# dblanm/gnn-manip

Hardware: AMD Instinct MI355X
Metric: rollout steps/sec (N particles, 10 MP steps, hidden=128) (higher is better)
Workload: dtype f32; 1 GPU; north_star target: N=100k dense synthetic scene, conn_r=0.015, max_neighbours=20, hidden=128, 10 MP steps; n_particles=100000, hidden=128, edges_last_step=1966056, k_steps=6, candidates_per_gpu=1, parallelism=candidate-parallel x1

## Files before the change

gnn_manip_amd/_lib.py:

```python
import ctypes as C
import os

_HERE = os.path.dirname(os.path.abspath(__file__))
LIB_PATH = os.environ.get("GM_LIB_PATH") or os.path.join(_HERE, "libgnnmanip_hip.so")

GM_OK = 0


class GMError(RuntimeError):
    def __init__(self, code, msg):
        super().__init__(f"libgnnmanip_hip: {msg} (status {code})")
        self.code = code


class FeatureDesc(C.Structure):
    _fields_ = [("conn_r", C.c_double), ("k_steps", C.c_int32), ("data_dim", C.c_int32),
                ("cart_col", C.c_int32), ("material_col", C.c_int32), ("control_col", C.c_int32),
                ("nodes_per_graph", C.c_int32),
                ("vel_mean", C.c_float * 3), ("vel_std", C.c_float * 3),
                ("acc_mean", C.c_float * 3), ("acc_std", C.c_float * 3),
                ("lower_bounds", C.c_float * 3), ("upper_bounds", C.c_float * 3)]


class ModelDesc(C.Structure):
# ... 40 lines not shown
    "gm_state_post_backward": (_i32, [_vp, _i64, _FD, _vp, _i32, _vp, _vp, _vp, _vp]),
    "gm_rigid_transform": (_i32, [_vp, _i64, _vp, _i64, C.POINTER(_f32 * 3), _vp, _vp]),
    "gm_rigid_transform_backward": (_i32, [_vp, _i64, _vp, _i64, C.POINTER(_f32 * 3), _vp, _vp, _vp]),
    "gm_model_num_tensors": (_i32, [_MD]),
    "gm_model_create": (_i32, [_MD, C.POINTER(_vp), _i32, _i32, _vp, C.POINTER(_vp)]),
    "gm_model_update": (_i32, [_vp, C.POINTER(_vp), _i32, _i32, _vp]),
    "gm_model_destroy": (None, [_vp]),
    "gm_forward_workspace_bytes": (_sz, [_MD, _i64, _i64]),
    "gm_block_workspace_bytes": (_sz, [_MD, _i64, _i64]),
    "gm_epd_forward": (_i32, [_vp, _vp, _i64, _vp, _i32, _vp, _i64, _vp, _vp, _sz, _vp]),
    "gm_graph_independent_forward": (_i32, [_vp, _vp, _i64, _vp, _i64, _vp, _vp, _vp]),
    "gm_interaction_network_forward": (_i32, [_vp, _i32, _vp, _i64, _vp, _vp, _i64, _vp, _vp, _vp, _sz, _vp]),
    "gm_train_tape_bytes": (_sz, [_MD, _i64, _i64]),
    "gm_train_backward_workspace_bytes": (_sz, [_MD, _i64, _i64]),
    "gm_epd_forward_train": (_i32, [_vp, _vp, _i64, _vp, _vp, _i64, _vp, _vp, _sz, _vp]),
    "gm_epd_backward": (_i32, [_vp, _vp, _i32, _vp, _vp, _i64, _i64, _vp, _vp, _vp, _sz, _vp, _sz, _vp]),
    "gm_train_backward_inputs_workspace_bytes": (_sz, [_MD, _i64, _i64]),
    "gm_epd_backward_inputs": (_i32, [_vp, _vp, _i32, _vp, _vp, _i64, _i64, _vp, _vp, _vp, _vp, _vp, _sz, _vp, _sz, _vp]),
    "gm_epd_backward_inputs_only": (_i32, [_vp, _vp, _i32, _vp, _vp, _i64, _i64, _vp, _vp, _vp, _vp, _sz, _vp, _sz, _vp]),
    "gm_block_tape_bytes": (_sz, [_MD, _i32, _i64, _i64]),
    "gm_block_backward_workspace_bytes": (_sz, [_MD, _i64, _i64]),
    "gm_graph_independent_forward_train": (_i32, [_vp, _vp, _i64, _vp, _i64, _vp, _vp, _vp, _sz, _vp]),
    "gm_graph_independent_backward": (_i32, [_vp, _vp, _i32, _vp, _vp, _i64, _i64, _vp, _vp, _vp, _vp, _vp, _vp, _sz, _vp, _sz, _vp]),
    "gm_interaction_network_forward_train": (_i32, [_vp, _i32, _vp, _i64, _vp, _vp, _i64, _vp, _vp, _vp, _sz, _vp]),
    "gm_interaction_network_backward": (_i32, [_vp, _i32, _vp, _i32, _vp, _vp, _i64, _i64, _vp, _vp, _vp, _vp, _vp, _vp, _sz, _vp, _sz, _vp]),
    "gm_sinkhorn_workspace_bytes": (_sz, [_i64, _i64]),
    "gm_sinkhorn_divergence": (_i32, [_vp, _i64, _vp, _i64, _f32, _f32, _vp, _vp, _sz, _vp]),
    "gm_sinkhorn_batched_workspace_bytes": (_sz, [_i64, _i64, _i64]),
    "gm_sinkhorn_divergence_batched": (_i32, [_vp, _i64, _i64, _vp, _i64, _i32, _f32, _f32, _f32, _vp, _vp, _sz, _vp]),
    "gm_sinkhorn_batched_backward_workspace_bytes": (_sz, [_i64, _i64, _i64, _i32]),
    "gm_sinkhorn_divergence_batched_backward": (_i32, [_vp, _i64, _i64, _vp, _i64, _i32, _f32, _f32, _vp, _vp, _vp, _vp, _sz, _vp, _sz, _vp]),
    "gm_rollout_workspace_bytes": (_sz, [_MD, _i64, _i32]),
    "gm_rollout_step": (_i32, [_vp, _vp, _i64, _FD, _i32, _vp, _vp, _vp, _vp, _sz, _vp]),
    "gm_rollout_renumber_workspace_bytes": (_sz, [_FD, _i64]),
    "gm_rollout": (_i32, [_vp, _vp, _i64, _FD, _i32, _vp, _vp, _i64, _i64, _i64, _vp, _i64, _vp, _sz, _vp, _sz, _vp]),
    "gm_rollout_status": (_i32, [_vp, _MD, _i64, _i32, C.POINTER(_i64), _vp]),
    "gm_state_recorded": (_i32, [_vp, _i64, _FD, _vp, _vp, _vp, _i32, _vp]),
    "gm_rollout_recorded": (_i32, [_vp, _vp, _i64, _FD, _i32, _vp, _vp, _i64, _vp, _vp, _i64, _vp, _sz, _vp, _sz, _vp]),
    "gm_rollout_errors": (_i32, [_vp, _vp, _vp, _i64, _i64, _i64, _i64, _FD, _vp, _vp]),
    "gm_rollout_step_backward_workspace_bytes": (_sz, [_MD, _FD, _i64, _i32]),
    "gm_rollout_step_backward": (_i32, [_vp, _vp, _i32, _vp, _i64, _FD, _i32, _vp, _vp, _vp, _vp, _vp, C.POINTER(_i64), _vp, _sz, _vp]),
    "gm_rollout_backward_workspace_bytes": (_sz, [_MD, _FD, _i64, _i32]),
    "gm_rollout_backward": (_i32, [_vp, _vp, _i32, _vp, _i64, _FD, _i32, _vp, _vp, _i64, _i64, _i64, _vp, _vp, _vp, _vp, _sz, _vp]),
    "gm_rollout_step_backward_train": (_i32, [_vp, _vp, _i32, _vp, _i64, _FD, _i32, _vp, _vp, _vp, _vp, _vp, _vp, _vp, C.POINTER(_i64), _vp, _sz,
                                              _vp]),
    "gm_rollout_backward_train": (_i32, [_vp, _vp, _i32, _vp, _i64, _FD, _i32, _vp, _vp, _i64, _i64, _i64, _vp, _vp, _vp, _vp, _vp, _vp, _sz,
                                         _vp]),
    "gm_train_batch_workspace_bytes": (_sz, [_FD, _i64, _i64, _i32]),
    "gm_train_batch_build": (_i32, [_vp, _i64, _i64, _i32, _FD, _i32, _f64, _u64, _u64, _vp, _vp, _vp, _vp, _vp, _sz, _vp]),
    "gm_train_batch_edges": (_i32, [_vp, _i64, _i64, _FD, _i32, _i64, _vp, _vp, _vp]),
    "gm_train_batch_ragged_workspace_bytes": (_sz, [_FD, _i64, _i64, _i32]),
    "gm_train_batch_build_ragged": (_i32, [_vp, _vp, _i64, _i32, _FD, _i32, _f64, _u64, _u64, _vp, _vp, _vp, _vp, _vp, _sz, _vp]),
    "gm_train_batch_edges_ragged": (_i32, [_vp, _vp, _i64, _FD, _i32, _i64, _vp, _vp, _vp]),
    "gm_train_batch_num_edges": (_i32, [_vp, C.POINTER(_i64), _vp]),
    "gm_train_batch_status": (_i32, [_vp, C.POINTER(_i64)]),
    "gm_l1_loss_workspace_bytes": (_sz, [_i64, _i32]),
    "gm_l1_loss": (_i32, [_vp, _vp, _i64, _i32, _vp, _i32, _i32, _vp, _vp, _vp, _vp, _sz, _vp]),
    "gm_trainer_create": (_i32, [_vp, _f64, _f64, _f64, _vp, C.POINTER(_vp)]),
    "gm_trainer_destroy": (None, [_vp]),
    "gm_train_step_workspace_bytes": (_sz, [_MD, _i64, _i64]),
    "gm_train_step": (_i32, [_vp, _vp, _i64, _vp, _vp, _i64, _vp, _i32, _f64, _vp, _vp, _sz, _vp]),
    "gm_trainer_record": (_i32, [_vp, _vp, _vp]),
    "gm_trainer_export": (_i32, [_vp, _i32, C.POINTER(_vp), _i32, _vp]),
    "gm_trainer_import": (_i32, [_vp, _i32, C.POINTER(_vp), _i32, _i64, _vp]),
    "gm_rollout_l1_loss_workspace_bytes": (_sz, [_i64, _i64]),
    "gm_rollout_l1_loss": (_i32, [_vp, _vp, _vp, _i32, _i64, _i64, _FD, _vp, _i32, _vp, _vp, _vp, _vp, _vp, _vp, _sz, _vp]),
    "gm_train_rollout_step_workspace_bytes": (_sz, [_MD, _FD, _i64, _i64, _i32, _i64]),
    "gm_train_rollout_step": (_i32, [_vp, _vp, _i64, _FD, _i32, _vp, _i64, _vp, _i32, _i64, _i32, _vp, _f64, _i32, _vp, _vp,
                                     _sz, _vp]),
    "gm_trainer_begin": (_i32, [_vp, _vp]),
    "gm_train_step_accumulate": (_i32, [_vp, _vp, _i64, _vp, _vp, _i64, _vp, _i32, _vp, _vp, _sz, _vp]),
    "gm_train_rollout_accumulate": (_i32, [_vp, _vp, _i64, _FD, _i32, _vp, _i64, _vp, _i32, _i64, _i32, _vp, _vp, _vp, _sz, _vp]),
    "gm_trainer_apply": (_i32, [_vp, _f64, _f64, _vp, _vp, _vp]),
    "gm_trainer_accum_record": (_i32, [_vp, _vp, _vp]),
    "gm_grad_sumsq_workspace_bytes": (_sz, [_i64]),
    "gm_grad_sumsq": (_i32, [_vp, _i64, _vp, _vp, _sz, _vp]),
    "gm_rank_sum": (_i32, [_vp, _i64, _i32, _i64, _vp, _vp]),
    "gm_trainer_contribution_bytes": (_sz, [_vp]),
    "gm_trainer_contribution": (_i32, [_vp, _vp, _sz, _i32, _vp]),
    "gm_trainer_reduce": (_i32, [_vp, _vp, _i32, _sz, _i64, _vp]),
    "gm_model_profile": (_i32, [_vp, _i32]),
    "gm_model_set_edge_kernel": (_i32, [_vp, _i32]),
    "gm_model_set_node_fusion": (_i32, [_vp, _i32]),
    "gm_model_set_precision": (_i32, [_vp, _i32]),
    "gm_model_profile_query": (_i32, [_vp, _i32, C.POINTER(_i64), C.POINTER(_f64)]),
}

_lib = None


def lib():
    global _lib
    if _lib is None:
        if not os.path.exists(LIB_PATH):
            raise RuntimeError(
                f"{LIB_PATH} not found: the HIP extension has not been built "
                "(run `python -m gnn_manip_amd.build`). gnn_manip_amd has no CPU fallback.")
        handle = C.CDLL(LIB_PATH)
        for name, (res, args) in PROTOTYPES.items():
            fn = getattr(handle, name)
            fn.restype = res
            fn.argtypes = args
        _lib = handle
    return _lib


def check(status):
    if status != GM_OK:
        msg = lib().gm_last_error()
        raise GMError(status, msg.decode() if msg else "unknown error")


import threading

_tls = threading.local()


def ptr(t):
    if t is None:
        return None
    assert t.is_contiguous(), "libgnnmanip_hip needs contiguous tensors"
    if t.is_cuda:
        _tls.device = t.device
    return C.c_void_p(t.data_ptr())


def current_stream(device=None):
    import torch
    if device is not None and not isinstance(device, torch.device):
        device = device.device
    dev = device if device is not None else getattr(_tls, "device", None)
    return C.c_void_p(torch.cuda.current_stream(dev).cuda_stream)
```

gnn_manip_amd/csrc/blocks_dev.h:

```cpp
#pragma once
#include "common.h"
#include "hedge.h"

namespace gm {

constexpr int kBlockEdges = 32;
__host__ __device__ inline int edge_blocks_padded(int n_edges) { return ((n_edges + kBlockEdges - 1) / kBlockEdges + 3) & ~3; }

#if defined(__HIPCC__)
__device__ inline void edge_blocks_plan(const int* __restrict__ in_ptr, int n_nodes, const int* n_per_dev, int n_per_host,
                                        EdgeBlockHeader* tab, int* gblk, int max_graphs) {
    int n_per = n_per_dev ? *n_per_dev : n_per_host;
    if (n_per <= 0) n_per = n_nodes > 0 ? n_nodes : 1;
    int G = (n_nodes + n_per - 1) / n_per;
    if (G > max_graphs) G = max_graphs;
    int pb = 0;
    for (int g = 0; g < G; ++g) {
        const int lo = g * n_per, hi = min(n_nodes, (g + 1) * n_per);
        gblk[g] = pb;
        pb += edge_blocks_padded(in_ptr[hi] - in_ptr[lo]);
    }
    gblk[G] = pb;
    tab->n_blocks = pb;
    tab->n_groups = pb / 4;
    tab->n_graphs = G;
    tab->n_per_graph = n_per;
    tab->n_stitch = 0;
}

__device__ inline void edge_blocks_fill(const int* __restrict__ in_ptr, const int* __restrict__ dst, int n_nodes, EdgeBlockHeader* tab,
                                        const int* __restrict__ gblk, int2* blk, int2* seg, int* __restrict__ head, int* __restrict__ stitch,
                                        int* __restrict__ stitch_list, int t, int nt) {
    constexpr int BE = kBlockEdges;
    const int nblk = tab->n_blocks, G = tab->n_graphs, n_per = tab->n_per_graph;
    for (int b = t; b < nblk; b += nt) {
        int lo = 0, hi = G;
        while (hi - lo > 1) {
            const int mid = (lo + hi) >> 1;
            if (gblk[mid] <= b) lo = mid; else hi = mid;
        }
        const int g = lo, j = b - gblk[g];
        const int e0 = in_ptr[g * n_per], e1 = in_ptr[min(n_nodes, (g + 1) * n_per)];
        const int start = min(e0 + j * BE, e1);
        const int cnt = min(BE, e1 - start);
        const int fl = ((j & 3) == 0 ? 1 : 0) | ((j & 3) == 3 ? 2 : 0);
        blk[b] = make_int2(start, cnt | (fl << 8));
        {
            unsigned cont = 0, last = 0;
            int prev = (cnt > 0 && (j & 3) != 0 && start > e0) ? dst[start - 1] : -1;
            for (int n = 0; n < cnt; ++n) {
                const int d = dst[start + n];
                if (d == prev) cont |= 1u << n;
                prev = d;
                bool is_last;
                if (n + 1 < cnt) is_last = dst[start + n + 1] != d;
                else is_last = (j & 3) == 3 || cnt < BE || start + cnt >= e1 || dst[start + cnt] != d;
                if (is_last) last |= 1u << n;
            }
            seg[b] = make_int2((int)cont, (int)last);
        }
        if ((j & 3) == 0) {
            int h = -1;
            if (cnt > 0 && start > e0 && dst[start - 1] == dst[start]) h = dst[start];
            head[b >> 2] = h;
            if (h >= 0) {
                const int ps = start - 4 * BE;
                const bool prev_is_head = j >= 4 && dst[ps] == h && ps > e0 && dst[ps - 1] == h;
                if (!prev_is_head) {
                    stitch[h] = b >> 2;
                    stitch_list[atomicAdd(&tab->n_stitch, 1)] = h;
                }
            }
        }
    }
}
#endif

}
```

gnn_manip_amd/csrc/common.h:

```cpp
#pragma once
#include <hip/hip_runtime.h>
#include <stdint.h>
#include <stdio.h>
#include <string.h>
#include <mutex>
#include "../../include/gnn_manip_hip.h"

namespace gm {

void set_error(const char* fmt, ...);

#define GM_HIP_CHECK(expr)                                                                  \
    do {                                                                                    \
        hipError_t _e = (expr);                                                             \
        if (_e != hipSuccess) {                                                             \
            gm::set_error("%s failed: %s (%s:%d)", #expr, hipGetErrorString(_e), __FILE__,  \
                          __LINE__);                                                        \
            return GM_ERR_HIP;                                                              \
        }                                                                                   \
    } while (0)

#define GM_REQUIRE(cond, code, ...)          \
    do {                                     \
        if (!(cond)) {                       \
// ... 72 lines not shown
    int n_per_graph;
    int ncells_local;
    int ticket;
    int order_skip;
};

struct GraphWs {
    GraphHeader* hdr;
    int* cell_of;
    int* cell_start;
    int* cell_cursor;
    float4* sorted;
    int* cnt;
    int* out_ptr;
    int* nbr;
    int* scan_cells;
    int* scan_cnt;
    int max_cells;
    size_t bytes;
};
int max_cells_for(int64_t n);
GraphWs carve_graph(void* ws, int64_t n, int max_nb);

struct CsrHeader {
    int n_edges;
    int error_flags;
    int flow;
    int pad;
};
struct CsrWs {
    CsrHeader* hdr;
    int* in_ptr;
    int* cursor;
    int* dst;
    int* src;
    int* eid;
    int* scan_in;
    int* sort_tmp;
    int64_t cap;
    int* blocks;
    size_t bytes;
};
CsrWs carve_csr(void* ws, int64_t n, int64_t cap);

enum ProfKind : int { PROF_EDGE = 0, PROF_NODE = 1, PROF_GRAPH = 2, PROF_ENC = 3, PROF_REST = 4, PROF_KINDS = 5 };
constexpr int PROF_MAX = 4096;
struct ProfState {
    int mask = 0;
    int count[PROF_KINDS] = {};
    int dropped[PROF_KINDS] = {};
    hipEvent_t* start[PROF_KINDS] = {};
    hipEvent_t* stop[PROF_KINDS] = {};
    ~ProfState();
};
struct ProfScope {
    ProfState* p;
    int idx;
    int kind;
    hipStream_t s;
    ProfScope(ProfState* state, int kind, hipStream_t s);
    ~ProfScope();
};

struct StepClear;
struct RecordedDrive {
    const float* frame;
    const int* row_map;
    float* record;
    float* pred;
};
int rollout_pre_features(float* obs, int64_t n, const gm_feature_desc* d, const int* rank, const float* target, float* out,
                         hipStream_t s, const StepClear* clear,
                         const RecordedDrive* rec = nullptr);
int rollout_integrate_post(float* obs, int64_t n, const gm_feature_desc* d, const float* pred, const int* rank,
                           const float* target, float* pred_out, hipStream_t s, const RecordedDrive* rec = nullptr);
int renumber_gather(const float* in, float* out, int k, int64_t n, int D, const int* perm, const void* graph_ws, const int* total_in,
                    int* total_out, const int* rank_caller, int* rank_out, hipStream_t s);
int renumber_scatter(const float* in, float* out, int frames, int64_t n, int D, const int* total, hipStream_t s);
int csr_from_graph_with_features(const void* graph_ws, int64_t n, int K, void* csr_ws, size_t csr_ws_bytes, const float* pos,
                                 int64_t pos_stride, float conn_r, float* edge_attr, int flow, hipStream_t s);
int csr_from_edge_index(const int64_t* ei, int64_t n, int64_t e, int flow, void* csr_ws, size_t csr_ws_bytes, bool with_blocks, hipStream_t stream);

int cell_order(const float* pos, int64_t pos_stride, int64_t n, int64_t n_per, double conn_r, int K, void* graph_ws, size_t graph_ws_bytes,
               int* perm, hipStream_t s);

size_t scan_state_ints(int64_t n_max);
struct ScanJob {
    const int* in;
    int* out;
    long long n;
    int* total_out;
    int* state;
};
int scan_lookback(const ScanJob* jobs, int n_jobs, hipStream_t s);

struct ClearJob {
    int* p;
    long long n;
    int v;
};
constexpr int kClearJobsMax = 12;
struct GraphHeader;
struct StepClear {
    int n_jobs = 0;
    ClearJob job[kClearJobsMax] = {};
    GraphHeader* gh = nullptr;
    CsrHeader* ch = nullptr;
    int flow = 0;
    int add(int* p, long long n, int v) {
        if (!p || n <= 0) return GM_OK;
        GM_REQUIRE(n_jobs < kClearJobsMax, GM_ERR_INVALID_ARGUMENT, "StepClear: more than %d resets in one pass", kClearJobsMax);
        job[n_jobs++] = ClearJob{p, n, v};
        return GM_OK;
    }
};
int launch_step_clear(const StepClear& c, hipStream_t s);
#if defined(__HIPCC__)
__device__ inline void step_clear_run(const StepClear& c, long long t, long long nt) {
    for (int q = 0; q < c.n_jobs; ++q) {
        int* p = c.job[q].p;
        const long long n = c.job[q].n;
        const int v = c.job[q].v;
        if ((reinterpret_cast<uintptr_t>(p) & 15) == 0 && n >= 4) {
            const long long n4 = n >> 2;
            int4* p4 = reinterpret_cast<int4*>(p);
            for (long long i = t; i < n4; i += nt) p4[i] = make_int4(v, v, v, v);
            for (long long i = (n4 << 2) + t; i < n; i += nt) p[i] = v;
        } else {
            for (long long i = t; i < n; i += nt) p[i] = v;
        }
    }
    if (t == 0) {
        if (GraphHeader* hdr = c.gh) {
            hdr->n_edges = 0;
            hdr->error_flags = 0;
            hdr->ncells = 1;
            for (int a = 0; a < 3; ++a) {
                hdr->bbox_min[a] = 0xffffffffu;
                hdr->bbox_max[a] = 0u;
                hdr->dims[a] = 1;
                hdr->origin[a] = 0.0;
            }
            hdr->inv_h = 1.0;
            hdr->n_per_graph = 1;
            hdr->ncells_local = 1;
            hdr->ticket = 0;
            hdr->order_skip = 0;
        }
        if (CsrHeader* ch = c.ch) {
            ch->n_edges = 0;
            ch->error_flags = 0;
            ch->flow = c.flow;
            ch->pad = 0;
        }
    }
}
#endif
struct GraphWs;
struct CsrWs;
int graph_clear_jobs(StepClear& c, const GraphWs& g, int64_t n);
int csr_clear_jobs(StepClear& c, const CsrWs& w, int64_t n, int flow);

int radius_graph_build_fused(const float* pos, int64_t pos_stride, int64_t n, int64_t n_per, double conn_r, int K, void* graph_ws,
                             size_t graph_ws_bytes, void* csr_ws, size_t csr_ws_bytes, int flow, hipStream_t s);
int csr_from_graph_fused(const void* graph_ws, int64_t n, int K, void* csr_ws, size_t csr_ws_bytes, const float* pos, int64_t pos_stride,
                         float conn_r, float* edge_attr, int flow, hipStream_t s);

}
```

gnn_manip_amd/csrc/features.hip:

```cpp
#include "common.h"
#include "step_rows.h"

namespace gm {

int to_params(const gm_feature_desc* d, FeatParams* p, const char* who) {
    GM_REQUIRE(d != nullptr, GM_ERR_INVALID_ARGUMENT, "%s: null feature descriptor", who);
    GM_REQUIRE(d->k_steps >= 2 && d->k_steps <= 64, GM_ERR_INVALID_ARGUMENT, "%s: k_steps=%d out of range", who, d->k_steps);
    GM_REQUIRE(d->data_dim >= 4 && d->cart_col >= 0 && d->cart_col + 3 <= d->data_dim, GM_ERR_INVALID_ARGUMENT,
               "%s: bad cartesian columns", who);
    GM_REQUIRE(d->material_col >= 0 && d->material_col < d->data_dim, GM_ERR_INVALID_ARGUMENT, "%s: bad material column", who);
    GM_REQUIRE(d->control_col < 0 || d->control_col + 3 <= d->data_dim, GM_ERR_INVALID_ARGUMENT, "%s: bad control columns", who);
    GM_REQUIRE(d->conn_r > 0.0, GM_ERR_INVALID_ARGUMENT, "%s: conn_r must be > 0", who);
    p->k = d->k_steps; p->D = d->data_dim; p->cart = d->cart_col; p->mat = d->material_col; p->ctrl = d->control_col;
    p->r = (float)d->conn_r;
    for (int a = 0; a < 3; ++a) {
        p->vm[a] = d->vel_mean[a]; p->vs[a] = d->vel_std[a];
        p->am[a] = d->acc_mean[a]; p->as[a] = d->acc_std[a];
        p->lo[a] = d->lower_bounds[a]; p->hi[a] = d->upper_bounds[a];
    }
    return GM_OK;
}

template <class Kernel, class... Args>
static int launch_rows(Kernel kernel, int64_t rows, hipStream_t s, Args... args) {
// ... 171 lines not shown
#pragma unroll
        for (int x = 0; x < 3; ++x) {
            const double d = (double)a[x] - (double)b[x];
            e += d * d;
        }
        s_all += e;
        if (gf[r * P.D + P.mat] != 0.0f) continue;
        s_cof += e;
        cnt += 1.0;
        if (!pred) continue;
        double ea = 0.0;
#pragma unroll
        for (int x = 0; x < 3; ++x) {
            const double acc = ((double)b[fs + x] - 2.0 * (double)b[x]) + (double)b[x - fs];
            const double d = (double)pred[(step * n + r) * 3 + x] - (acc - (double)P.am[x]) / (double)P.as[x];
            ea += d * d;
        }
        s_acc += ea;
    }
    red[0][tid] = s_all; red[1][tid] = s_cof; red[2][tid] = s_acc; red[3][tid] = cnt;
    __syncthreads();
    for (int w = 128; w >= 1; w >>= 1) {
        if (tid < w) {
#pragma unroll
            for (int q = 0; q < 4; ++q) red[q][tid] += red[q][tid + w];
        }
        __syncthreads();
    }
    if (tid < 4) sums[(int64_t)blockIdx.x * 4 + tid] = red[tid][0];
}

__global__ void __launch_bounds__(256) rigid_transform_kernel(const float* __restrict__ init, int64_t nr,
                                                               const float* __restrict__ cst, int64_t steps, float tx,
                                                               float ty, float tz, float* __restrict__ out) {
    const int64_t id = (int64_t)blockIdx.x * blockDim.x + threadIdx.x;
    if (id >= nr * steps) return;
    const int64_t t = id / nr, i = id - t * nr;
    const float c = cst[t * 3], s = cst[t * 3 + 1], typ = cst[t * 3 + 2];
    const float i0 = __fsub_rn(tx, init[i * 3 + 0]);
    const float i1 = __fsub_rn(ty, init[i * 3 + 2]);
    const float i2 = __fsub_rn(tz, init[i * 3 + 1]);
    const float p0 = __fadd_rn(i0, tx);
    const float p1 = __fadd_rn(__fmaf_rn(-s, i2, __fmul_rn(c, i1)), typ);
    const float p2 = __fadd_rn(__fmaf_rn(c, i2, __fmul_rn(s, i1)), tz);
    out[id * 3 + 0] = p0;
    out[id * 3 + 2] = p1;
    out[id * 3 + 1] = p2;
}

__global__ void __launch_bounds__(256) rigid_transform_bwd_kernel(const float* __restrict__ init, int64_t nr, float ty, float tz,
                                                                   const float* __restrict__ g, float* __restrict__ d_cst) {
    __shared__ double red[3][256];
    const int tid = threadIdx.x;
    const int64_t t = blockIdx.x;
    const float* gt = g + t * nr * 3;
    double dc = 0.0, ds = 0.0, dt = 0.0;
    for (int64_t i = tid; i < nr; i += 256) {
        const double i1 = (double)ty - (double)init[i * 3 + 2];
        const double i2 = (double)tz - (double)init[i * 3 + 1];
        const double g1 = gt[i * 3 + 1], g2 = gt[i * 3 + 2];
        dc += g2 * i1 + g1 * i2;
        ds += g1 * i1 - g2 * i2;
        dt += g2;
    }
    red[0][tid] = dc; red[1][tid] = ds; red[2][tid] = dt;
    __syncthreads();
    for (int w = 128; w >= 1; w >>= 1) {
        if (tid < w) {
#pragma unroll
            for (int a = 0; a < 3; ++a) red[a][tid] += red[a][tid + w];
        }
        __syncthreads();
    }
    if (tid < 3) d_cst[t * 3 + tid] = (float)red[tid][0];
}

__global__ void __launch_bounds__(256) renumber_gather_kernel(const float* __restrict__ in, float* __restrict__ out, int k, int64_t n, int D,
                                                               const int* __restrict__ perm, const GraphHeader* __restrict__ ghdr,
                                                               const int* __restrict__ total_in, int* __restrict__ total_out,
                                                               const int* __restrict__ rank_caller, int* __restrict__ rank_out) {
    const int64_t id = (int64_t)blockIdx.x * blockDim.x + threadIdx.x;
    if (id >= (int64_t)k * n) return;
    const int64_t t = id / n, j = id - t * n;
    const int64_t src = ghdr->order_skip ? j : (int64_t)perm[j];
    const float* a = in + (t * n + src) * D;
    float* b = out + (t * n + j) * D;
    for (int d = 0; d < D; ++d) b[d] = a[d];
    if (t == 0) {
        const int tot = total_in ? total_in[src] : (int)src;
        total_out[j] = tot;
        if (rank_out) rank_out[j] = rank_caller[tot];
    }
}
__global__ void __launch_bounds__(256) renumber_scatter_kernel(const float* __restrict__ in, float* __restrict__ out, int frames, int64_t n, int D,
                                                                const int* __restrict__ total) {
    const int64_t id = (int64_t)blockIdx.x * blockDim.x + threadIdx.x;
    if (id >= (int64_t)frames * n) return;
    const int64_t t = id / n, j = id - t * n;
    const float* a = in + (t * n + j) * D;
    float* b = out + (t * n + (int64_t)total[j]) * D;
    for (int d = 0; d < D; ++d) b[d] = a[d];
}
int renumber_gather(const float* in, float* out, int k, int64_t n, int D, const int* perm, const void* graph_ws, const int* total_in,
                    int* total_out, const int* rank_caller, int* rank_out, hipStream_t s) {
    if (n <= 0 || k <= 0) return GM_OK;
    return launch_rows(renumber_gather_kernel, (int64_t)k * n, s, in, out, k, n, D, perm, static_cast<const GraphHeader*>(graph_ws), total_in,
                       total_out, rank_caller, rank_out);
}
int renumber_scatter(const float* in, float* out, int frames, int64_t n, int D, const int* total, hipStream_t s) {
    if (n <= 0 || frames <= 0) return GM_OK;
    return launch_rows(renumber_scatter_kernel, (int64_t)frames * n, s, in, out, frames, n, D, total);
}

int rollout_pre_features(float* obs, int64_t n, const gm_feature_desc* d, const int* rank, const float* target, float* out,
                         hipStream_t s, const StepClear* clear, const RecordedDrive* rec) {
    FeatParams P;
    int rc = to_params(d, &P, "gm_rollout_step");
    if (rc != GM_OK) return rc;
    const StepClear clr = clear ? *clear : StepClear{};
    if (rec) return launch_rows(pre_features_kernel<RecordedDrive>, n, s, obs, n, P, rank, target, out, clr, *rec);
    return launch_rows(pre_features_kernel<>, n, s, obs, n, P, rank, target, out, clr);
}

int rollout_integrate_post(float* obs, int64_t n, const gm_feature_desc* d, const float* pred, const int* rank,
                           const float* target, float* pred_out, hipStream_t s, const RecordedDrive* rec) {
    FeatParams P;
    int rc = to_params(d, &P, "gm_rollout_step");
    if (rc != GM_OK) return rc;
    if (rec) return launch_rows(integrate_post_kernel<RecordedDrive>, n, s, obs, n, P, pred, rank, target, pred_out, *rec);
    return launch_rows(integrate_post_kernel<>, n, s, obs, n, P, pred, rank, target, pred_out);
}



__device__ __forceinline__ void zero_window_row(float* __restrict__ row, int64_t fs, const FeatParams& P) {
    for (int t = 0; t < P.k; ++t)
        for (int d = 0; d < P.D; ++d) row[t * fs + d] = 0.f;
}

__global__ void __launch_bounds__(256) node_features_bwd_kernel(const float* __restrict__ obs, int64_t n, FeatParams P,
                                                                 const float* __restrict__ g, float* __restrict__ d_obs) {
    const int64_t i = (int64_t)blockIdx.x * blockDim.x + threadIdx.x;
    if (i >= n) return;
    const float* gi = g + i * node_feature_dim(P.k, P.ctrl);
    const int64_t fs = n * P.D;
    float* row = d_obs + i * P.D;
    zero_window_row(row, fs, P);
    for (int t = 0; t < P.k; ++t) {
#pragma unroll
        for (int a = 0; a < 3; ++a) {
            float v = 0.f;
            if (t >= 1) v = __fdiv_rn(gi[(t - 1) * 3 + a], P.vs[a]);
            if (t + 1 < P.k) v = __fsub_rn(v, __fdiv_rn(gi[t * 3 + a], P.vs[a]));
            row[t * fs + P.cart + a] = v;
        }
    }
    const float* b = gi + 3 * (P.k - 1);
    const float* last_in = obs + (int64_t)(P.k - 1) * fs + i * P.D;
    float* last = row + (int64_t)(P.k - 1) * fs;
#pragma unroll
    for (int a = 0; a < 3; ++a) {
        float l, u;
        boundary_terms(last_in[P.cart + a], P, a, l, u);
        float v = last[P.cart + a];
        if (in_unit(l)) v = __fadd_rn(v, __fdiv_rn(b[a], P.r));
        if (in_unit(u)) v = __fsub_rn(v, __fdiv_rn(b[3 + a], P.r));
        last[P.cart + a] = v;
// ... 414 lines not shown
```

gnn_manip_amd/csrc/graph.hip:

```cpp
#include <stdarg.h>
#include "common.h"
#include "hedge.h"
#include "blocks_dev.h"
#include "step_rows.h"

namespace gm {

static thread_local char g_err[512] = "";
void set_error(const char* fmt, ...) {
    va_list ap;
    va_start(ap, fmt);
    vsnprintf(g_err, sizeof(g_err), fmt, ap);
    va_end(ap);
}
const char* last_error() { return g_err; }

ProfState::~ProfState() {
    for (int k = 0; k < PROF_KINDS; ++k) {
        if (!start[k]) continue;
        for (int i = 0; i < PROF_MAX; ++i) { (void)hipEventDestroy(start[k][i]); (void)hipEventDestroy(stop[k][i]); }
        delete[] start[k];
        delete[] stop[k];
    }
}
// ... 299 lines not shown
            d[a] = (int)c;
            prod *= c;
        }
        if (prod <= (double)max_cells) break;
        h *= 1.2599210498948732;
    }
    for (int a = 0; a < 3; ++a) {
        hdr->dims[a] = d[a];
        hdr->origin[a] = lo[a];
    }
    hdr->inv_h = 1.0 / h;
    hdr->ncells_local = d[0] * d[1] * d[2];
    hdr->ncells = hdr->ncells_local * (int)n_graphs;
    hdr->n_per_graph = RAGGED ? (int)n : (int)(n_per > 0 ? n_per : (n > 0 ? n : 1));
}

__device__ __forceinline__ int cell_coord(float v, double origin, double inv_h, int dim) {
    double c = floor(((double)v - origin) * inv_h);
    int ci = (c > 0.0) ? (c < (double)(dim - 1) ? (int)c : dim - 1) : 0;
    return ci;
}

__device__ __forceinline__ int ragged_graph_of_row(const RaggedOffsets& R, int64_t i) {
    __shared__ int s_off[GM_RAGGED_MAX_GRAPHS + 1];
    for (int t = threadIdx.x; t <= R.n_graphs; t += blockDim.x) s_off[t] = R.off[t];
    __syncthreads();
    int lo = 0, hi = R.n_graphs;
    while (hi - lo > 1) {
        const int mid = (lo + hi) >> 1;
        if ((int64_t)s_off[mid] <= i) lo = mid; else hi = mid;
    }
    return lo;
}

template <typename... Ragged>
__global__ void __launch_bounds__(256) cell_assign_kernel(const float* __restrict__ pos, int64_t stride, int64_t n,
                                                           const GraphHeader* __restrict__ hdr,
                                                           int* __restrict__ cell_of, int* __restrict__ cell_count, Ragged... ragged) {
    int64_t i = (int64_t)blockIdx.x * blockDim.x + threadIdx.x;
    int graph = 0;
    if constexpr (sizeof...(Ragged) != 0) graph = ragged_graph_of_row(ragged..., i < n ? i : n - 1);
    if (i >= n) return;
    const int dx = hdr->dims[0], dy = hdr->dims[1], dz = hdr->dims[2];
    float x = pos[i * stride], y = pos[i * stride + 1], z = pos[i * stride + 2];
    if (!isfinite(x)) x = 0.f;
    if (!isfinite(y)) y = 0.f;
    if (!isfinite(z)) z = 0.f;
    int cx = cell_coord(x, hdr->origin[0], hdr->inv_h, dx);
    int cy = cell_coord(y, hdr->origin[1], hdr->inv_h, dy);
    int cz = cell_coord(z, hdr->origin[2], hdr->inv_h, dz);
    if constexpr (sizeof...(Ragged) == 0) graph = (int)(i / hdr->n_per_graph);
    int c = graph * hdr->ncells_local + (cz * dy + cy) * dx + cx;
    cell_of[i] = c;
    atomicAdd(&cell_count[c], 1);
}

__global__ void __launch_bounds__(256) cell_fill_kernel(const float* __restrict__ pos, int64_t stride, int64_t n,
                                                         const int* __restrict__ cell_of,
                                                         const int* __restrict__ cell_start,
                                                         int* __restrict__ cell_cursor, float4* __restrict__ sorted) {
    int64_t i = (int64_t)blockIdx.x * blockDim.x + threadIdx.x;
    if (i >= n) return;
    int c = cell_of[i];
    int p = cell_start[c] + atomicAdd(&cell_cursor[c], 1);
    sorted[p] = make_float4(pos[i * stride], pos[i * stride + 1], pos[i * stride + 2], __int_as_float((int)i));
}

constexpr int kCellOrderCap = 1024;
__global__ void __launch_bounds__(256) cell_order_kernel(const float4* __restrict__ sorted, const int* __restrict__ cell_of,
                                                          const int* __restrict__ cell_start, GraphHeader* hdr, int64_t n,
                                                          int* __restrict__ perm) {
    const int64_t p = (int64_t)blockIdx.x * blockDim.x + threadIdx.x;
    if (p >= n) return;
    const int i = __float_as_int(sorted[p].w);
    const int c = cell_of[i];
    const int lo = cell_start[c], hi = cell_start[c + 1];
    if (hi - lo > kCellOrderCap) {
        if (p == lo) atomicOr(&hdr->order_skip, 1);
        return;
    }
    int before = 0;
    for (int q = lo; q < hi; ++q) before += __float_as_int(sorted[q].w) < i ? 1 : 0;
    perm[lo + before] = i;
}

constexpr int NB_LPQ = 16;
constexpr int NB_CAP = 96;
constexpr int NB_STRIDE = NB_CAP + 1;
constexpr int NB_QPB = 256 / NB_LPQ;

struct Query {
    int qi;
    double x, y, z;
    int cbase, dx, dy, x0, x1, y0, y1, z0, z1;
    __device__ __forceinline__ void row_range(const int* __restrict__ cell_start, int zc, int yc, int& b, int& e) const {
        const int row = cbase + (zc * dy + yc) * dx;
        b = cell_start[row + x0];
        e = cell_start[row + x1 + 1];
    }
};
template <typename... CellOf>
__device__ __forceinline__ Query decode_query(const float4 q, const GraphHeader* __restrict__ hdr, CellOf... cell_of) {
    Query Q;
    Q.qi = __float_as_int(q.w);
    Q.dx = hdr->dims[0];
    Q.dy = hdr->dims[1];
    const int dz = hdr->dims[2];
    const double inv_h = hdr->inv_h;
    const int cx = cell_coord(q.x, hdr->origin[0], inv_h, Q.dx);
    const int cy = cell_coord(q.y, hdr->origin[1], inv_h, Q.dy);
    const int cz = cell_coord(q.z, hdr->origin[2], inv_h, dz);
    Q.x = (double)q.x; Q.y = (double)q.y; Q.z = (double)q.z;
    if constexpr (sizeof...(CellOf) == 0) {
        Q.cbase = (Q.qi / hdr->n_per_graph) * hdr->ncells_local;
    } else {
        const int own = (cell_of[Q.qi], ...);
        Q.cbase = own - own % hdr->ncells_local;
    }
    Q.x0 = max(cx - 1, 0); Q.x1 = min(cx + 1, Q.dx - 1);
    Q.y0 = max(cy - 1, 0); Q.y1 = min(cy + 1, Q.dy - 1);
    Q.z0 = max(cz - 1, 0); Q.z1 = min(cz + 1, dz - 1);
    return Q;
}
__device__ __forceinline__ double query_dist2(const Query& Q, const float4 p) {
    double d = Q.x - (double)p.x;
    double d2 = __dmul_rn(d, d);
    d = Q.y - (double)p.y;
    d2 = __dadd_rn(d2, __dmul_rn(d, d));
    d = Q.z - (double)p.z;
    return __dadd_rn(d2, __dmul_rn(d, d));
}

template <typename... CellOf>
__global__ void __launch_bounds__(256) neighbor_fast_kernel(const float4* __restrict__ sorted,
                                                             const int* __restrict__ cell_start,
                                                             const GraphHeader* __restrict__ hdr, int64_t n, double r2,
                                                             int K, int* __restrict__ cnt, int* __restrict__ nbr,
                                                             int* __restrict__ indeg, int* __restrict__ arrival, int flow,
                                                             CellOf... cell_of) {
    __shared__ double sd2[NB_QPB * NB_STRIDE];
    __shared__ int sj[NB_QPB * NB_STRIDE];
    const int tid = threadIdx.x, sub = tid & (NB_LPQ - 1), ql = tid / NB_LPQ, lane = tid & 63;
    const int grp_shift = (lane / NB_LPQ) * NB_LPQ;
    const int64_t slot = (int64_t)blockIdx.x * NB_QPB + ql;
    const bool active = slot < n;
    const Query Q = decode_query(sorted[active ? slot : 0], hdr, cell_of...);
    const int qi = Q.qi;
    double* ld = sd2 + ql * NB_STRIDE;
    int* lj = sj + ql * NB_STRIDE;
    int count = 0;
    if (active) {
        for (int z = Q.z0; z <= Q.z1; ++z) {
            for (int y = Q.y0; y <= Q.y1; ++y) {
                int b, e;
                Q.row_range(cell_start, z, y, b, e);
                for (int c0 = b; c0 < e; c0 += NB_LPQ) {
                    const int c = c0 + sub;
                    bool in = false;
                    double d2 = 0.0;
                    int j = 0;
                    if (c < e) {
                        const float4 p = sorted[c];
                        d2 = query_dist2(Q, p);
                        in = d2 <= r2;
                        j = __float_as_int(p.w);
                    }
// ... 50 lines not shown
    extern __shared__ __attribute__((aligned(16))) char smem[];
    double* kd = reinterpret_cast<double*>(smem);
    int* ki = reinterpret_cast<int*>(smem + (size_t)K * BS * 8);
    const int t = threadIdx.x;
    const int64_t slot = (int64_t)blockIdx.x * BS + t;
    if (slot >= n) return;
    const float4 q = sorted[slot];
    if (cnt[__float_as_int(q.w)] != -1) return;
    const Query Q = decode_query(q, hdr, cell_of...);
    const int qi = Q.qi;
    int kept = 0;
    for (int z = Q.z0; z <= Q.z1; ++z) {
        for (int y = Q.y0; y <= Q.y1; ++y) {
            int b, e;
            Q.row_range(cell_start, z, y, b, e);
            for (int c = b; c < e; ++c) {
                const float4 p = sorted[c];
                const double d2 = query_dist2(Q, p);
                if (!(d2 <= r2)) continue;
                const int j = __float_as_int(p.w);
                int pos;
                if (kept < K) {
                    pos = kept++;
                } else {
                    const double ld = kd[(K - 1) * BS + t];
                    const int lj = ki[(K - 1) * BS + t];
                    if (!(d2 < ld || (d2 == ld && j < lj))) continue;
                    pos = K - 1;
                }
                while (pos > 0) {
                    const double pd = kd[(pos - 1) * BS + t];
                    const int pj = ki[(pos - 1) * BS + t];
                    if (!(d2 < pd || (d2 == pd && j < pj))) break;
                    kd[pos * BS + t] = pd;
                    ki[pos * BS + t] = pj;
                    --pos;
                }
                kd[pos * BS + t] = d2;
                ki[pos * BS + t] = j;
            }
        }
    }
    cnt[qi] = kept;
    for (int s = 0; s < kept; ++s) {
        const int j = ki[s * BS + t];
        nbr[(int64_t)qi * K + s] = j;
        if (indeg) arrival[(int64_t)qi * K + s] = atomicAdd(&indeg[flow ? qi : j], 1);
    }
}

__device__ __forceinline__ bool decode_slot(int64_t id, int64_t n, int K, const int* __restrict__ cnt, int64_t& i, int& s) {
    if (id >= n * K) return false;
    i = id / K;
    s = (int)(id - i * K);
    return s < cnt[i];
}

__global__ void __launch_bounds__(256) emit_edges_kernel(const int* __restrict__ cnt, const int* __restrict__ out_ptr,
                                                          const int* __restrict__ nbr, int64_t n, int K,
                                                          int64_t capacity, int64_t* __restrict__ senders,
                                                          int64_t* __restrict__ receivers) {
    int64_t id = (int64_t)blockIdx.x * blockDim.x + threadIdx.x, i;
    int s;
    if (!decode_slot(id, n, K, cnt, i, s)) return;
    int64_t e = (int64_t)out_ptr[i] + s;
    if (e >= capacity) return;
    senders[e] = i;
    receivers[e] = nbr[id];
}

__global__ void __launch_bounds__(256) indeg_graph_kernel(const int* __restrict__ cnt, const int* __restrict__ nbr,
                                                           int64_t n, int K, int flow, int* __restrict__ indeg, int* __restrict__ slot) {
    int64_t id = (int64_t)blockIdx.x * blockDim.x + threadIdx.x, i;
    int s;
    if (!decode_slot(id, n, K, cnt, i, s)) return;
    slot[id] = atomicAdd(&indeg[flow ? (int)i : nbr[id]], 1);
}

__global__ void __launch_bounds__(256) fill_graph_kernel(const int* __restrict__ cnt, const int* __restrict__ out_ptr,
                                                          const int* __restrict__ nbr, int64_t n, int K,
                                                          const int* __restrict__ in_ptr, const int* __restrict__ slot,
                                                          int64_t cap, int flow, int* __restrict__ dst, int* __restrict__ src,
                                                          int* __restrict__ eid, CsrHeader* hdr, const int* n_per_dev,
                                                          EdgeBlockHeader* tab, int* gblk) {
    int64_t id = (int64_t)blockIdx.x * blockDim.x + threadIdx.x, i;
    int s;
    if (id == 0 && tab) edge_blocks_plan(in_ptr, (int)n, n_per_dev, 0, tab, gblk, (int)n + 1);
    if (!decode_slot(id, n, K, cnt, i, s)) return;
    const int d = flow ? (int)i : nbr[id];
    int p = in_ptr[d] + slot[id];
    if (p >= cap) { atomicOr(&hdr->error_flags, ERRF_CAPACITY); return; }
    dst[p] = d;
    src[p] = flow ? nbr[id] : (int)i;
    eid[p] = out_ptr[i] + s;
}

__device__ __forceinline__ bool decode_endpoints(const int64_t* __restrict__ ei, int64_t n, int64_t e, int64_t id, int flow, int64_t& s,
                                                 int64_t& d) {
    s = ei[flow ? e + id : id];
    d = ei[flow ? id : e + id];
    return s >= 0 && s < n && d >= 0 && d < n;
}

__global__ void __launch_bounds__(256) indeg_ei_kernel(const int64_t* __restrict__ ei, int64_t n, int64_t e, int flow,
                                                        int* __restrict__ indeg, CsrHeader* hdr) {
    int64_t id = (int64_t)blockIdx.x * blockDim.x + threadIdx.x, s, d;
    if (id >= e) return;
    if (!decode_endpoints(ei, n, e, id, flow, s, d)) { atomicOr(&hdr->error_flags, ERRF_BAD_EDGE_INDEX); return; }
    atomicAdd(&indeg[d], 1);
}

__global__ void __launch_bounds__(256) fill_ei_kernel(const int64_t* __restrict__ ei, int64_t n, int64_t e, int flow,
                                                       const int* __restrict__ in_ptr, int* __restrict__ cursor,
                                                       int* __restrict__ dst, int* __restrict__ src,
                                                       int* __restrict__ eid, CsrHeader* hdr) {
    int64_t id = (int64_t)blockIdx.x * blockDim.x + threadIdx.x, s, d;
    if (id >= e) return;
    if (!decode_endpoints(ei, n, e, id, flow, s, d)) {
        const int p = (int)e - 1 - atomicAdd(&hdr->pad, 1);
        dst[p] = 0;
        src[p] = 0;
        eid[p] = (int)id;
        return;
    }
    int p = in_ptr[d] + atomicAdd(&cursor[d], 1);
    dst[p] = (int)d;
    src[p] = (int)s;
    eid[p] = (int)id;
}

constexpr int SEG_LPS = 8;
constexpr int SEG_PER_WG = 256 / SEG_LPS;
constexpr int SEG_CAP = 96;
constexpr int SEG_STRIDE = SEG_CAP + 1;
struct BlockTabArgs {
    const int* dst;
    EdgeBlockHeader* hdr;
    const int* gblk;
    int2* blk;
    int2* seg;
    int* head;
    int* stitch;
    int* stitch_list;
    int n_tab;
};
__global__ void __launch_bounds__(256) segment_sort_kernel(const int* __restrict__ in_ptr, int64_t n,
                                                            int* __restrict__ src, int* __restrict__ eid,
                                                            CsrHeader* hdr, const float* __restrict__ pos,
                                                            int64_t pos_stride, float conn_r, float* __restrict__ edge_attr, int flow,
                                                            int* __restrict__ tmp_eid, int* __restrict__ tmp_src, BlockTabArgs bt) {
    __shared__ int se[SEG_PER_WG * SEG_STRIDE];
    __shared__ int ss[SEG_PER_WG * SEG_STRIDE];
    __shared__ int s_long[SEG_PER_WG];
    if ((int)blockIdx.x < bt.n_tab) {
        edge_blocks_fill(in_ptr, bt.dst, (int)n, bt.hdr, bt.gblk, bt.blk, bt.seg, bt.head, bt.stitch, bt.stitch_list,
                         (int)blockIdx.x * 256 + (int)threadIdx.x, bt.n_tab * 256);
        return;
    }
    const int wg = (int)blockIdx.x - bt.n_tab;
    const int tid = threadIdx.x, sub = tid & (SEG_LPS - 1), sl = tid / SEG_LPS;
    const int64_t i = (int64_t)wg * SEG_PER_WG + sl;
    if (i == 0 && sub == 0) hdr->n_edges = in_ptr[n];
    const bool active = i < n;
    const int b = active ? in_ptr[i] : 0, e = active ? in_ptr[i + 1] : 0;
    const int len = e - b;
    int* le = se + sl * SEG_STRIDE;
    int* ls = ss + sl * SEG_STRIDE;
    const bool small = len <= SEG_CAP;
    if (small)
        for (int a = sub; a < len; a += SEG_LPS) {
            le[a] = eid[b + a];
            ls[a] = src[b + a];
        }
    if (sub == 0) s_long[sl] = (active && !small) ? 1 : 0;
    __syncthreads();
    auto write_attr = [&](int64_t node, int srcv, int64_t at) {
        const int64_t s = flow ? node : (int64_t)srcv, r = flow ? (int64_t)srcv : node;
        *reinterpret_cast<float4*>(edge_attr + at * 4) = edge_feature(pos + s * pos_stride, pos + r * pos_stride, conn_r);
    };
    if (active && small) {
        for (int a = sub; a < len; a += SEG_LPS) {
            const int ka = le[a];
            int rank = 0;
            for (int f = 0; f < len; ++f) rank += le[f] < ka ? 1 : 0;
            eid[b + rank] = ka;
            src[b + rank] = ls[a];
            if (edge_attr) write_attr(i, ls[a], (int64_t)b + rank);
        }
    }
    for (int q = 0; q < SEG_PER_WG; ++q) {
        if (!s_long[q]) continue;
        const int64_t node = (int64_t)wg * SEG_PER_WG + q;
        const int lb = in_ptr[node], ll = in_ptr[node + 1] - lb;
        for (int a = tid; a < ll; a += 256) { tmp_eid[lb + a] = eid[lb + a]; tmp_src[lb + a] = src[lb + a]; }
        __syncthreads();
        for (int a = tid; a < ll; a += 256) {
            const int ka = tmp_eid[lb + a];
            int rank = 0;
            for (int f = 0; f < ll; ++f) rank += tmp_eid[lb + f] < ka ? 1 : 0;
            eid[lb + rank] = ka;
            src[lb + rank] = tmp_src[lb + a];
            if (edge_attr) write_attr(node, tmp_src[lb + a], (int64_t)lb + rank);
        }
        __syncthreads();
    }
}

static int grid_phase(const float* pos, int64_t pos_stride, int64_t n, int64_t n_per, double conn_r, const GraphWs& g, hipStream_t s,
                      const RaggedOffsets* ragged = nullptr) {
    const int nb = (int)cdiv(n, 256);
    if (ragged) {
        hipLaunchKernelGGL(bbox_kernel<true>, dim3(nb < 64 ? nb : 64), dim3(256), 0, s, pos, pos_stride, n, g.hdr, conn_r, g.max_cells,
                           (int64_t)ragged->n_graphs);
        hipLaunchKernelGGL(cell_assign_kernel<RaggedOffsets>, dim3(nb), dim3(256), 0, s, pos, pos_stride, n, g.hdr, g.cell_of, g.cell_start,
                           *ragged);
    } else {
        hipLaunchKernelGGL(bbox_kernel<false>, dim3(nb < 64 ? nb : 64), dim3(256), 0, s, pos, pos_stride, n, g.hdr, conn_r, g.max_cells, n_per);
        hipLaunchKernelGGL(cell_assign_kernel<>, dim3(nb), dim3(256), 0, s, pos, pos_stride, n, g.hdr, g.cell_of, g.cell_start);
    }
    const ScanJob sj{g.cell_start, g.cell_start, (long long)g.max_cells + 1, nullptr, g.scan_cells};
    const int rc = scan_lookback(&sj, 1, s);
    if (rc != GM_OK) return rc;
    hipLaunchKernelGGL(cell_fill_kernel, dim3(nb), dim3(256), 0, s, pos, pos_stride, n, g.cell_of, g.cell_start, g.cell_cursor, g.sorted);
    GM_LAUNCH_CHECK();
    return GM_OK;
}

int cell_order(const float* pos, int64_t pos_stride, int64_t n, int64_t n_per, double conn_r, int K, void* graph_ws, size_t graph_ws_bytes,
               int* perm, hipStream_t s) {
    GM_REQUIRE(pos && graph_ws && perm && n > 0 && pos_stride >= 3 && conn_r > 0.0, GM_ERR_INVALID_ARGUMENT, "cell_order: bad argument");
    GraphWs g = carve_graph(graph_ws, n, K);
    GM_REQUIRE(graph_ws_bytes >= g.bytes, GM_ERR_WORKSPACE, "cell_order: workspace %zu < %zu", graph_ws_bytes, g.bytes);
    StepClear clr;
    int rc = graph_clear_jobs(clr, g, n);
    if (rc == GM_OK) rc = launch_step_clear(clr, s);
    if (rc == GM_OK) rc = grid_phase(pos, pos_stride, n, n_per, conn_r, g, s);
    if (rc != GM_OK) return rc;
    hipLaunchKernelGGL(cell_order_kernel, dim3((unsigned)cdiv(n, 256)), dim3(256), 0, s, g.sorted, g.cell_of, g.cell_start, g.hdr, n, perm);
    GM_LAUNCH_CHECK();
    return GM_OK;
}

}

using namespace gm;

extern "C" {

const char* gm_last_error(void) { return gm::last_error(); }

int gm_abi_version(void) { return 7; }

size_t gm_graph_workspace_bytes(int64_t n_nodes, int max_neighbours) {
    if (n_nodes < 0 || max_neighbours < 1) return 0;
    return carve_graph(nullptr, n_nodes, max_neighbours).bytes;
}

int gm_radius_graph_build(const float* pos, int64_t pos_stride, int64_t n, double conn_r, int K, void* ws,
                          size_t ws_bytes, void* stream) {
    return gm_radius_graph_build_batched(pos, pos_stride, n, n, conn_r, K, ws, ws_bytes, stream);
}

}

namespace {
int check_build_args(const float* pos, int64_t pos_stride, int64_t n, int64_t n_per, double conn_r, int K, const void* ws) {
    GM_REQUIRE(n_per >= 0 && (n_per == 0 || n % n_per == 0 || n_per >= n), GM_ERR_INVALID_ARGUMENT,
               "gm_radius_graph_build_batched: n_nodes=%lld is not a multiple of nodes_per_graph=%lld", (long long)n, (long long)n_per);
    GM_REQUIRE(n >= 0 && n < (int64_t)1 << 30, GM_ERR_INVALID_ARGUMENT, "gm_radius_graph_build: n_nodes=%lld out of range", (long long)n);
    GM_REQUIRE(K >= 1 && K <= 160, GM_ERR_UNSUPPORTED, "gm_radius_graph_build: max_neighbours=%d unsupported (1..160)", K);
    GM_REQUIRE(n * (int64_t)K < (int64_t)1 << 31, GM_ERR_UNSUPPORTED, "gm_radius_graph_build: n*max_neighbours overflows int32");
    GM_REQUIRE(conn_r > 0.0 && conn_r == conn_r, GM_ERR_INVALID_ARGUMENT, "gm_radius_graph_build: conn_r must be > 0");
    GM_REQUIRE(pos_stride >= 3, GM_ERR_INVALID_ARGUMENT, "gm_radius_graph_build: pos_stride < 3");
    GM_REQUIRE(ws != nullptr && (pos != nullptr || n == 0), GM_ERR_INVALID_ARGUMENT, "gm_radius_graph_build: null pointer");
    return GM_OK;
}

template <int BS, typename... CellOf>
int launch_neighbor(const GraphWs& g, int64_t n, double r2, int K, int* indeg, int* slot, int flow, hipStream_t s, CellOf... cell_of) {
    const auto kernel = neighbor_kernel<BS, CellOf...>;
    const size_t lds = (size_t)K * BS * 12;
    GM_REQUIRE(lds <= 160 * 1024, GM_ERR_UNSUPPORTED, "gm_radius_graph_build: max_neighbours=%d needs %zu bytes of LDS", K, lds);
    if (lds > 64 * 1024) {
        static PerDeviceOnce big_lds;
        const int rc_attr = big_lds.run([kernel]() -> int {
            GM_HIP_CHECK(hipFuncSetAttribute(reinterpret_cast<const void*>(kernel), hipFuncAttributeMaxDynamicSharedMemorySize, 160 * 1024));
            return GM_OK;
        });
        if (rc_attr != GM_OK) return rc_attr;
    }
    hipLaunchKernelGGL(kernel, dim3((int)cdiv(n, BS)), dim3(BS), lds, s, g.sorted, g.cell_start, g.hdr, n, r2, K, g.cnt, g.nbr,
                       indeg, slot, flow, cell_of...);
    GM_LAUNCH_CHECK();
    return GM_OK;
}

}
namespace gm {
int radius_graph_check_args(const float* pos, int64_t pos_stride, int64_t n, int64_t n_per, double conn_r, int K, const void* ws) {
    return check_build_args(pos, pos_stride, n, n_per, conn_r, K, ws);
}
int radius_graph_build_core(const float* pos, int64_t pos_stride, int64_t n, int64_t n_per, double conn_r, int K, const GraphWs& g,
                            int* indeg, int* slot, int flow, hipStream_t s) {
    if (n <= 0) return GM_OK;
    const int rc = grid_phase(pos, pos_stride, n, n_per, conn_r, g, s);
    if (rc != GM_OK) return rc;
    const double r2 = conn_r * conn_r;
    hipLaunchKernelGGL(neighbor_fast_kernel<>, dim3((unsigned)cdiv(n, NB_QPB)), dim3(256), 0, s, g.sorted, g.cell_start,
                       g.hdr, n, r2, K, g.cnt, g.nbr, indeg, slot, flow);
    return K <= 64 ? launch_neighbor<128>(g, n, r2, K, indeg, slot, flow, s) : launch_neighbor<64>(g, n, r2, K, indeg, slot, flow, s);
}
int radius_graph_build_ragged_core(const float* pos, int64_t pos_stride, const RaggedOffsets& R, double conn_r, int K, const GraphWs& g,
                                   hipStream_t s) {
    const int64_t n = R.off[R.n_graphs];
    const int rc = grid_phase(pos, pos_stride, n, 0, conn_r, g, s, &R);
    if (rc != GM_OK) return rc;
    const double r2 = conn_r * conn_r;
    const int* cell_of = g.cell_of;
    hipLaunchKernelGGL(neighbor_fast_kernel<const int*>, dim3((unsigned)cdiv(n, NB_QPB)), dim3(256), 0, s, g.sorted, g.cell_start,
                       g.hdr, n, r2, K, g.cnt, g.nbr, (int*)nullptr, (int*)nullptr, 0, cell_of);
    return K <= 64 ? launch_neighbor<128>(g, n, r2, K, nullptr, nullptr, 0, s, cell_of) : launch_neighbor<64>(g, n, r2, K, nullptr, nullptr, 0, s, cell_of);
// ... 29 lines not shown
    if (rc != GM_OK) return rc;
    GraphWs g = carve_graph(ws, n, K);
    GM_REQUIRE(ws_bytes >= g.bytes, GM_ERR_WORKSPACE, "gm_radius_graph_build: workspace %zu < %zu", ws_bytes, g.bytes);
    hipStream_t s = (hipStream_t)stream;
    StepClear clr;
    rc = graph_clear_jobs(clr, g, n);
    if (rc == GM_OK) rc = launch_step_clear(clr, s);
    if (rc == GM_OK) rc = radius_graph_build_core(pos, pos_stride, n, n_per, conn_r, K, g, nullptr, nullptr, 0, s);
    if (rc != GM_OK) return rc;
    const ScanJob sj{g.cnt, g.out_ptr, (long long)n + 1, &g.hdr->n_edges, g.scan_cnt};
    return scan_lookback(&sj, 1, s);
}

size_t gm_graph_ragged_workspace_bytes(int64_t n_nodes, int64_t n_graphs, int max_neighbours) {
    if (n_graphs < 1 || n_graphs > GM_RAGGED_MAX_GRAPHS || n_nodes < n_graphs || n_nodes >= (int64_t)1 << 30) return 0;
    if (max_neighbours < 1 || max_neighbours > 160 || n_nodes * max_neighbours >= (int64_t)1 << 31) return 0;
    return carve_graph(nullptr, n_nodes, max_neighbours).bytes;
}

int gm_radius_graph_build_ragged(const float* pos, int64_t pos_stride, const int64_t* graph_offsets_host, int64_t n_graphs, double conn_r,
                                 int K, void* ws, size_t ws_bytes, void* stream) {
    const char* who = "gm_radius_graph_build_ragged";
    RaggedOffsets R;
    int rc = ragged_offsets(graph_offsets_host, n_graphs, conn_r, K, ws, who, &R);
    if (rc != GM_OK) return rc;
    GM_REQUIRE(pos, GM_ERR_INVALID_ARGUMENT, "%s: null pointer", who);
    GM_REQUIRE(pos_stride >= 3, GM_ERR_INVALID_ARGUMENT, "%s: pos_stride < 3", who);
    const int64_t n = R.off[R.n_graphs];
    GraphWs g = carve_graph(ws, n, K);
    GM_REQUIRE(ws_bytes >= g.bytes, GM_ERR_INVALID_ARGUMENT, "%s: workspace %zu < %zu", who, ws_bytes, g.bytes);
    gm::DevGuard dev_guard(pos);
    hipStream_t s = (hipStream_t)stream;
    StepClear clr;
    rc = graph_clear_jobs(clr, g, n);
    if (rc == GM_OK) rc = launch_step_clear(clr, s);
    if (rc == GM_OK) rc = radius_graph_build_ragged_core(pos, pos_stride, R, conn_r, K, g, s);
    if (rc != GM_OK) return rc;
    const ScanJob sj{g.cnt, g.out_ptr, (long long)n + 1, &g.hdr->n_edges, g.scan_cnt};
    return scan_lookback(&sj, 1, s);
}

int gm_radius_graph_num_edges(const void* ws, int64_t* n_edges_host, void* stream) {
    gm::DevGuard dev_guard(ws);
    GM_REQUIRE(ws && n_edges_host, GM_ERR_INVALID_ARGUMENT, "gm_radius_graph_num_edges: null pointer");
    GraphHeader h;
    GM_HIP_CHECK(hipMemcpyAsync(&h, ws, sizeof(h), hipMemcpyDeviceToHost, (hipStream_t)stream));
    GM_HIP_CHECK(hipStreamSynchronize((hipStream_t)stream));
    *n_edges_host = h.n_edges;
    GM_REQUIRE(!(h.error_flags & ERRF_NONFINITE_POS), GM_ERR_DATA, "radius graph: non-finite position in input");
    return GM_OK;
}

int gm_radius_graph_edges(const void* ws, int64_t n, int K, int64_t* senders, int64_t* receivers, int64_t capacity,
                          void* stream) {
    gm::DevGuard dev_guard(ws);
    GM_REQUIRE(ws && (capacity == 0 || (senders && receivers)), GM_ERR_INVALID_ARGUMENT, "gm_radius_graph_edges: null pointer");
    if (n == 0 || capacity == 0) return GM_OK;
    GraphWs g = carve_graph(const_cast<void*>(ws), n, K);
    hipLaunchKernelGGL(emit_edges_kernel, dim3((unsigned)cdiv(n * K, 256)), dim3(256), 0, (hipStream_t)stream, g.cnt,
                       g.out_ptr, g.nbr, n, K, capacity, senders, receivers);
    GM_LAUNCH_CHECK();
    return GM_OK;
}

size_t gm_csr_workspace_bytes(int64_t n_nodes, int64_t edge_capacity) {
    if (n_nodes < 0 || edge_capacity < 0) return 0;
    return carve_csr(nullptr, n_nodes, edge_capacity).bytes;
}

int gm_csr_from_graph(const void* graph_ws, int64_t n, int K, void* csr_ws, size_t csr_ws_bytes, void* stream) {
    return gm_csr_from_graph_flow(graph_ws, n, K, 0, csr_ws, csr_ws_bytes, stream);
}

int gm_csr_from_graph_flow(const void* graph_ws, int64_t n, int K, int flow, void* csr_ws, size_t csr_ws_bytes, void* stream) {
    gm::DevGuard dev_guard(graph_ws);
    return gm::csr_from_graph_with_features(graph_ws, n, K, csr_ws, csr_ws_bytes, nullptr, 3, 1.f, nullptr, flow, (hipStream_t)stream);
}

}

namespace gm {
namespace {
int csr_tail(const GraphWs& g, int64_t n, int K, const CsrWs& c, const float* pos, int64_t pos_stride, float conn_r, float* edge_attr,
             int flow, bool with_cnt_scan, hipStream_t s) {
    const int64_t cap = n * K;
    const unsigned nb = (unsigned)cdiv(cap, 256);
    int* slot = c.sort_tmp;
    ScanJob sj[2] = {{c.in_ptr, c.in_ptr, (long long)n + 1, nullptr, c.scan_in},
                     {g.cnt, g.out_ptr, (long long)n + 1, &g.hdr->n_edges, g.scan_cnt}};
    int rc = scan_lookback(sj, with_cnt_scan ? 2 : 1, s);
    if (rc != GM_OK) return rc;
    const EdgeBlocks t = carve_edge_blocks(c.blocks, n, cap);
    hipLaunchKernelGGL(fill_graph_kernel, dim3(nb), dim3(256), 0, s, g.cnt, g.out_ptr, g.nbr, n, K, c.in_ptr,
                       slot, cap, flow, c.dst, c.src, c.eid, c.hdr, &g.hdr->n_per_graph, t.hdr, t.gblk);
    int gb = (int)cdiv(cdiv(cap, kBlockEdges) + 8, 256);
    gb = gb < 1 ? 1 : (gb > 512 ? 512 : gb);
    const BlockTabArgs bt{c.dst, t.hdr, t.gblk, t.blk, t.seg, t.head, t.stitch, t.stitch_list, gb};
    hipLaunchKernelGGL(segment_sort_kernel, dim3((unsigned)cdiv(n, SEG_PER_WG) + (unsigned)gb), dim3(256), 0, s, c.in_ptr, n, c.src, c.eid, c.hdr,
                       pos, pos_stride, conn_r, edge_attr, flow, c.sort_tmp, c.sort_tmp + c.cap, bt);
    GM_LAUNCH_CHECK();
    return GM_OK;
}
}

int csr_from_graph_with_features(const void* graph_ws, int64_t n, int K, void* csr_ws, size_t csr_ws_bytes, const float* pos,
                                 int64_t pos_stride, float conn_r, float* edge_attr, int flow, hipStream_t stream) {
    GM_REQUIRE(graph_ws && csr_ws, GM_ERR_INVALID_ARGUMENT, "gm_csr_from_graph: null pointer");
    GM_REQUIRE(flow == 0 || flow == 1, GM_ERR_INVALID_ARGUMENT, "gm_csr_from_graph: flow must be 0 or 1");
    const int64_t cap = n * K;
    GraphWs g = carve_graph(const_cast<void*>(graph_ws), n, K);
    CsrWs c = carve_csr(csr_ws, n, cap);
    GM_REQUIRE(csr_ws_bytes >= c.bytes, GM_ERR_WORKSPACE, "gm_csr_from_graph: workspace %zu < %zu", csr_ws_bytes, c.bytes);
    hipStream_t s = (hipStream_t)stream;
    StepClear clr;
    int rc = csr_clear_jobs(clr, c, n, flow);
    if (rc == GM_OK) rc = launch_step_clear(clr, s);
    if (rc != GM_OK || n <= 0) return rc;
    hipLaunchKernelGGL(indeg_graph_kernel, dim3((unsigned)cdiv(cap, 256)), dim3(256), 0, s, g.cnt, g.nbr, n, K, flow, c.in_ptr, c.sort_tmp);
    return csr_tail(g, n, K, c, pos, pos_stride, conn_r, edge_attr, flow, false, s);
}

int radius_graph_build_fused(const float* pos, int64_t pos_stride, int64_t n, int64_t n_per, double conn_r, int K, void* graph_ws,
                             size_t graph_ws_bytes, void* csr_ws, size_t csr_ws_bytes, int flow, hipStream_t s) {
    int rc = check_build_args(pos, pos_stride, n, n_per, conn_r, K, graph_ws);
    if (rc != GM_OK) return rc;
    GM_REQUIRE(csr_ws && (flow == 0 || flow == 1), GM_ERR_INVALID_ARGUMENT, "radius_graph_build_fused: bad csr workspace / flow");
    GraphWs g = carve_graph(graph_ws, n, K);
    CsrWs c = carve_csr(csr_ws, n, n * K);
    GM_REQUIRE(graph_ws_bytes >= g.bytes && csr_ws_bytes >= c.bytes, GM_ERR_WORKSPACE, "radius_graph_build_fused: workspace too small");
    return radius_graph_build_core(pos, pos_stride, n, n_per, conn_r, K, g, c.in_ptr, c.sort_tmp, flow, s);
}
int csr_from_graph_fused(const void* graph_ws, int64_t n, int K, void* csr_ws, size_t csr_ws_bytes, const float* pos, int64_t pos_stride,
                         float conn_r, float* edge_attr, int flow, hipStream_t s) {
    if (n <= 0) return GM_OK;
    GraphWs g = carve_graph(const_cast<void*>(graph_ws), n, K);
    CsrWs c = carve_csr(csr_ws, n, n * K);
    GM_REQUIRE(csr_ws_bytes >= c.bytes, GM_ERR_WORKSPACE, "csr_from_graph_fused: workspace %zu < %zu", csr_ws_bytes, c.bytes);
    return csr_tail(g, n, K, c, pos, pos_stride, conn_r, edge_attr, flow, true, s);
}
}

extern "C" {

int gm_csr_from_edge_index(const int64_t* ei, int64_t n, int64_t e, void* csr_ws, size_t csr_ws_bytes, void* stream) {
    return gm_csr_from_edge_index_flow(ei, n, e, 0, csr_ws, csr_ws_bytes, stream);
}

int gm_csr_from_edge_index_flow(const int64_t* ei, int64_t n, int64_t e, int flow, void* csr_ws, size_t csr_ws_bytes, void* stream) {
    return gm::csr_from_edge_index(ei, n, e, flow, csr_ws, csr_ws_bytes, true, (hipStream_t)stream);
}

}

namespace gm {
int csr_from_edge_index(const int64_t* ei, int64_t n, int64_t e, int flow, void* csr_ws, size_t csr_ws_bytes, bool with_blocks, hipStream_t stream) {
    gm::DevGuard dev_guard(csr_ws);
    GM_REQUIRE(flow == 0 || flow == 1, GM_ERR_INVALID_ARGUMENT, "gm_csr_from_edge_index: flow must be 0 or 1");
    GM_REQUIRE(csr_ws && (ei || e == 0), GM_ERR_INVALID_ARGUMENT, "gm_csr_from_edge_index: null pointer");
    GM_REQUIRE(n >= 0 && e >= 0 && e < ((int64_t)1 << 31) && n < ((int64_t)1 << 31), GM_ERR_INVALID_ARGUMENT,
               "gm_csr_from_edge_index: sizes out of range");
    CsrWs c = carve_csr(csr_ws, n, e);
    GM_REQUIRE(csr_ws_bytes >= c.bytes, GM_ERR_WORKSPACE, "gm_csr_from_edge_index: workspace %zu < %zu", csr_ws_bytes, c.bytes);
    hipStream_t s = (hipStream_t)stream;
    {
        StepClear clr;
        int rc = csr_clear_jobs(clr, c, n, flow);
        if (rc == GM_OK) rc = clr.add(c.cursor, n + 1, 0);
        if (rc == GM_OK) rc = launch_step_clear(clr, s);
        if (rc != GM_OK) return rc;
    }
    if (e > 0) {
        unsigned nb = (unsigned)cdiv(e, 256);
        hipLaunchKernelGGL(indeg_ei_kernel, dim3(nb), dim3(256), 0, s, ei, n, e, flow, c.in_ptr, c.hdr);
        const ScanJob sj{c.in_ptr, c.in_ptr, (long long)n + 1, nullptr, c.scan_in};
        int rc = scan_lookback(&sj, 1, s);
        if (rc != GM_OK) return rc;
        hipLaunchKernelGGL(fill_ei_kernel, dim3(nb), dim3(256), 0, s, ei, n, e, flow, c.in_ptr, c.cursor, c.dst, c.src, c.eid, c.hdr);
    }
    if (n > 0)
        hipLaunchKernelGGL(segment_sort_kernel, dim3((unsigned)cdiv(n, SEG_PER_WG)), dim3(256), 0, s, c.in_ptr, n, c.src, c.eid, c.hdr, nullptr, 3, 1.f, nullptr, 0, c.sort_tmp, c.sort_tmp + c.cap, BlockTabArgs{});
    GM_LAUNCH_CHECK();
    if (!with_blocks) return GM_OK;
    return build_edge_blocks(c.in_ptr, c.dst, n, nullptr, (int)n, carve_edge_blocks(c.blocks, n, e), s);
}
}

extern "C" {

int gm_csr_header_status(const int32_t* header_host, int64_t* n_edges_host) {
    GM_REQUIRE(header_host, GM_ERR_INVALID_ARGUMENT, "gm_csr_header_status: null pointer");
    CsrHeader h;
    memcpy(&h, header_host, sizeof(h));
    if (n_edges_host) *n_edges_host = h.n_edges;
    GM_REQUIRE(!(h.error_flags & ERRF_BAD_EDGE_INDEX), GM_ERR_DATA, "edge_index entry out of range [0, n_nodes)");
    GM_REQUIRE(!(h.error_flags & ERRF_CAPACITY), GM_ERR_DATA, "edge capacity exceeded");
    GM_REQUIRE(!(h.error_flags & ERRF_SPLIT_RANGE), GM_ERR_DATA,
               "fp16 split range exceeded: a feature, latent or hidden activation of the last forward over this edge structure reached "
               "|x| >= 65504 in a matrix-pipe operand image (include/gnn_manip_hip.h, numeric domain); its results are not valid");
    return GM_OK;
}

int gm_csr_num_edges(const void* csr_ws, int64_t* n_edges_host, void* stream) {
    gm::DevGuard dev_guard(csr_ws);
    GM_REQUIRE(csr_ws && n_edges_host, GM_ERR_INVALID_ARGUMENT, "gm_csr_num_edges: null pointer");
    CsrHeader h;
    GM_HIP_CHECK(hipMemcpyAsync(&h, csr_ws, sizeof(h), hipMemcpyDeviceToHost, (hipStream_t)stream));
    GM_HIP_CHECK(hipStreamSynchronize((hipStream_t)stream));
    return gm_csr_header_status(reinterpret_cast<const int32_t*>(&h), n_edges_host);
}

}
```

gnn_manip_amd/csrc/hedge.h:

```cpp
#pragma once
#include "common.h"
#include "mlp.h"

namespace gm {

struct EdgeBlockHeader {
    int n_blocks;
    int n_groups;
    int n_graphs;
    int n_per_graph;
    int n_stitch;
    int pad[3];
};
struct EdgeBlocks {
    EdgeBlockHeader* hdr;
    int* gblk;
    int2* blk;
    int2* seg;
    int* head;
    int* stitch;
    int* stitch_list;
    int64_t max_blocks;
};
size_t edge_blocks_ints(int64_t n_nodes, int64_t edge_capacity);
constexpr int kSinkRows = 1024;
size_t edge_groups_max(int64_t n_nodes, int64_t edge_capacity);
EdgeBlocks carve_edge_blocks(int* base, int64_t n_nodes, int64_t edge_capacity);
int build_edge_blocks(const int* in_ptr, const int* dst, int64_t n_nodes, const int* n_per_graph_dev, int n_per_graph_host, const EdgeBlocks& t, hipStream_t s);

constexpr int kPackH3Max = 16;
struct PackH3Job {
    const float* W1;
    int W1_col0;
    int W1_ld;
    const float* W2;
    const float* W3;
    const float* b1;
    const float* b2;
    const float* b3;
    const float* gamma;
    const float* beta;
    float* dst;
    int enc_k1;
};
size_t h3_image_floats();
int pack_h3(const PackH3Job* jobs, int n, hipStream_t s);

int launch_edge_sys(const EdgeArgs& a, const EdgeBlocks& t, int64_t edge_capacity, hipStream_t s);
inline const float* edge_sys_p_scale(const float* h3_image) { return h3_image; }

struct NodeSysArgs {
    const float* h;
    const float* agg;
    const float* Q;
    float* h_out;
    const float* image;
    int n;
    int* flags;
    float eps;
    ProfState* prof;
    int precision;
};
int launch_node_sys(const NodeSysArgs& a, hipStream_t s);
struct ProjSysArgs {
    const float* h;
    float* P;
    float* Q;
    const float* img_p;
    const float* img_q;
    const float* scale_p;
    const float* scale_q;
    int n;
    int* flags;
    ProfState* prof;
    int precision;
};
int launch_proj_sys(const ProjSysArgs& a, hipStream_t s);
int launch_node_proj_sys(const NodeSysArgs& a, const ProjSysArgs& p, hipStream_t s);
int launch_agg_stitch(float* agg, const float* side, const EdgeBlocks& t, int64_t n, ProfState* prof, hipStream_t s);
constexpr int64_t kSysNodeMinNodes = 32 * 256 * 6;
int launch_edge_sys_enc(const EdgeArgs& a, hipStream_t s);
bool edge_sys_fits(int64_t n_nodes, int64_t edge_capacity);
constexpr int kEdgePadRows = 32;
int zero_edge_pad_rows(const CsrHeader* hdr, float* e, int row_floats, hipStream_t s);

}
```

gnn_manip_amd/csrc/hedge.hip:

```cpp
#include <type_traits>
#include "common.h"
#include "mlp.h"
#include "hedge.h"
#include "hmlp.h"
#include "hmma_dev.h"
#include "blocks_dev.h"

namespace gm {

namespace {

constexpr int H = 128;
constexpr int BE = 32;
constexpr int SYS_THREADS = 768;
static_assert(BE == kBlockEdges, "block tables and the systolic kernels agree on the block size");
#ifdef HEDGE_STAMPS
__device__ unsigned long long g_sys_stamps[3 * 32 * 8 + 32];
#define SYS_STAMP(tick, slot)                                                                                         \
    do {                                                                                                              \
        if (blockIdx.x == 0 && jb == 0 && lane0 == 0 && (tick) >= 16 && (tick) < 48) {                                \
            g_sys_stamps[(role * 32 + (tick) - 16) * 8 + (slot)] = __builtin_readcyclecounter();                     \
            if (role == 0 && (slot) == 0) g_sys_stamps[3 * 32 * 8 + (tick) - 16] = __builtin_amdgcn_s_memrealtime(); \
        }                                                                                                             \
    } while (0)
// ... 187 lines not shown
}

__device__ __forceinline__ void set_role_prio(int role) {
    if (role == 2) __builtin_amdgcn_s_setprio(3);
    else __builtin_amdgcn_s_setprio(1);
}

__device__ __forceinline__ floatx16 vec_to_acc(char* smem, int vec_b, int f, int jb, int hi) {
    floatx16 a;
#pragma unroll
    for (int g = 0; g < 4; ++g) {
        const floatx4 v = LDS(floatx4, vec_b + (f + 32 * jb + 4 * hi + 8 * g) * 4);
#pragma unroll
        for (int tt = 0; tt < 4; ++tt) a[4 * g + tt] = v[tt];
    }
    return a;
}

__device__ __forceinline__ void publish_ln_stats(const floatx16& acc, unsigned st_w, unsigned z_w) {
    float q = 0.f;
#pragma unroll
    for (int r = 0; r < 16; ++r) q = fmaf(acc[r], acc[r], q);
    LDS(float, st_w) = sum_of_halves(q);
#pragma unroll
    for (int g = 0; g < 4; ++g) {
        floatx4 z;
#pragma unroll
        for (int tt = 0; tt < 4; ++tt) z[tt] = acc[4 * g + tt];
        LDS(floatx4, z_w + 32 * g) = z;
    }
}

struct LnGroup {
    float k;
    floatx4 z;
    __device__ __forceinline__ void load(unsigned km, unsigned zt) {
        k = LDS(float, km);
        z = LDS(floatx4, zt);
    }
    template <int AUX>
    __device__ __forceinline__ void store(float* out, unsigned r0, int j, int cnt, unsigned v_off, const floatx4& gm, const floatx4& bt, floatx4& e,
                                          float res_w, srd_t srd_e, unsigned res_row) const {
        floatx4 o;
#pragma unroll
        for (int tt = 0; tt < 4; ++tt) o[tt] = fmaf(e[tt], res_w, fmaf(z[tt] * k, gm[tt], bt[tt]));
        bst4s<AUX>(make_srd(out + (size_t)(r0 + 8 * j) * H, (unsigned)s_clamp0(cnt - 8 * j, 8) * 512u), v_off, 0, o);
        e = bld4(srd_e, v_off, res_row * 512 + j * 4096);
    }
};

#define RUN_TICKS(FIRST, last, tick)                                                   \
    _Pragma("unroll 1") for (int t_ = (FIRST); t_ <= (last); t_ += 2) {                \
        tick(std::integral_constant<int, (FIRST) & 1>{}, t_);                          \
        tick(std::integral_constant<int, 1 - ((FIRST) & 1)>{}, t_ + 1);                \
    }

constexpr int TICK_FULL = 0, TICK_FILL = 1, TICK_DRAIN = 2;
constexpr int TICK_IDLE = 3, TICK_LAST = 4;
template <int V>
using int_c = std::integral_constant<int, V>;

#define NODE_TICKS(tick_as)                                                                          \
    {                                                                                                \
        auto tick = [&](auto par_c, int t) { tick_as(par_c, int_c<TICK_FULL>{}, t); };               \
        tick_as(int_c<1>{}, int_c<TICK_FILL>{}, -1);                                                 \
        RUN_TICKS(0, nb, tick);                                                                      \
        if (nb & 1) {                                                                                \
            tick(int_c<0>{}, nb + 1);                                                                \
            tick_as(int_c<1>{}, int_c<TICK_DRAIN>{}, nb + 2);                                        \
        } else {                                                                                     \
            tick_as(int_c<0>{}, int_c<TICK_DRAIN>{}, nb + 2);                                        \
        }                                                                                            \
    }

template <bool MAY_BE_NULL = true>
__device__ __forceinline__ void report_split_range(int rng, int lane0, int* flags) {
    if (rng && lane0 == 0 && (!MAY_BE_NULL || flags)) atomicOr(flags, ERRF_SPLIT_RANGE);
}

template <bool WRITE_E, bool STREAM, int NP>
__global__ void __launch_bounds__(SYS_THREADS, 1) sys_edge_kernel(const CsrHeader* a_hdr, const int* __restrict__ a_dst, const int* __restrict__ a_src, const float* __restrict__ a_P,
                                                                       const float* a_e_in, float* a_e_out, float* __restrict__ a_agg, const float* __restrict__ a_hw,
                                                                       const int2* __restrict__ a_blk, const int2* __restrict__ a_seg, const int* __restrict__ a_head,
                                                                       const EdgeBlockHeader* __restrict__ a_tab, unsigned a_side_off, unsigned a_agg_bytes, unsigned a_P_bytes,
                                                                       int* a_flags, float a_eps, int a_residual) {
    const int tid = threadIdx.x, lane0 = tid & 63;
    const int wave = __builtin_amdgcn_readfirstlane(tid >> 6);
#ifdef HEDGE_FORCE_ROLE
    const int role = HEDGE_FORCE_ROLE, jb = wave & 3;
#else
    const int role = wave >> 2, jb = wave & 3;
#endif
    const int E = a_hdr->n_edges;
    const int2 cr = wg_range(a_tab->n_groups, true);
    if (cr.y <= cr.x) return;
    const int b0 = 4 * cr.x, b1 = 4 * cr.y;
    const int nb = b1 - b0;
    if (nb <= 0) return;
    const float inv_T = a_hw[1];
    half8 wh[8], wl[8];
    sys_prologue<NP>(wh, wl, reinterpret_cast<const half8*>(a_hw + HW_HEADER_FLOATS + HW_VEC_FLOATS), role * 4 + jb, false, L_ZERO_END, L_VEC,
                      a_hw + HW_HEADER_FLOATS, 4 * H);
    auto ok = [&](int x) { return x >= b0 && x < b1; };
    auto clampb = [&](int x) { return x < b0 ? b0 : (x < b1 ? x : b1 - 1); };
    const int e0 = a_blk[b0].x;
    const srd_t srd_ein = make_srd(a_e_in + (size_t)e0 * H, 0xffffffffu);
    const int n = lane0 & 31, hi = lane0 >> 5, rr = lane0 >> 3, cq = lane0 & 7;
    const unsigned v_eoff = opaque(rr * 512 + jb * 128 + cq * 16);
    set_role_prio(role);
    if (role == 0) {
        const srd_t srd_P = make_srd(a_P, a_P_bytes);
        const unsigned idx_bytes = (unsigned)s_clamp0(E - e0, 1 << 28) * 4u;
        const srd_t srd_dst = make_srd(a_dst + e0, idx_bytes), srd_src = make_srd(a_src + e0, idx_bytes);
        const unsigned v_poff = opaque(jb * 128 + cq * 16), v_ioff = opaque(rr * 16);
        const unsigned ps_w = opaque(L_PS + jb * TILE_B + 4 * rr * TILE_ROW_B + cq * 16);
        const unsigned ps_r = opaque(L_PS + jb * TILE_B + n * TILE_ROW_B + hi * 16);
        const int kg = cq & 1, ksb = cq >> 2, half = (cq >> 1) & 1;
        const unsigned e_w = opaque(L_E + ((2 * jb + ksb) * 2 * 64 + ((rr ^ (2 * (ksb + 2 * kg))) + 32 * kg)) * 16 + half * 8);
        const unsigned e_r0 = opaque(L_E + eslot(n, hi, 0) * 16), e_r1 = opaque(L_E + eslot(n, hi, 1) * 16);
        const unsigned x1_w = opaque(L_X1 + 4 * jb * 1024 + lane0 * 16);
        floatx4 pi[4], pj[4];
#pragma unroll
        for (int j = 0; j < 4; ++j) { pi[j] = floatx4{0.f, 0.f, 0.f, 0.f}; pj[j] = pi[j]; }
        int rng = 0;
        floatx4 eq[4];
#pragma unroll
        for (int j = 0; j < 4; ++j) eq[j] = bld4(srd_ein, v_eoff, j * 4096);
        floatx16 acc, c0v;
#pragma unroll
        for (int r = 0; r < 16; ++r) { c0v[r] = 0.f; acc[r] = 0.f; }
        intx4 di = bldi4(srd_dst, v_ioff, 0), si = bldi4(srd_src, v_ioff, 0);
        int2 be = a_blk[clampb(b0 + 1)];
        auto tick_as = [&](auto par_c, auto kind_c, int t) __attribute__((always_inline)) {
            constexpr int PAR = decltype(par_c)::value;
            constexpr int KIND = decltype(kind_c)::value;
            if constexpr (KIND == TICK_IDLE) {
                lds_barrier();
                return;
            }
            if constexpr (KIND == TICK_LAST) {
                auto nothing = [](int) {};
                mlp_layer<NP>(acc, c0v, wh, wl, smem, e_r0 + PAR * IMG_B, e_r1 + PAR * IMG_B, nothing);
                rng |= __any(row_bad<NP>(acc[0])) ? 1 : 0;
                GM_SB;
                acc_to_image<NP>(acc, smem, x1_w + PAR * IMG_B);
                lds_barrier();
                return;
            }
            const int x = b0 + t;
            SYS_STAMP(t, 0);
            auto prepare = [&]() {
#pragma unroll
                for (int j = 0; j < 4; ++j) LDS(floatx4, ps_w + j * TILE_ROW_B) = pi[j] + pj[j];
#pragma unroll
                for (int g = 0; g < 4; ++g) {
                    const floatx4 v = LDS(floatx4, ps_r + 32 * g);
#pragma unroll
                    for (int tt = 0; tt < 4; ++tt) c0v[4 * g + tt] = v[tt];
                }
            };
            SYS_STAMP(t, 1);
            if (jb == 0 && cq == 0) LDS(intx4, v_ioff + (L_DR + ((x + 1) & (DR_SLOTS - 1)) * (BE * 4))) = di;
            const unsigned rel = (unsigned)(be.x - e0);
            auto p_loads = [&](int j) {
                pi[j] = bld4(srd_P, (unsigned)(di[j] << 10) + v_poff, 0);
                pj[j] = bld4(srd_P, (unsigned)(si[j] << 10) + v_poff + H * 4, 0);
            };
            auto idx_loads = [&]() {
                di = bldi4(srd_dst, v_ioff + rel * 4, 0);
                si = bldi4(srd_src, v_ioff + rel * 4, 0);
            };
#pragma unroll
            for (int j = 0; j < 4; ++j) p_loads(j);
            SYS_STAMP(t, 7);
            idx_loads();
            const int2 be_next = a_blk[clampb(x + 3)];
            auto side = [&](int slot) {
// ... 785 lines not shown
        for (int i = tid; i < H * cols; i += H3_PACK_THREADS) {
            const int col = i % cols;
            float v = Wl[l][(size_t)(i / cols) * ld[l] + (l == 0 ? 0 : c0[l]) + col];
            if (l == 2) v = (float)((double)v - (double)coarse[col]) - cmean[col];
            ss = fmaf(v, v, ss);
            if (l != 0 || enc || (col >= c0[0] && col < c0[0] + H)) wm = fmaxf(wm, fabsf(v));
        }
        red[tid] = ss;
        __syncthreads();
        for (int s = H3_PACK_THREADS / 2; s > 0; s >>= 1) {
            if (tid < s) red[tid] += red[tid + s];
            __syncthreads();
        }
        const float ss_all = red[0];
        __syncthreads();
        red[tid] = wm;
        __syncthreads();
        for (int s = H3_PACK_THREADS / 2; s > 0; s >>= 1) {
            if (tid < s) red[tid] = fmaxf(red[tid], red[tid + s]);
            __syncthreads();
        }
        if (tid == 0) {
            const float wmax = red[0];
            float bs = 0.f, bmax = 0.f;
            for (int o = 0; o < H; ++o) {
                const float bv = l == 2 ? (float)((double)bl[l][o] - (double)coarse[H]) - cmean[H] : bl[l][o];
                bs = fmaf(bv, bv, bs);
                bmax = fmaxf(bmax, fabsf(bv));
            }
            const float g2 = ss_all / (float)H * 0.5f;
            float m = sqrtf(fmaf(enc ? 0.f : 0.5f, bs / (float)H, g2 * m_est * m_est));
            if (!(m > 1.0e-30f) || !(m < 1.0e30f)) m = 1.f;
            auto pow2 = [](float want, bool nearest) {
                if (!(want > 0.f) || !(want < 3.0e38f)) return 1.f;
                int ex;
                const float f = frexpf(want, &ex);
                int sh = (nearest && f >= 0.70710678f) ? ex : ex - 1;
                sh = sh < -100 ? -100 : (sh > 100 ? 100 : sh);
                return ldexpf(1.f, sh);
            };
            float t = pow2(kHmTargetRms / m, true) / U_prev;
            if (wmax > 0.f && wmax < 3.0e38f) {
                if (wmax * t > 8192.0f) t = pow2(8192.0f / wmax, false);
                if (wmax * t < 0.0625f) t = 2.f * pow2(0.0625f / wmax, false);
            }
            tsc[l] = t;
            tsc[3] = m;
            if (enc && bmax > 0.f) capv = fminf(capv, pow2(4096.0f / (U_prev * t * bmax), false));
        }
        __syncthreads();
        m_est = tsc[3];
        U_prev *= tsc[l];
        __syncthreads();
    }
    const float T1 = tsc[0], T2 = T1 * tsc[1], T3 = T2 * tsc[2];
    float* dst = J.dst[job];
    if (tid == 0) { dst[0] = T1; dst[1] = 1.0f / T3; dst[2] = capv; dst[3] = 0.f; }
    float* vec = dst + HW_HEADER_FLOATS;
    for (int i = tid; i < H; i += H3_PACK_THREADS) {
        vec[4 * H + i] = J.b1[job][i] * T1;
        vec[i] = J.b2[job][i] * T2;
        vec[H + i] = ((float)((double)J.b3[job][i] - (double)coarse[H]) - cmean[H]) * T3;
        vec[2 * H + i] = J.gamma[job][i];
        vec[3 * H + i] = J.beta[job][i];
    }
    _Float16* img = reinterpret_cast<_Float16*>(dst + HW_HEADER_FLOATS + HW_VEC_FLOATS);
    for (int idx = tid; idx < 3 * 4 * 8 * 64 * 8; idx += H3_PACK_THREADS) {
        const int j = idx & 7, lane = (idx >> 3) & 63, ks = (idx >> 9) & 7, w = (idx >> 12) & 3, l = idx >> 14;
        const int i = lane & 31, kg = lane >> 5;
        const int kcol = 16 * ks + 8 * (j >> 2) + 4 * kg + (j & 3);
        const bool pad = l == 0 && enc && kcol >= k1;
        const float wv = pad ? 0.f : Wl[l][(size_t)(32 * w + i) * ld[l] + c0[l] + kcol];
        const float v = (l == 2 ? (float)((double)wv - (double)coarse[kcol]) - cmean[kcol] : wv) * tsc[l];
        const _Float16 h = (_Float16)v;
        const _Float16 lo = (_Float16)(v - (float)h);
        const size_t base = ((((size_t)(l * 4 + w) * 8 + ks) * 2) * 64 + lane) * 8 + j;
        img[base] = h;
        img[base + 64 * 8] = lo;
    }
}

__global__ void __launch_bounds__(256) edge_blocks_plan_kernel(const int* __restrict__ in_ptr, int n_nodes, const int* n_per_dev, int n_per_host,
                                                               EdgeBlockHeader* tab, int* gblk, int max_graphs) {
    if (threadIdx.x == 0) edge_blocks_plan(in_ptr, n_nodes, n_per_dev, n_per_host, tab, gblk, max_graphs);
}

__global__ void __launch_bounds__(256) edge_blocks_fill_kernel(const int* __restrict__ in_ptr, const int* __restrict__ dst, int n_nodes,
                                                               EdgeBlockHeader* tab, const int* __restrict__ gblk, int2* blk, int2* seg,
                                                               int* __restrict__ head, int* __restrict__ stitch, int* __restrict__ stitch_list) {
    edge_blocks_fill(in_ptr, dst, n_nodes, tab, gblk, blk, seg, head, stitch, stitch_list, blockIdx.x * blockDim.x + threadIdx.x,
                     gridDim.x * blockDim.x);
}

}

size_t h3_image_floats() { return (size_t)HW_HEADER_FLOATS + HW_VEC_FLOATS + (size_t)HW_IMAGE_HALF8 * 4; }

int pack_h3(const PackH3Job* jobs, int n, hipStream_t s) {
    for (int off = 0; off < n; off += kPackH3Max) {
        PackH3Jobs J{};
        J.n = n - off < kPackH3Max ? n - off : kPackH3Max;
        for (int i = 0; i < J.n; ++i) {
            const PackH3Job& j = jobs[off + i];
            J.W1[i] = j.W1; J.c1[i] = j.W1_col0; J.W2[i] = j.W2; J.W3[i] = j.W3; J.b1[i] = j.b1; J.b2[i] = j.b2; J.b3[i] = j.b3; J.gamma[i] = j.gamma; J.beta[i] = j.beta;
            J.dst[i] = j.dst;
            J.enc_k1[i] = j.enc_k1;
            J.ld1[i] = j.W1_ld;
        }
        hipLaunchKernelGGL(pack_h3_kernel, dim3(J.n), dim3(H3_PACK_THREADS), 0, s, J);
        GM_LAUNCH_CHECK();
    }
    return GM_OK;
}

static size_t max_blocks_of(int64_t n_nodes, int64_t edge_capacity) {
    return (size_t)cdiv(edge_capacity, BE) + 4 * (size_t)n_nodes + 4;
}
size_t edge_groups_max(int64_t n_nodes, int64_t edge_capacity) { return max_blocks_of(n_nodes, edge_capacity) / 4 + 1 + kSinkRows; }

size_t edge_blocks_ints(int64_t n_nodes, int64_t edge_capacity) {
    const size_t nblk = max_blocks_of(n_nodes, edge_capacity);
    return 8 + ((size_t)n_nodes + 2) + 1 + 4 * nblk + (nblk / 4 + 2) + 2 * (size_t)n_nodes;
}

EdgeBlocks carve_edge_blocks(int* base, int64_t n_nodes, int64_t edge_capacity) {
    EdgeBlocks t;
    const size_t nblk = max_blocks_of(n_nodes, edge_capacity);
    t.hdr = reinterpret_cast<EdgeBlockHeader*>(base);
    t.gblk = base + 8;
    int* p = t.gblk + n_nodes + 2;
    p += (reinterpret_cast<uintptr_t>(p) & 4) ? 1 : 0;
    t.blk = reinterpret_cast<int2*>(p);
    t.seg = reinterpret_cast<int2*>(p + 2 * nblk);
    t.head = p + 4 * nblk;
    t.stitch = t.head + nblk / 4 + 2;
    t.stitch_list = t.stitch + n_nodes;
    t.max_blocks = (int64_t)nblk;
    return t;
}

int build_edge_blocks(const int* in_ptr, const int* dst, int64_t n_nodes, const int* n_per_graph_dev, int n_per_graph_host, const EdgeBlocks& t, hipStream_t s) {
    hipLaunchKernelGGL(edge_blocks_plan_kernel, dim3(1), dim3(64), 0, s, in_ptr, (int)n_nodes, n_per_graph_dev, n_per_graph_host,
                       t.hdr, t.gblk, (int)n_nodes + 1);
    int gb = (int)cdiv(t.max_blocks, 256);
    gb = gb < 1 ? 1 : (gb > 1024 ? 1024 : gb);
    hipLaunchKernelGGL(edge_blocks_fill_kernel, dim3(gb), dim3(256), 0, s, in_ptr, dst, (int)n_nodes, t.hdr, t.gblk, t.blk, t.seg, t.head, t.stitch,
                       t.stitch_list);
    GM_LAUNCH_CHECK();
    return GM_OK;
}

bool edge_sys_fits(int64_t n_nodes, int64_t edge_capacity) {
    const uint64_t agg_rows = (uint64_t)n_nodes + edge_groups_max(n_nodes, edge_capacity);
    return (uint64_t)n_nodes * 2 * H * 4 < (1ull << 32) && agg_rows * H * 4 < (1ull << 32);
}

constexpr uint64_t kStreamStoreBytes = 128ull << 20;

template <auto KERNEL, class... Args>
static int launch_sys(size_t lds, ProfState* prof_state, int kind, hipStream_t s, Args... args) {
    static PerDeviceOnce attr_done;
    const int rc_attr = attr_done.run([lds]() -> int {
        GM_HIP_CHECK(hipFuncSetAttribute(reinterpret_cast<const void*>(KERNEL), hipFuncAttributeMaxDynamicSharedMemorySize, (int)lds));
        return GM_OK;
    });
    if (rc_attr != GM_OK) return rc_attr;
    {
        ProfScope prof(prof_state, kind, s);
        hipLaunchKernelGGL(KERNEL, dim3(device_cus()), dim3(SYS_THREADS), lds, s, args...);
    }
    GM_LAUNCH_CHECK();
    return GM_OK;
}
template <auto KERNEL>
using kernel_c = std::integral_constant<decltype(KERNEL), KERNEL>;
int launch_edge_sys(const EdgeArgs& a, const EdgeBlocks& t, int64_t edge_capacity, hipStream_t s) {
    GM_REQUIRE(a.hdr && a.wstream_h3 && a.agg && a.side && !a.eid && !a.eid_out, GM_ERR_INVALID_ARGUMENT, "launch_edge_sys: unsupported argument combination");
    GM_REQUIRE(a.P_prescaled, GM_ERR_INVALID_ARGUMENT, "launch_edge_sys: P must carry the weight scale of this step (HmNodeArgs::p_scale = edge_sys_p_scale(image))");
    const uint64_t agg_bytes = ((uint64_t)(a.side - a.agg) + (uint64_t)(t.max_blocks / 4 + 1) * H) * 4;
    GM_REQUIRE(a.side >= a.agg && agg_bytes < (1ull << 32) && (uint64_t)a.n_nodes_tab * 2 * H * 4 < (1ull << 32), GM_ERR_INVALID_ARGUMENT,
               "launch_edge_sys: P and agg + side buffer must each stay below 4 GiB (edge_sys_fits)");
    const bool stream = (uint64_t)edge_capacity * H * 4 > kStreamStoreBytes;
    auto go = [&](auto kern) {
        return launch_sys<decltype(kern)::value>(SYS_LDS_BYTES, a.prof, PROF_EDGE, s, a.hdr, a.dst, a.src, a.P, a.e_in, a.e_out, a.agg, a.wstream_h3,
                                                 t.blk, t.seg, t.head, t.hdr, (unsigned)(a.side - a.agg), (unsigned)agg_bytes,
                                                 (unsigned)((uint64_t)a.n_nodes_tab * 2 * H * 4), const_cast<int*>(&a.hdr->error_flags), a.eps, a.residual);
    };
    auto pick = [&](auto np_c) {
        constexpr int NP = decltype(np_c)::value;
        if (a.discard_e_out) return stream ? go(kernel_c<sys_edge_kernel<false, true, NP>>{}) : go(kernel_c<sys_edge_kernel<false, false, NP>>{});
        return stream ? go(kernel_c<sys_edge_kernel<true, true, NP>>{}) : go(kernel_c<sys_edge_kernel<true, false, NP>>{});
    };
    return a.precision == kPrecisionF16 ? pick(int_c<NP_F16>{}) : pick(int_c<NP_F32>{});
}

int launch_edge_sys_enc(const EdgeArgs& a, hipStream_t s) {
    GM_REQUIRE(a.hdr && a.wstream_h3 && a.e_in && a.e_out && !a.eid && !a.eid_out && a.k1 == 4, GM_ERR_INVALID_ARGUMENT,
               "launch_edge_sys_enc: unsupported argument combination");
    auto go = [&](auto kern) {
        return launch_sys<decltype(kern)::value>(ENC_LDS_BYTES, a.prof, PROF_ENC, s, a.hdr, a.e_in, a.e_out, a.wstream_h3, const_cast<int*>(&a.hdr->error_flags),
                                                 a.eps, a.zero_pad_rows ? 1 : 0);
    };
    return a.precision == kPrecisionF16 ? go(kernel_c<sys_enc_kernel<NP_F16>>{}) : go(kernel_c<sys_enc_kernel<NP_F32>>{});
}

int launch_node_sys(const NodeSysArgs& a, hipStream_t s) {
    GM_REQUIRE(a.h && a.agg && a.Q && a.h_out && a.image && a.n > 0, GM_ERR_INVALID_ARGUMENT, "launch_node_sys: bad argument");
    auto go = [&](auto kern) {
        return launch_sys<decltype(kern)::value>(NODE_LDS_BYTES, a.prof, PROF_NODE, s, a.h, a.agg, a.Q, a.h_out, a.image, a.n, a.flags, a.eps);
    };
    return a.precision == kPrecisionF16 ? go(kernel_c<sys_node_kernel<NP_F16>>{}) : go(kernel_c<sys_node_kernel<NP_F32>>{});
}

int launch_proj_sys(const ProjSysArgs& a, hipStream_t s) {
    GM_REQUIRE(a.h && a.P && a.Q && a.img_p && a.img_q && a.n > 0, GM_ERR_INVALID_ARGUMENT, "launch_proj_sys: bad argument");
    auto go = [&](auto kern) {
        return launch_sys<decltype(kern)::value>(PROJ_LDS_BYTES, a.prof, PROF_NODE, s, a.h, a.P, a.Q, a.img_p, a.img_q, a.scale_p, a.scale_q, a.n, a.flags);
    };
    return a.precision == kPrecisionF16 ? go(kernel_c<sys_proj_kernel<NP_F16>>{}) : go(kernel_c<sys_proj_kernel<NP_F32>>{});
}

int launch_node_proj_sys(const NodeSysArgs& a, const ProjSysArgs& p, hipStream_t s) {
    GM_REQUIRE(a.h && a.agg && a.Q && a.h_out && a.image && a.n > 0, GM_ERR_INVALID_ARGUMENT, "launch_node_proj_sys: bad argument");
    GM_REQUIRE(p.P && p.img_p && p.img_q, GM_ERR_INVALID_ARGUMENT, "launch_node_proj_sys: bad argument");
    GM_REQUIRE(p.h == a.h_out && p.Q == a.Q && p.n == a.n && p.flags == a.flags, GM_ERR_INVALID_ARGUMENT,
               "launch_node_proj_sys: the projection must read the node MLP's h_out and write its Q, over the same rows");
    GM_REQUIRE(p.precision == a.precision, GM_ERR_INVALID_ARGUMENT, "launch_node_proj_sys: the two halves disagree on the precision");
    auto go = [&](auto kern) {
        return launch_sys<decltype(kern)::value>(NODE_PROJ_LDS_BYTES, a.prof, PROF_NODE, s, a.h, a.h_out, a.agg, p.Q, a.image, p.P, p.img_p, p.img_q,
                                                 p.scale_p, p.scale_q, a.n, a.flags, a.eps);
    };
    return a.precision == kPrecisionF16 ? go(kernel_c<sys_node_proj_kernel<NP_F16>>{}) : go(kernel_c<sys_node_proj_kernel<NP_F32>>{});
}

int launch_agg_stitch(float* agg, const float* side, const EdgeBlocks& t, int64_t n, ProfState* prof_state, hipStream_t s) {
    if (n <= 0) return GM_OK;
    {
        ProfScope prof(prof_state, PROF_NODE, s);
        int64_t gb = cdiv(n * 8, 256 * 4);
        gb = gb < 1 ? 1 : (gb > 2048 ? 2048 : gb);
        hipLaunchKernelGGL(agg_stitch_kernel, dim3((unsigned)gb), dim3(256), 0, s, agg, side, t.stitch, t.stitch_list, t.head, t.hdr, (int)n);
    }
    GM_LAUNCH_CHECK();
    return GM_OK;
}

__global__ void __launch_bounds__(256) edge_pad_rows_kernel(const CsrHeader* hdr, float* e, int row_floats) {
    const size_t base = (size_t)hdr->n_edges * row_floats;
    for (int i = blockIdx.x * blockDim.x + threadIdx.x; i < kEdgePadRows * row_floats; i += gridDim.x * blockDim.x) e[base + i] = 0.f;
}
int zero_edge_pad_rows(const CsrHeader* hdr, float* e, int row_floats, hipStream_t s) {
    hipLaunchKernelGGL(edge_pad_rows_kernel, dim3(4), dim3(256), 0, s, hdr, e, row_floats);
    GM_LAUNCH_CHECK();
    return GM_OK;
}

#ifdef HEDGE_STAMPS
extern "C" int gm_debug_sys_stamps(unsigned long long* out) {
    return hipMemcpyFromSymbol(out, HIP_SYMBOL(g_sys_stamps), sizeof(unsigned long long) * (3 * 32 * 8 + 32)) == hipSuccess ? 0 : -1;
}
#endif

}
```

gnn_manip_amd/csrc/mlp.h:

```cpp
#pragma once
#include "common.h"

namespace gm {

constexpr int kPrecisionF32 = 0;
constexpr int kPrecisionF16 = 1;

struct EdgeArgs {
    const CsrHeader* hdr;
    int n_edges_host;
    const int* dst;
    const int* src;
    const int* eid;
    const int* eid_out;
    const float* P;
    const float* e_in;
    float* e_out;
    float* agg;
    float* side;
    const float* wstream_h3;
    const float* wstream_hm;
    const int* edge_blocks;
    int64_t n_nodes_tab;
    ProfState* prof;
    const float* ln_g;
    const float* ln_b;
    float eps;
    int residual;
    int discard_e_out;
    int P_prescaled;
    int k1;
    int h_valid;
    int zero_pad_rows;
    int precision;
};

#ifdef __HIPCC__
__device__ __forceinline__ float coarse_mean(double mean, float spread) {
    if (!(spread > 0.f)) return (float)mean;
    if (!(spread < 1.0e30f)) return 0.f;
    int ex;
    (void)frexpf(spread, &ex);
    const double g = ldexp(1.0, ex + 1);
    return (float)(rint(mean / g) * g);
}
__device__ __forceinline__ float coarse_mean_of(const float* p, size_t stride, int n) {
    if (n <= 0) return 0.f;
    double a = 0.0;
    for (int r = 0; r < n; ++r) a += (double)p[(size_t)r * stride];
    a /= (double)n;
    float s = 0.f;
    for (int r = 0; r < n; ++r) s = fmaxf(s, fabsf((float)((double)p[(size_t)r * stride] - a)));
    return coarse_mean(a, s);
}
#endif

struct VecJob {
    const float* src;
    size_t dst_off;
    int count;
    int zero_to;
    int center;
};
constexpr int kVecJobsMax = 96;
struct VecJobs {
    int n;
    VecJob job[kVecJobsMax];
};
int launch_vec_batch(const VecJobs& jobs, float* base, hipStream_t s);
int launch_edge(int H, int NL, bool enc, bool sys, const EdgeArgs& a, int64_t edge_capacity, hipStream_t s);

}
```

gnn_manip_amd/csrc/model.h:

```cpp
#pragma once
#include <mutex>
#include <vector>
#include "common.h"
#include "hmlp.h"
#include "mlp.h"
#include "step_rows.h"
#include "train.h"

namespace gm {
enum EdgeKernel : int {
    EK_AUTO = 0,
    EK_SYS = 5,
    EK_HM = 6,
    EK_SYS_ALL = 7,
};

struct MlpSpec { int base, end, in, out; bool normed; };
struct TStream { size_t off = 0; int stages = 0, stages_tail = 0; };
std::vector<MlpSpec> model_mlps(const gm_model_desc& d);

static inline int check_model_for_scene(const gm_model_desc& d, const gm_feature_desc* fd, const char* who) {
    const int F = node_feature_dim(fd);
    GM_REQUIRE(d.node_dim == F, GM_ERR_INVALID_ARGUMENT, "%s: model node_dim=%d but features give %d", who, d.node_dim, F);
    GM_REQUIRE(d.edge_dim == 4 && d.out_dim == 3, GM_ERR_INVALID_ARGUMENT, "%s: needs edge_dim=4, out_dim=3 (3-D scene)", who);
    return GM_OK;
}
}

struct gm_model {
    gm_model_desc d;
    int H, NL, M;
    int Hp = 0;
    int ci = 0, cj = 1, ce = 2;
    int ch = 0, ca = 1;
    std::vector<gm::MlpSpec> mlp;
    const gm::MlpSpec& edge_mlp(int k) const { return mlp[2 + 2 * k]; }
    const gm::MlpSpec& node_mlp(int k) const { return mlp[3 + 2 * k]; }
    float* raw = nullptr;
    std::vector<gm::VecJob> raw_jobs;
    float* vec = nullptr;
    std::vector<gm::VecJob> vec_jobs;
    size_t v_enc_edge, v_enc_node, v_dec;
    std::vector<size_t> v_edge, v_node;
    float* packed_t3 = nullptr;
    std::vector<gm::PackTJob> t_jobs;
    gm::TStream t_enc_edge, t_enc_node, t_dec;
    std::vector<gm::TStream> t_edge, t_node, t_proj;
    float* packed_hm = nullptr;
    std::vector<gm::PackHmJob> hm_jobs;
    gm::PackHmJob* hm_jobs_dev = nullptr;
    float* hm_stats = nullptr;
    size_t hm_enc_edge = 0, hm_enc_node = 0, hm_enc_node_tail = 0;
    std::vector<size_t> hm_edge, hm_node, hm_node_tail, hm_node_q;
    float* packed_h3 = nullptr;
    std::vector<gm::PackH3Job> h3_jobs;
    size_t h3_enc = 0;
    std::vector<size_t> h3_edge, h3_node;
    bool infer_stale = true;
    std::mutex lazy_mu;
    gm::ProfState* prof = nullptr;
    int edge_kernel = gm::EK_AUTO;
    bool node_fusion = true;
    int precision = gm::kPrecisionF32;
    hipEvent_t ready = nullptr;
    hipStream_t ready_stream = nullptr;
};
int ensure_inference_images(const gm_model* m, hipStream_t s);
int weights_ready_on(const gm_model* m, hipStream_t s);
int weights_changed_in_place(gm_model* m, hipStream_t s);
```

gnn_manip_amd/csrc/model.hip:

```cpp
#include <algorithm>
#include <vector>
#include "common.h"
#include "mlp.h"
#include "model.h"
#include "train.h"
#include "hedge.h"
#include "hmlp.h"

using namespace gm;

std::vector<MlpSpec> gm::model_mlps(const gm_model_desc& d) {
    const int H = d.hidden_size, NL = d.num_layers;
    std::vector<MlpSpec> mlp;
    auto add = [&](int in, int out, bool normed) {
        const int base = mlp.empty() ? 0 : mlp.back().end;
        mlp.push_back({base, base + 2 * (NL + 1) + (normed ? 2 : 0), in, out, normed});
    };
    add(d.edge_dim, H, true);
    add(d.node_dim, H, true);
    for (int k = 0; k < d.m_steps; ++k) {
        add(3 * H, H, true);
        add(2 * H, H, true);
    }
    add(H, d.out_dim, false);
// ... 369 lines not shown
    r.sys_enc = sys && attr_sorted && m->d.edge_dim == 4;
    r.sys_edge = sys && cap > 0 && edge_sys_fits(n, cap);
    r.sys_node = r.sys_edge && (m->edge_kernel == EK_SYS_ALL || (n_per_graph > 0 ? n_per_graph : n) >= kSysNodeMinNodes);
    return r;
}

template <class A>
void set_ln(const gm_model* m, A& a, size_t voff) {
    const float* v = m->vec + voff;
    a.ln_g = v + (size_t)(m->NL + 1) * m->Hp; a.ln_b = v + (size_t)(m->NL + 2) * m->Hp; a.eps = m->d.ln_eps;
}

EdgeArgs enc_edge_args(const gm_model* m, const float* edge_attr, const int* eid, const CsrHeader* hdr, int e_host, float* e_out) {
    EdgeArgs a{};
    a.hdr = hdr; a.n_edges_host = e_host; a.eid = eid;
    a.e_in = edge_attr; a.e_out = e_out; a.k1 = m->d.edge_dim;
    a.wstream_hm = m->packed_hm + m->hm_enc_edge;
    a.wstream_h3 = m->packed_h3 ? m->packed_h3 + m->h3_enc : nullptr;
    a.prof = m->prof;
    a.precision = m->precision;
    set_ln(m, a, m->v_enc_edge);
    a.h_valid = m->H;
    return a;
}
EdgeArgs proc_edge_args(const gm_model* m, int k, const CsrWs& c, int64_t n, const int* eid, const float* P, const float* e_in,
                        float* e_out, float* agg, float* side, int residual) {
    EdgeArgs a{};
    a.hdr = c.hdr; a.dst = c.dst; a.src = c.src; a.eid = eid; a.eid_out = eid;
    a.P = P; a.e_in = e_in; a.e_out = e_out; a.agg = agg; a.side = side; a.residual = residual;
    a.wstream_hm = m->packed_hm + m->hm_edge[k];
    a.wstream_h3 = m->packed_h3 ? m->packed_h3 + m->h3_edge[k] : nullptr;
    a.edge_blocks = c.blocks;
    a.n_nodes_tab = n;
    a.prof = m->prof;
    a.precision = m->precision;
    set_ln(m, a, m->v_edge[k]);
    a.h_valid = m->H;
    return a;
}

HmNodeArgs node_args(const gm_model* m, int64_t n, const float* x_in, int* flags) {
    HmNodeArgs a{};
    a.n_nodes = (int)n; a.x_in = x_in; a.nl = m->NL; a.h_valid = m->H; a.flags = flags; a.prof = m->prof;
    a.precision = m->precision;
    return a;
}
HmNodeArgs enc_node_args(const gm_model* m, int64_t n, const float* x, float* h_out, int* flags) {
    HmNodeArgs a = node_args(m, n, x, flags);
    a.k1 = m->d.node_dim; a.h_out = h_out;
    a.w = m->packed_hm + m->hm_enc_node;
    set_ln(m, a, m->v_enc_node);
    return a;
}
HmNodeArgs proc_node_args(const gm_model* m, int k, const CsrWs& c, int64_t n, int64_t cap, const float* h, const float* agg,
                          const float* side, float* h_out, int residual) {
    HmNodeArgs a = node_args(m, n, h, &c.hdr->error_flags);
    a.agg = agg; a.h_out = h_out; a.residual = residual;
    a.w = m->packed_hm + m->hm_node[k];
    set_ln(m, a, m->v_node[k]);
    const EdgeBlocks t = carve_edge_blocks(c.blocks, n, cap);
    a.stitch = t.stitch; a.head = t.head; a.side = side; a.tab = t.hdr;
    return a;
}
void set_tail(const gm_model* m, HmNodeArgs& a, int next, float* P, float* out, bool p_scaled) {
    a.w_tail = m->packed_hm + (next == 0 ? m->hm_enc_node_tail : m->hm_node_tail[next - 1]);
    if (next < m->M) {
        a.tail = 1;
        a.P_out = P;
        a.p_scale = p_scaled ? edge_sys_p_scale(m->packed_h3 + m->h3_edge[next]) : nullptr;
    } else {
        a.tail = 2;
        a.dec_out = out;
        a.out_dim = m->d.out_dim;
    }
}
HmNodeArgs tail_args(const gm_model* m, int next, int64_t n, const float* h, float* P, float* out, int* flags) {
    HmNodeArgs a = node_args(m, n, h, flags);
    set_tail(m, a, next, P, out, false);
    return a;
}

int epd_forward_impl(const gm_model* m, const float* nodes, int64_t n, const float* edge_attr, int attr_is_csr_order,
                     const void* csr_ws, int64_t cap, float* out, void* fwd_ws, size_t fwd_ws_bytes, void* stream, bool agg_cleared,
                     int64_t n_per_graph) {
    gm::DevGuard dev_guard(out);
    GM_REQUIRE(m && csr_ws && fwd_ws, GM_ERR_INVALID_ARGUMENT, "gm_epd_forward: null pointer");
    GM_REQUIRE(n >= 0 && cap >= 0 && n < ((int64_t)1 << 31) && cap < ((int64_t)1 << 31), GM_ERR_INVALID_ARGUMENT, "gm_epd_forward: sizes out of range");
    if (n == 0) return GM_OK;
    GM_REQUIRE(nodes && out && (edge_attr || cap == 0), GM_ERR_INVALID_ARGUMENT, "gm_epd_forward: null tensor");
    const int H = m->Hp, NL = m->NL, M = m->M;
    FwdWs f = carve_fwd(fwd_ws, H, n, cap, cap);
    GM_REQUIRE(fwd_ws_bytes >= f.bytes, GM_ERR_WORKSPACE, "gm_epd_forward: workspace %zu < %zu", fwd_ws_bytes, f.bytes);
    CsrWs c = carve_csr(const_cast<void*>(csr_ws), n, cap);
    int* flags = &c.hdr->error_flags;
    hipStream_t s = (hipStream_t)stream;
    int rc = ensure_inference_images(m, s);
    if (rc != GM_OK) return rc;
    const Route route = route_forward(m, Entry::Fused, n, n_per_graph, cap, attr_is_csr_order != 0);
    {
        EdgeArgs ee = enc_edge_args(m, edge_attr, attr_is_csr_order ? nullptr : c.eid, c.hdr, 0, f.e);
        ee.zero_pad_rows = 1;
        rc = launch_edge(H, NL, true, route.sys_enc, ee, cap, s);
    }
    if (rc != GM_OK) return rc;
    if (cap > 0 && !route.sys_enc) {
        ProfScope prof(m->prof, PROF_REST, s);
        rc = zero_edge_pad_rows(c.hdr, f.e, H, s);
        if (rc != GM_OK) return rc;
    }
    auto proj_args = [&](int k) {
        ProjSysArgs pa{};
        pa.h = f.h; pa.P = f.P; pa.Q = f.Q; pa.n = (int)n; pa.flags = flags; pa.prof = m->prof;
        pa.precision = m->precision;
        pa.img_p = m->packed_hm + (k == 0 ? m->hm_enc_node_tail : m->hm_node_tail[k - 1]);
        pa.img_q = m->packed_hm + m->hm_node_q[k];
        pa.scale_p = edge_sys_p_scale(m->packed_h3 + m->h3_edge[k]);
        pa.scale_q = edge_sys_p_scale(m->packed_h3 + m->h3_node[k]);
        return pa;
    };
    {
        HmNodeArgs na = enc_node_args(m, n, nodes, f.h, flags);
        if (!route.sys_node) set_tail(m, na, 0, f.P, out, route.sys_edge);
        rc = launch_node_hm(H, 0, na, s);
    }
    if (rc == GM_OK && route.sys_node) rc = launch_proj_sys(proj_args(0), s);
    if (rc != GM_OK) return rc;
    if (!agg_cleared) {
        ProfScope prof(m->prof, PROF_REST, s);
        GM_HIP_CHECK(hipMemsetAsync(f.agg, 0, (size_t)n * H * sizeof(float), s));
    }
    for (int k = 0; k < M; ++k) {
        EdgeArgs ea = proc_edge_args(m, k, c, n, nullptr, f.P, f.e, f.e, f.agg, f.side, 1);
        ea.discard_e_out = k + 1 == M;
        ea.P_prescaled = route.sys_edge;
        rc = launch_edge(H, NL, false, route.sys_edge, ea, cap, s);
        if (rc != GM_OK) return rc;
        if (route.sys_node) {
            rc = launch_agg_stitch(f.agg, f.side, carve_edge_blocks(c.blocks, n, cap), n, m->prof, s);
            NodeSysArgs ns{};
            ns.h = f.h; ns.agg = f.agg; ns.Q = f.Q; ns.h_out = f.h; ns.image = m->packed_h3 + m->h3_node[k];
            ns.n = (int)n; ns.flags = flags; ns.eps = m->d.ln_eps; ns.prof = m->prof;
            ns.precision = m->precision;
            const bool fused = k + 1 < M && m->node_fusion;
            if (rc == GM_OK) rc = fused ? launch_node_proj_sys(ns, proj_args(k + 1), s) : launch_node_sys(ns, s);
            if (rc == GM_OK && k + 1 < M && !fused) rc = launch_proj_sys(proj_args(k + 1), s);
            if (rc == GM_OK && k + 1 == M) rc = launch_node_hm(H, 2, tail_args(m, M, n, f.h, f.P, out, flags), s);
        } else {
            HmNodeArgs a = proc_node_args(m, k, c, n, cap, f.h, f.agg, f.side, f.h, 1);
            set_tail(m, a, k + 1, f.P, out, route.sys_edge);
            rc = launch_node_hm(H, 1, a, s);
        }
        if (rc != GM_OK) return rc;
    }
    return GM_OK;
}
}

extern "C" {

int gm_epd_forward(const gm_model* m, const float* nodes, int64_t n, const float* edge_attr, int attr_is_csr_order,
                   const void* csr_ws, int64_t cap, float* out, void* fwd_ws, size_t fwd_ws_bytes, void* stream) {
    return epd_forward_impl(m, nodes, n, edge_attr, attr_is_csr_order, csr_ws, cap, out, fwd_ws, fwd_ws_bytes, stream, false, n);
}

int gm_graph_independent_forward(const gm_model* m, const float* x, int64_t n, const float* edge_attr, int64_t e,
                                 float* h_out, float* e_out, void* stream) {
    gm::DevGuard dev_guard(x ? (const void*)x : (const void*)edge_attr);
    GM_REQUIRE(m, GM_ERR_INVALID_ARGUMENT, "gm_graph_independent_forward: null model");
    GM_REQUIRE(n >= 0 && e >= 0 && n < ((int64_t)1 << 31) && e < ((int64_t)1 << 31), GM_ERR_INVALID_ARGUMENT, "sizes out of range");
    GM_REQUIRE((n == 0 || (x && h_out)) && (e == 0 || (edge_attr && e_out)), GM_ERR_INVALID_ARGUMENT, "gm_graph_independent_forward: null tensor");
    hipStream_t s = (hipStream_t)stream;
    int rc = ensure_inference_images(m, s);
    if (rc != GM_OK) return rc;
    const Route route = route_forward(m, Entry::Independent, n, n, e, true);
    rc = launch_edge(m->Hp, m->NL, true, route.sys_enc, enc_edge_args(m, edge_attr, nullptr, nullptr, (int)e, e_out), e, s);
    if (rc != GM_OK || n == 0) return rc;
    return launch_node_hm(m->Hp, 0, enc_node_args(m, n, x, h_out, nullptr), s);
}

int gm_interaction_network_forward(const gm_model* m, int k, const float* h, int64_t n, const float* e,
                                   const void* csr_ws, int64_t cap, float* h_out, float* e_out, void* fwd_ws,
                                   size_t fwd_ws_bytes, void* stream) {
    gm::DevGuard dev_guard(h);
    GM_REQUIRE(m && csr_ws && fwd_ws, GM_ERR_INVALID_ARGUMENT, "gm_interaction_network_forward: null pointer");
    GM_REQUIRE(k >= 0 && k < m->M, GM_ERR_INVALID_ARGUMENT, "gm_interaction_network_forward: block %d out of range", k);
    GM_REQUIRE(n >= 0 && cap >= 0 && n < ((int64_t)1 << 31) && cap < ((int64_t)1 << 31), GM_ERR_INVALID_ARGUMENT, "sizes out of range");
    if (n == 0) return GM_OK;
    GM_REQUIRE(h && h_out && (cap == 0 || (e && e_out)), GM_ERR_INVALID_ARGUMENT, "gm_interaction_network_forward: null tensor");
    const int H = m->Hp, NL = m->NL;
    FwdWs f = carve_fwd(fwd_ws, H, n, 0, cap);
    GM_REQUIRE(fwd_ws_bytes >= f.bytes, GM_ERR_WORKSPACE, "gm_interaction_network_forward: workspace %zu < %zu", fwd_ws_bytes, f.bytes);
    CsrWs c = carve_csr(const_cast<void*>(csr_ws), n, cap);
    hipStream_t s = (hipStream_t)stream;
    int rc = ensure_inference_images(m, s);
    if (rc != GM_OK) return rc;
    const Route route = route_forward(m, Entry::Block, n, n, cap, false);
    rc = launch_node_hm(H, 2, tail_args(m, k, n, h, f.P, nullptr, &c.hdr->error_flags), s);
    if (rc != GM_OK) return rc;
    GM_HIP_CHECK(hipMemsetAsync(f.agg, 0, (size_t)n * H * sizeof(float), s));
    rc = launch_edge(H, NL, false, route.sys_edge, proc_edge_args(m, k, c, n, c.eid, f.P, e, e_out, f.agg, f.side, 0), cap, s);
    if (rc != GM_OK) return rc;
    return launch_node_hm(H, 1, proc_node_args(m, k, c, n, cap, h, f.agg, f.side, h_out, 0), s);
}

}

namespace {
struct RolloutWs {
    void *graph, *csr, *fwd;
    float *x, *edge_attr, *pred;
    size_t graph_bytes, csr_bytes, fwd_bytes, bytes;
};
RolloutWs carve_rollout(void* ws, const gm_model_desc* d, int64_t n, int K) {
    RolloutWs r;
    const int64_t cap = n * K;
    r.graph_bytes = gm_graph_workspace_bytes(n, K);
    r.csr_bytes = gm_csr_workspace_bytes(n, cap);
    r.fwd_bytes = gm_forward_workspace_bytes(d, n, cap);
    Carver c(ws);
    r.graph = c.take<char>(r.graph_bytes);
    r.csr = c.take<char>(r.csr_bytes);
    r.fwd = c.take<char>(r.fwd_bytes);
    r.x = c.take<float>((size_t)n * 32);
    r.edge_attr = c.take<float>((size_t)cap * 4);
    r.pred = c.take<float>((size_t)n * 4);
    r.bytes = c.used();
    return r;
}
struct RenumberWs {
    float* state[2];
    int* total[2];
    int *perm, *rank;
    size_t bytes;
};
RenumberWs carve_renumber(void* ws, const gm_feature_desc* fd, int64_t n) {
    RenumberWs w;
    Carver c(ws);
    const size_t st = (size_t)fd->k_steps * n * fd->data_dim;
    w.state[0] = c.take<float>(st);
    w.state[1] = c.take<float>(st);
    w.total[0] = c.take<int>(n);
    w.total[1] = c.take<int>(n);
    w.perm = c.take<int>(n);
    w.rank = c.take<int>(n);
    w.bytes = c.used();
    return w;
}
}

extern "C" {

int gm_model_set_edge_kernel(gm_model* m, int choice) {
    GM_REQUIRE(m, GM_ERR_INVALID_ARGUMENT, "gm_model_set_edge_kernel: null model");
    GM_REQUIRE(choice >= EK_AUTO && choice <= EK_SYS_ALL, GM_ERR_INVALID_ARGUMENT, "gm_model_set_edge_kernel: choice %d out of range", choice);
    GM_REQUIRE(choice == EK_AUTO || choice >= EK_SYS, GM_ERR_UNSUPPORTED,
               "gm_model_set_edge_kernel: choices 1..4 (the round-1 fp32 / bf16 x 6 kernels) were removed from the library (round 5)");
    GM_REQUIRE((choice != EK_SYS && choice != EK_SYS_ALL) || m->packed_h3, GM_ERR_UNSUPPORTED, "gm_model_set_edge_kernel: the systolic kernel is for hidden_size 128, num_layers 2");
    m->edge_kernel = choice;
    return GM_OK;
}

int gm_model_set_node_fusion(gm_model* m, int on) {
    GM_REQUIRE(m, GM_ERR_INVALID_ARGUMENT, "gm_model_set_node_fusion: null model");
    m->node_fusion = on != 0;
    return GM_OK;
}

int gm_model_set_precision(gm_model* m, int precision) {
    GM_REQUIRE(m, GM_ERR_INVALID_ARGUMENT, "gm_model_set_precision: null model");
    GM_REQUIRE(precision == GM_PRECISION_F32 || precision == GM_PRECISION_F16, GM_ERR_INVALID_ARGUMENT,
               "gm_model_set_precision: precision %d (GM_PRECISION_F32 = 0, GM_PRECISION_F16 = 1)", precision);
    m->precision = precision;
    return GM_OK;
}

int gm_model_profile(gm_model* m, int kind_mask) {
    GM_REQUIRE(m, GM_ERR_INVALID_ARGUMENT, "gm_model_profile: null model");
    if (!m->prof) {
        if (!kind_mask) return GM_OK;
        m->prof = new ProfState();
    }
    for (int k = 0; k < PROF_KINDS; ++k)
        if (((kind_mask & ~m->prof->mask) >> k) & 1) m->prof->count[k] = m->prof->dropped[k] = 0;
    m->prof->mask = kind_mask;
    return GM_OK;
}

int gm_model_profile_query(const gm_model* m, int kind, int64_t* launches, double* total_ms) {
    GM_REQUIRE(m && kind >= 0 && kind < PROF_KINDS && launches && total_ms, GM_ERR_INVALID_ARGUMENT, "gm_model_profile_query: bad argument");
    *launches = 0;
    *total_ms = 0.0;
    const ProfState* p = m->prof;
    if (!p) return GM_OK;
    *launches = p->dropped[kind] ? -(int64_t)(p->count[kind] + p->dropped[kind]) : p->count[kind];
    for (int i = 0; i < p->count[kind]; ++i) {
        GM_HIP_CHECK(hipEventSynchronize(p->stop[kind][i]));
        float ms = 0.f;
        GM_HIP_CHECK(hipEventElapsedTime(&ms, p->start[kind][i], p->stop[kind][i]));
        *total_ms += ms;
    }
    return GM_OK;
}

size_t gm_rollout_workspace_bytes(const gm_model_desc* desc, int64_t n, int K) {
    if (!desc || n < 0 || K < 1) return 0;
    return carve_rollout(nullptr, desc, n, K).bytes;
}

}

namespace {
int rollout_step_impl(const gm_model* m, float* obs, int64_t n, const gm_feature_desc* fd, int K, const int32_t* rigid_rank,
                      const float* rigid_target, float* pred_acc_out, const gm::RecordedDrive* rec, void* ws, size_t ws_bytes,
                      void* stream) {
    gm::DevGuard dev_guard(obs);
    GM_REQUIRE(m && obs && fd && ws, GM_ERR_INVALID_ARGUMENT, "gm_rollout_step: null pointer");
    int rc = gm::check_model_for_scene(m->d, fd, "gm_rollout_step");
    if (rc != GM_OK) return rc;
    GM_REQUIRE(n < ((int64_t)1 << 31) / (K > 0 ? K : 1), GM_ERR_UNSUPPORTED, "gm_rollout_step: n*max_neighbours overflows int32");
    RolloutWs r = carve_rollout(ws, &m->d, n, K);
    GM_REQUIRE(ws_bytes >= r.bytes, GM_ERR_WORKSPACE, "gm_rollout_step: workspace %zu < %zu", ws_bytes, r.bytes);
    if (n == 0) return GM_OK;
    const int64_t cap = n * K;
    hipStream_t hs = (hipStream_t)stream;
    {
        StepClear clr;
        rc = graph_clear_jobs(clr, carve_graph(r.graph, n, K), n);
        if (rc == GM_OK) rc = csr_clear_jobs(clr, carve_csr(r.csr, n, cap), n, m->d.flow);
        FwdWs f = carve_fwd(r.fwd, m->Hp, n, cap, cap);
        if (rc == GM_OK) rc = clr.add(reinterpret_cast<int*>(f.agg), (long long)n * m->Hp, 0);
        if (rc != GM_OK) return rc;
        ProfScope prof(m->prof, PROF_REST, hs);
        rc = gm::rollout_pre_features(obs, n, fd, rigid_rank, rigid_target, r.x, hs, &clr, rec);
    }
    if (rc != GM_OK) return rc;
    const float* last_pos = obs + (size_t)(fd->k_steps - 1) * n * fd->data_dim + fd->cart_col;
    {
        ProfScope prof(m->prof, PROF_GRAPH, hs);
        rc = gm::radius_graph_build_fused(last_pos, fd->data_dim, n, gm::graph_nodes(fd, n), fd->conn_r, K,
                                          r.graph, r.graph_bytes, r.csr, r.csr_bytes, m->d.flow, hs);
    }
    if (rc != GM_OK) return rc;
    {
        ProfScope prof(m->prof, PROF_REST, hs);
        rc = gm::csr_from_graph_fused(r.graph, n, K, r.csr, r.csr_bytes, last_pos, fd->data_dim, (float)fd->conn_r, r.edge_attr,
                                      m->d.flow, hs);
    }
    if (rc != GM_OK) return rc;
    rc = epd_forward_impl(m, r.x, n, r.edge_attr, 1, r.csr, cap, r.pred, r.fwd, r.fwd_bytes, stream, true, gm::graph_nodes(fd, n));
    if (rc != GM_OK) return rc;
    ProfScope prof(m->prof, PROF_REST, hs);
    return gm::rollout_integrate_post(obs, n, fd, r.pred, rigid_rank, rigid_target, pred_acc_out, hs, rec);
}
}

extern "C" {

int gm_rollout_step(const gm_model* m, float* obs, int64_t n, const gm_feature_desc* fd, int K, const int32_t* rigid_rank,
                    const float* rigid_target, float* pred_acc_out, void* ws, size_t ws_bytes, void* stream) {
    return rollout_step_impl(m, obs, n, fd, K, rigid_rank, rigid_target, pred_acc_out, nullptr, ws, ws_bytes, stream);
}

size_t gm_rollout_renumber_workspace_bytes(const gm_feature_desc* fd, int64_t n) {
    if (!fd || n < 0 || fd->k_steps < 1 || fd->data_dim < 1) return 0;
    return carve_renumber(nullptr, fd, n).bytes;
}

}

namespace {
struct RolloutDrive {
    const float* targets = nullptr;
    int64_t n_targets = 0, n_rigid = 0;
    const float* frames = nullptr;
    float* record_pred = nullptr;
};
int rollout_loop(const char* who, const gm_model* m, float* obs, int64_t n, const gm_feature_desc* fd, int K, const int32_t* rigid_rank,
                 const RolloutDrive& drive, int64_t steps, float* record_last, int64_t renumber_every, void* renumber_ws,
                 size_t renumber_ws_bytes, void* ws, size_t ws_bytes, void* stream) {
    hipStream_t hs = (hipStream_t)stream;
    const float* rigid_targets = drive.targets;
    const int64_t n_targets = drive.n_targets, n_rigid = drive.n_rigid;
    const size_t frame = (size_t)n * fd->data_dim;
    const bool renum = renumber_every > 0 && n > 0 && steps > 0;
    RenumberWs rw{};
    RolloutWs r{};
    if (renum) {
        GM_REQUIRE(renumber_ws, GM_ERR_INVALID_ARGUMENT, "%s: renumber_every > 0 needs renumber_ws (gm_rollout_renumber_workspace_bytes)", who);
        rw = carve_renumber(renumber_ws, fd, n);
        GM_REQUIRE(renumber_ws_bytes >= rw.bytes, GM_ERR_WORKSPACE, "%s: renumber workspace %zu < %zu", who, renumber_ws_bytes, rw.bytes);
        GM_REQUIRE(n < ((int64_t)1 << 31) / (K > 0 ? K : 1), GM_ERR_UNSUPPORTED, "%s: n*max_neighbours overflows int32", who);
        r = carve_rollout(ws, &m->d, n, K);
        GM_REQUIRE(ws_bytes >= r.bytes, GM_ERR_WORKSPACE, "%s: workspace %zu < %zu", who, ws_bytes, r.bytes);
    }
    float* state = obs;
    const int* rank = rigid_rank;
    const int* total = nullptr;
    int flip = 0;
    for (int64_t i = 0; i < steps; ++i) {
        if (renum && i % renumber_every == 0) {
            const float* last_pos = state + (size_t)(fd->k_steps - 1) * frame + fd->cart_col;
            int rc = gm::cell_order(last_pos, fd->data_dim, n, gm::graph_nodes(fd, n), fd->conn_r, K, r.graph,
                                    r.graph_bytes, rw.perm, hs);
            if (rc != GM_OK) return rc;
            rc = gm::renumber_gather(state, rw.state[flip], fd->k_steps, n, fd->data_dim, rw.perm, r.graph, total, rw.total[flip],
                                     rigid_rank, rigid_rank ? rw.rank : nullptr, hs);
            if (rc != GM_OK) return rc;
            state = rw.state[flip];
            total = rw.total[flip];
            rank = rigid_rank ? rw.rank : nullptr;
            flip ^= 1;
        }
        if (drive.frames) {
            const gm::RecordedDrive rec{drive.frames + (size_t)i * frame, total, record_last ? record_last + (size_t)i * frame : nullptr,
                                        drive.record_pred ? drive.record_pred + (size_t)i * n * 3 : nullptr};
            int rc = rollout_step_impl(m, state, n, fd, K, rank, nullptr, nullptr, &rec, ws, ws_bytes, stream);
            if (rc != GM_OK) return rc;
            continue;
        }
        float* last = state + (size_t)(fd->k_steps - 1) * frame;
        const float* target = i < n_targets ? rigid_targets + (size_t)i * n_rigid * 3 : nullptr;
        if (record_last) {
            int rc = fd->control_col >= 0 ? gm_state_pre(state, n, fd, rank, target, stream) : GM_OK;
            if (rc != GM_OK) return rc;
            if (total) rc = gm::renumber_scatter(last, record_last + (size_t)i * frame, 1, n, fd->data_dim, total, hs);
            else GM_HIP_CHECK(hipMemcpyAsync(record_last + (size_t)i * frame, last, frame * sizeof(float), hipMemcpyDeviceToDevice, hs));
            if (rc != GM_OK) return rc;
        }
        int rc = gm_rollout_step(m, state, n, fd, K, rank, target, nullptr, ws, ws_bytes, stream);
        if (rc != GM_OK) return rc;
    }
    if (total) return gm::renumber_scatter(state, obs, fd->k_steps, n, fd->data_dim, total, hs);
    return GM_OK;
}
}

extern "C" {

int gm_rollout(const gm_model* m, float* obs, int64_t n, const gm_feature_desc* fd, int K, const int32_t* rigid_rank,
               const float* rigid_targets, int64_t n_targets, int64_t n_rigid, int64_t steps, float* record_last,
               int64_t renumber_every, void* renumber_ws, size_t renumber_ws_bytes, void* ws, size_t ws_bytes, void* stream) {
    gm::DevGuard dev_guard(obs);
    GM_REQUIRE(m && obs && fd && ws, GM_ERR_INVALID_ARGUMENT, "gm_rollout: null pointer");
    GM_REQUIRE(steps >= 0 && n_targets >= 0 && n_rigid >= 0 && renumber_every >= 0, GM_ERR_INVALID_ARGUMENT, "gm_rollout: negative count");
    GM_REQUIRE(rigid_targets || n_targets == 0 || n_rigid == 0, GM_ERR_INVALID_ARGUMENT, "gm_rollout: n_targets > 0 without rigid_targets");
    GM_REQUIRE(!rigid_targets || rigid_rank, GM_ERR_INVALID_ARGUMENT, "gm_rollout: rigid_targets need rigid_rank");
    RolloutDrive drive;
    drive.targets = rigid_targets; drive.n_targets = n_targets; drive.n_rigid = n_rigid;
    return rollout_loop("gm_rollout", m, obs, n, fd, K, rigid_rank, drive, steps, record_last, renumber_every, renumber_ws, renumber_ws_bytes,
                        ws, ws_bytes, stream);
}

int gm_rollout_recorded(const gm_model* m, float* obs, int64_t n, const gm_feature_desc* fd, int K, const int32_t* rigid_rank,
                        const float* frames, int64_t steps, float* record_last, float* record_pred, int64_t renumber_every,
                        void* renumber_ws, size_t renumber_ws_bytes, void* ws, size_t ws_bytes, void* stream) {
    gm::DevGuard dev_guard(obs);
    GM_REQUIRE(m && obs && fd && ws, GM_ERR_INVALID_ARGUMENT, "gm_rollout_recorded: null pointer");
    GM_REQUIRE(steps >= 0 && renumber_every >= 0, GM_ERR_INVALID_ARGUMENT, "gm_rollout_recorded: negative count");
    GM_REQUIRE(frames || steps == 0 || n == 0, GM_ERR_INVALID_ARGUMENT, "gm_rollout_recorded: steps > 0 without frames");
    if (steps == 0 || n <= 0) return GM_OK;
    RolloutDrive drive;
    drive.frames = frames; drive.record_pred = record_pred;
    return rollout_loop("gm_rollout_recorded", m, obs, n, fd, K, rigid_rank, drive, steps, record_last, renumber_every, renumber_ws,
                        renumber_ws_bytes, ws, ws_bytes, stream);
}

int gm_rollout_status(const void* ws, const gm_model_desc* desc, int64_t n, int K, int64_t* n_edges_host, void* stream) {
    gm::DevGuard dev_guard(ws);
    GM_REQUIRE(ws && desc && n_edges_host, GM_ERR_INVALID_ARGUMENT, "gm_rollout_status: null pointer");
    RolloutWs r = carve_rollout(const_cast<void*>(ws), desc, n, K);
    int rc = gm_radius_graph_num_edges(r.graph, n_edges_host, stream);
    if (rc != GM_OK) return rc;
    int64_t e2 = 0;
    return gm_csr_num_edges(r.csr, &e2, stream);
}

}
```

gnn_manip_amd/rollout.py:

```python
import ctypes as C
import os

import torch
from torch.autograd.function import once_differentiable

from ._lib import ModelDesc, check, current_stream, lib, ptr
from .epd_gnn import _device_arrays, _pointers, _zeroed_like
from .graph import _NodeFeaturesFunction, _need_cuda, _node_features, _ws, get_connectivity, get_edges_displacement, make_feature_desc


def get_position_from_prediction(stats, cartesian_idx, pred_acc, obs_seq, _desc=None):
    _need_cuda(pred_acc, "pred_acc")
    obs = obs_seq.contiguous().float()
    pred = pred_acc.contiguous().float()
    k, n, dd = obs.shape
    if _desc is None:
        one = [1.0, 1.0, 1.0]
        full = dict(velocity_mean=[0.0] * 3, velocity_std=one)
        full.update(stats)
        _desc = make_feature_desc(1.0, full, dict(lower_bounds=[0.0] * 3, upper_bounds=one), cartesian_idx,
                                  [0], None, k, dd)
    if torch.is_grad_enabled() and (pred.requires_grad or obs.requires_grad):
        return _IntegrateFunction.apply(pred, obs, _desc)
    return _integrate(pred, obs, _desc)
# ... 33 lines not shown
        if records is not None:
            records[t].copy_(obs[-2])
    engine.status()
    return obs, traj


class _RolloutFunction(torch.autograd.Function):

    @staticmethod
    def forward(ctx, engine, obs0, trajectory, steps, edges):
        windows = []
        obs, traj = _roll_forward(engine, obs0, trajectory, steps, lambda t, window: windows.append(window.clone()))
        ctx.engine, ctx.windows, ctx.traj, ctx.edges = engine, windows, traj, edges
        ctx.scene = (engine.rigid_rank, engine.rigid_rows, engine.n_rigid)
        return obs

    @staticmethod
    @once_differentiable
    def backward(ctx, d_window):
        eng, traj = ctx.engine, ctx.traj
        eng.rigid_rank, eng.rigid_rows, eng.n_rigid = ctx.scene
        need_traj = traj is not None and ctx.needs_input_grad[2]
        d_traj = torch.zeros_like(traj) if need_traj else None
        edges = [None] * len(ctx.windows)
        d_window = d_window.contiguous().float()
        for t in range(len(ctx.windows) - 1, -1, -1):
            with torch.enable_grad():
                w = ctx.windows[t].requires_grad_(True)
                pose = None if traj is None else traj[t].clone().requires_grad_(need_traj)
                nxt, _, ei = eng.differentiable_step(w, pose, inputs_only=True)
            grads = torch.autograd.grad(nxt, [w, pose] if need_traj else [w], grad_outputs=d_window)
            d_window = grads[0]
            if need_traj:
                d_traj[t] = grads[1]
            ctx.windows[t] = None
            edges[t] = ei if ctx.edges is not None else None
            del nxt, w, pose, grads
        if ctx.edges is not None:
            ctx.edges[:] = edges
        return None, (d_window if ctx.needs_input_grad[1] else None), d_traj, None, None


class _RolloutTrainFunction(torch.autograd.Function):

    @staticmethod
    def forward(ctx, engine, obs0, trajectory, steps, record, model, *tensors):
        windows = torch.empty((steps,) + tuple(obs0.shape), dtype=torch.float32, device=obs0.device)
        records = torch.empty((steps,) + tuple(obs0.shape[1:]), dtype=torch.float32, device=obs0.device) if record else None
        obs, traj = _roll_forward(engine, obs0, trajectory, steps, lambda t, window: windows[t].copy_(window), records)
        ctx.engine, ctx.windows, ctx.traj, ctx.steps, ctx.model, ctx.record = engine, windows, traj, steps, model, record
        ctx.scene = (engine.rigid_rank, engine.n_rigid)
        ctx.save_for_backward(*tensors)
        ctx.set_materialize_grads(False)
        return (obs, records) if record else obs

    @staticmethod
    @once_differentiable
    def backward(ctx, d_final, d_records=None):
        eng = ctx.engine
        if d_final is None:
            d_final = torch.zeros((eng.k, eng.n, eng.data_dim), dtype=torch.float32, device=eng.device)
        need_traj = ctx.traj is not None and ctx.needs_input_grad[2]
        tensors = ctx.saved_tensors
        model = grads = None
        if ctx.model is not None:
            h, mdesc = ctx.model
            model = (h,) + _device_arrays(tensors, eng.device) + (mdesc,)
            if any(ctx.needs_input_grad[6:]):
                grads = _zeroed_like(model[1])
        d_obs0, d_traj = eng._sweep_backward(ctx.windows, ctx.traj, ctx.steps, d_final.contiguous().float(), ctx.scene, need_traj,
                                             d_records=None if d_records is None else d_records.contiguous().float(), model=model,
                                             grads=grads)
        ctx.windows = None
        d_tensors = tuple(g if ctx.needs_input_grad[6 + i] else None for i, g in enumerate(grads)) if grads else (None,) * len(tensors)
        return (None, (d_obs0 if ctx.needs_input_grad[1] else None), d_traj, None, None, None) + d_tensors


class RolloutEngine:

    RENUMBER_MIN_NODES = 20000
    RENUMBER_EVERY = 64

    def __init__(self, model, graph_attr, n_nodes, k_steps=6, data_dim=None, max_neighbours=20, device="cuda:0",
                 candidates=1, renumber="auto"):
        self.model = model
        self.graph_attr = graph_attr
        self.candidates = int(candidates)
        self.n_per = int(n_nodes)
        self.n = int(n_nodes) * self.candidates
        self.k = int(k_steps)
        self.device = torch.device(device)
        self.max_neighbours = int(max_neighbours)
        if data_dim is None:
            data_dim = (graph_attr.control_idx[-1] + 1) if graph_attr.control_idx is not None else graph_attr.cartesian_idx[-1] + 1
        self.data_dim = int(data_dim)
        self.fdesc = make_feature_desc(graph_attr.conn_r, graph_attr.stats, graph_attr.bounds, graph_attr.cartesian_idx,
                                       graph_attr.material_idx, graph_attr.control_idx, self.k, self.data_dim)
        self.fdesc.nodes_per_graph = self.n_per if self.candidates > 1 else 0
        self.mdesc = ModelDesc(*model.model_desc())
        L = lib()
        self.ws = _ws(L.gm_rollout_workspace_bytes(C.byref(self.mdesc), self.n, self.max_neighbours), self.device)
        self.rigid_rank = None
        self.rigid_rows = None
        self.n_rigid = 0
        if renumber == "auto" and os.environ.get("GM_RENUMBER") in ("0", "1"):
            renumber = os.environ["GM_RENUMBER"] == "1"
        self.renumber = (self.n_per >= self.RENUMBER_MIN_NODES) if renumber == "auto" else bool(renumber)
        self._renumber_ws = None

    def _rank_rigid(self, obs):
        rank = torch.empty(self.n, dtype=torch.int32, device=self.device)
        cnt = torch.zeros(1, dtype=torch.int32, device=self.device)
        check(lib().gm_rigid_rank(ptr(obs), self.n, C.byref(self.fdesc), ptr(rank), ptr(cnt), current_stream()))
        return rank, cnt

    def set_scene(self, obs):
        _need_cuda(obs, "obs")
        assert obs.shape == (self.k, self.n, self.data_dim) and obs.dtype == torch.float32 and obs.is_contiguous()
        self.rigid_rank, cnt = self._rank_rigid(obs)
        self.n_rigid = int(cnt.item())
        self.rigid_rows = torch.nonzero(self.rigid_rank >= 0).flatten()
        return self.n_rigid

    def _check_tensor(self, t, name, shape, converted=False, min_rows=0):
        fits = isinstance(t, torch.Tensor) and t.device == self.device and (converted or (t.dtype == torch.float32 and t.is_contiguous()))
        if fits and isinstance(shape, int):
            fits = t.numel() == shape
        elif fits and t.shape != shape:
            fits = (t.dim() == len(shape) and all(isinstance(want, str) or want == got for want, got in zip(shape, t.shape))
                    and t.shape[0] >= min_rows)
        if not fits:
            want = f"with {shape} elements" if isinstance(shape, int) else "[" + ", ".join(str(d) for d in shape) + "]"
            given = f"{tuple(t.shape)} {t.dtype} on {t.device}" if isinstance(t, torch.Tensor) else type(t).__name__
            raise ValueError(f"{name} must be {'a tensor' if converted else 'contiguous float32'} {want} on {self.device}, got {given}")

    def _check_state(self, obs, rigid_target, pred_out, use_rigid):
        self._check_tensor(obs, "obs", (self.k, self.n, self.data_dim))
        if use_rigid and self.rigid_rank is None:
            raise RuntimeError("RolloutEngine.set_scene(obs) must be called before step()")
        if rigid_target is not None:
            if not use_rigid:
                raise ValueError("rigid_target needs use_rigid=True")
            self._check_tensor(rigid_target, "rigid_target", (self.n_rigid, 3))
        if pred_out is not None:
            self._check_tensor(pred_out, "pred_out", self.n * 3)

    def step(self, obs, rigid_target=None, pred_out=None, use_rigid=True):
        self._check_state(obs, rigid_target, pred_out, use_rigid)
        handle = self.model.device_handle(self.device)
        rr = self.rigid_rank if use_rigid else None
        check(lib().gm_rollout_step(handle, ptr(obs), self.n, C.byref(self.fdesc), self.max_neighbours, ptr(rr),
                                    ptr(rigid_target), ptr(pred_out), ptr(self.ws), self.ws.numel(), current_stream()))

    def differentiable_step(self, obs, rigid_target=None, inputs_only=False):
        self._check_state(obs, rigid_target, None, True)
        ga = self.graph_attr
        c0 = ga.cartesian_idx[0]
        rows = self.rigid_rows
        last = obs[-1]
        if ga.control_idx is not None:
            u0 = ga.control_idx[0]
            cur = last[rows, c0:c0 + 3]
            last = last.clone()
            last[rows, u0:u0 + 3] = cur if rigid_target is None else rigid_target - cur
        obs_pre = torch.cat((obs[:-1], last.unsqueeze(0)))
        if torch.is_grad_enabled() and obs_pre.requires_grad:
            nodes = _NodeFeaturesFunction.apply(obs_pre, self.fdesc)
        else:
            nodes = _node_features(obs_pre, self.fdesc)
        pos = obs_pre[-1][:, c0:c0 + 3]
        senders, receivers = get_connectivity(pos.detach(), ga.conn_r, self.max_neighbours,
                                              self.n_per if self.candidates > 1 else None)
        edge_attr = get_edges_displacement(pos, senders, receivers, ga.conn_r)
        edge_index = torch.stack((senders, receivers))
        pred = (self.model.forward_inputs_only if inputs_only else self.model.forward)(nodes, edge_attr, edge_index)
        next_pos = get_position_from_prediction(ga.stats, ga.cartesian_idx, pred, obs_pre, _desc=self.fdesc)
        new_last = obs_pre[-1].clone()
        new_last[:, c0:c0 + 3] = next_pos
        keep = obs_pre[-1][rows]
        if rigid_target is not None:
            keep = keep.clone()
            keep[:, c0:c0 + 3] = rigid_target
        new_last[rows] = keep
        return torch.cat((obs_pre[1:], new_last.unsqueeze(0))), pred, edge_index

    def _training_model(self):
        with torch.no_grad():
            desc_t, handle, tensors, key = self.model._training_spec([p.detach() for p in self.model.parameters()])
        h = handle.get(desc_t, tensors, self.device, key)
        return (h,) + _device_arrays(tensors, self.device) + (ModelDesc(*desc_t),)

# ... 4 lines not shown
        if getattr(self, "_bwd_ws", None) is None or self._bwd_ws.numel() < need:
            self._bwd_ws = _ws(need, self.device)
        return self._bwd_ws

    def _check_param_grads(self, grads, tensors):
        if len(grads) != len(tensors):
            raise ValueError(f"grads must be {len(tensors)} tensors shaped like the training model's, got {len(grads)}")
        for g, t in zip(grads, tensors):
            self._check_tensor(g, "each of grads", t.shape)
        return _pointers(grads)

    def step_backward(self, obs_before, rigid_target, d_obs_after, return_edge_count=False, d_record=None, grads=None):
        self._check_state(obs_before, rigid_target, None, True)
        self._check_tensor(d_obs_after, "d_obs_after", (self.k, self.n, self.data_dim))
        if d_record is not None:
            self._check_tensor(d_record, "d_record", (self.n, self.data_dim))
        h, tensors, t_arr, mdesc = self._training_model()
        g_arr = None if grads is None else self._check_param_grads(grads, tensors)
        ws = self._backward_ws(mdesc)
        d_obs = torch.empty_like(obs_before)
        d_tgt = None if rigid_target is None else torch.empty_like(rigid_target)
        e = C.c_int64(0)
        check(lib().gm_rollout_step_backward_train(h, t_arr, len(tensors), ptr(obs_before), self.n, C.byref(self.fdesc), self.max_neighbours,
                                                   ptr(self.rigid_rank), ptr(rigid_target), ptr(d_obs_after), ptr(d_record), g_arr,
                                                   ptr(d_obs), ptr(d_tgt), C.byref(e), ptr(ws), ws.numel(), current_stream()))
        return (d_obs, d_tgt, int(e.value)) if return_edge_count else (d_obs, d_tgt)

    def _sweep_backward(self, windows, traj, steps, d_final, scene, need_traj, d_records=None, model=None, grads=None):
        rank, n_rigid = scene
        self._check_tensor(d_final, "d_final", (self.k, self.n, self.data_dim))
        if traj is not None:
            self._check_tensor(traj, "trajectory", ("T", n_rigid, 3))
        self._check_tensor(windows, "windows", (steps, self.k, self.n, self.data_dim))
        if d_records is not None:
            self._check_tensor(d_records, "d_records", (steps, self.n, self.data_dim))
        h, tensors, t_arr, mdesc = self._training_model() if model is None else model
        g_arr = None if grads is None else self._check_param_grads(grads, tensors)
        ws = self._backward_ws(mdesc)
        d_obs0 = torch.empty_like(d_final)
        d_traj = torch.empty_like(traj) if need_traj else None
        n_targets = 0 if traj is None else int(traj.shape[0])
        check(lib().gm_rollout_backward_train(h, t_arr, len(tensors), ptr(windows), self.n, C.byref(self.fdesc), self.max_neighbours,
                                              ptr(rank), ptr(traj), n_targets, n_rigid, steps, ptr(d_final), ptr(d_records), g_arr,
                                              ptr(d_obs0), ptr(d_traj), ptr(ws), ws.numel(), current_stream()))
        return d_obs0, d_traj

    def differentiable_rollout(self, obs0, trajectory=None, horizon=None, return_edges=False, sweep="autograd", record=False,
                               params=False):
        if sweep not in ("autograd", "library"):
            raise ValueError(f"sweep must be 'autograd' or 'library', got {sweep!r}")
        if sweep == "library" and return_edges:
            raise ValueError("sweep='library' hands out no edge lists: return_edges needs sweep='autograd'")
        if sweep != "library" and (record or params):
            raise ValueError("record=True / params=True need sweep='library' (the autograd sweep returns the final state alone, "
                             "with the parameters as constants)")
        steps = int(horizon) if horizon is not None else (int(trajectory.shape[0]) if trajectory is not None else 0)
        self._check_state(obs0, None, None, False)
        if trajectory is not None:
            self._check_tensor(trajectory, "trajectory", (f"T >= {steps}", "N_rigid", 3), converted=True, min_rows=steps)
        if sweep == "library":
            model, tensors = None, ()
            if params:
                desc_t, handle, tensors, key = self.model._training_spec(list(self.model.parameters()))
                model = (handle.get(desc_t, tensors, self.device, key), ModelDesc(*desc_t))
            return _RolloutTrainFunction.apply(self, obs0, trajectory, steps, bool(record), model, *tensors)
        edges = [] if return_edges else None
        out = _RolloutFunction.apply(self, obs0, trajectory, steps, edges)
        return (out, edges) if return_edges else out

    def status(self):
        e = C.c_int64(0)
        check(lib().gm_rollout_status(ptr(self.ws), C.byref(self.mdesc), self.n, self.max_neighbours, C.byref(e), current_stream()))
        return int(e.value)

    def run(self, obs, trajectory=None, steps=None, record=False):
        T = 0 if trajectory is None else int(trajectory.shape[0])
        steps = T if steps is None else int(steps)
        self._check_state(obs, None, None, True)
        if trajectory is not None:
            self._check_tensor(trajectory, "trajectory", ("T", self.n_rigid, 3))
        recs = torch.empty((steps, self.n, self.data_dim), dtype=torch.float32, device=self.device) if record else None
        handle = self.model.device_handle(self.device)
        every, rws = self._renumbering(steps)
        check(lib().gm_rollout(handle, ptr(obs), self.n, C.byref(self.fdesc), self.max_neighbours, ptr(self.rigid_rank),
                           ptr(trajectory), T, self.n_rigid, steps, ptr(recs), every, ptr(rws), 0 if rws is None else rws.numel(),
                           ptr(self.ws), self.ws.numel(), current_stream()))
        return recs

    def _renumbering(self, steps):
        if not (self.renumber and self.n > 0 and steps > 0):
            return 0, None
        if self._renumber_ws is None:
            self._renumber_ws = _ws(lib().gm_rollout_renumber_workspace_bytes(C.byref(self.fdesc), self.n), self.device)
        return self.RENUMBER_EVERY, self._renumber_ws

    def run_recorded(self, obs, frames, steps=None, record=False, record_pred=False):
        self._check_state(obs, None, None, True)
        self._check_tensor(frames, "frames", ("T", self.n, self.data_dim))
        steps = int(frames.shape[0]) if steps is None else int(steps)
        if not 0 <= steps <= frames.shape[0]:
            raise ValueError(f"steps must be between 0 and the {frames.shape[0]} frames given, got {steps}")
        recs = torch.empty((steps, self.n, self.data_dim), dtype=torch.float32, device=self.device) if record else None
        preds = torch.empty((steps, self.n, 3), dtype=torch.float32, device=self.device) if record_pred else None
        handle = self.model.device_handle(self.device)
        every, rws = self._renumbering(steps)
        check(lib().gm_rollout_recorded(handle, ptr(obs), self.n, C.byref(self.fdesc), self.max_neighbours, ptr(self.rigid_rank),
                                        ptr(frames), steps, ptr(recs), ptr(preds), every, ptr(rws), 0 if rws is None else rws.numel(),
                                        ptr(self.ws), self.ws.numel(), current_stream()))
        return recs, preds

    def rollout_candidates(self, obs0, trajectories, horizon=None):
        b, k, n = self.candidates, self.k, self.n_per
        assert trajectories.shape[0] == b
        obs = obs0.unsqueeze(1).repeat(1, b, 1, 1).reshape(k, b * n, self.data_dim).contiguous()
        self.set_scene(obs)
        steps = horizon if horizon is not None else trajectories.shape[1]
        traj_t = trajectories.permute(1, 0, 2, 3).reshape(trajectories.shape[1], -1, 3).contiguous().float()
        self.run(obs, traj_t, steps)
        self.status()
        return obs.reshape(k, b, n, self.data_dim).permute(1, 0, 2, 3).contiguous()

    def rollout(self, obs0, trajectory=None, horizon=None, record=False):
        obs = obs0.clone().contiguous()
        self.set_scene(obs)
        steps = horizon if horizon is not None else (trajectory.shape[0] if trajectory is not None else 0)
        traj = None if trajectory is None else trajectory.contiguous().float()
        recs = self.run(obs, traj, steps, record=record)
        self.status()
        if record:
            return obs, recs
        return obs


def get_rigid_body_trajectory_from_diff(trajectory, horizon, ty_init, rigid_particles):
    from .planner import get_rigid_body_trajectory
    return get_rigid_body_trajectory(trajectory[:, 0], trajectory[:, 1], horizon, ty_init, rigid_particles)


def extract_groundtruth(dataset, nof_steps, nof_particles=None, data_dim=None):
    return torch.stack([dataset[i][0][-1] for i in range(nof_steps)]).float()


def compute_rollout(dataset, model, args):
    import numpy as np
    obs0, _ = dataset[0]
    k, n, dd = obs0.shape
    dev = obs0.device
    nof_steps = dataset.time_steps if args.cma_traj is not None else dataset.time_steps - args.k_steps
    eng = RolloutEngine(model, dataset.graph_attr, n, k_steps=k, data_dim=dd, max_neighbours=20, device=dev,
                        renumber="auto" if args.cma_traj is not None else False)
    obs = obs0.clone().contiguous()
    eng.set_scene(obs)
    rigid = obs[0, :, dataset.material_id] == 1
    c0 = dataset.cartesian_idx[0]
    with torch.no_grad():
        if args.cma_traj is not None:
            npy_trajectory = np.load(args.cma_traj) if isinstance(args.cma_traj, str) else np.asarray(args.cma_traj)
            rigid_pos = obs[-1, rigid, c0:c0 + 3].contiguous()
            trajectory = get_rigid_body_trajectory_from_diff(npy_trajectory, nof_steps, [0.5, 0.5, 0.4], rigid_pos)
            _, recs = eng.rollout(obs, trajectory, horizon=nof_steps, record=True)
            return recs.cpu().numpy().astype(np.float64)
        groundtruth = extract_groundtruth(dataset, nof_steps).contiguous()
        recs, _ = eng.run_recorded(obs, groundtruth, nof_steps, record=True)
        eng.status()
        return recs.cpu().numpy().astype(np.float64)

# ... 88 lines not shown
```

include/gnn_manip_hip.h:

```cpp
#ifndef GNN_MANIP_HIP_H
#define GNN_MANIP_HIP_H

#include <stddef.h>
#include <stdint.h>

#ifdef __cplusplus
extern "C" {
#endif

typedef enum gm_status {
    GM_OK = 0,
    GM_ERR_INVALID_ARGUMENT = -1,
    GM_ERR_UNSUPPORTED = -2,
    GM_ERR_HIP = -3,
    GM_ERR_WORKSPACE = -4,
    GM_ERR_DATA = -5
} gm_status;

typedef struct gm_model gm_model;

const char* gm_last_error(void);
int gm_abi_version(void);

size_t gm_graph_workspace_bytes(int64_t n_nodes, int max_neighbours);
// ... 23 lines not shown
int gm_csr_from_graph_flow(const void* graph_ws, int64_t n_nodes, int max_neighbours, int flow,
                           void* csr_ws, size_t csr_ws_bytes, void* stream);
int gm_csr_from_edge_index_flow(const int64_t* edge_index, int64_t n_nodes, int64_t n_edges, int flow,
                                void* csr_ws, size_t csr_ws_bytes, void* stream);
int gm_csr_num_edges(const void* csr_ws, int64_t* n_edges_host, void* stream);
int gm_csr_header_status(const int32_t* header_host , int64_t* n_edges_host );

int gm_edge_features(const float* pos, int64_t pos_stride, const int64_t* senders,
                     const int64_t* receivers, int64_t n_edges, float conn_r, float* out ,
                     void* stream);
int gm_edge_features_csr(const float* pos, int64_t pos_stride, const void* csr_ws, int64_t n_nodes,
                         int64_t edge_capacity, float conn_r, float* out , void* stream);

typedef struct gm_feature_desc {
    double conn_r;
    int32_t k_steps;
    int32_t data_dim;
    int32_t cart_col;
    int32_t material_col;
    int32_t control_col;
    int32_t nodes_per_graph;
    float vel_mean[3], vel_std[3];
    float acc_mean[3], acc_std[3];
    float lower_bounds[3], upper_bounds[3];
} gm_feature_desc;

int gm_node_features(const float* obs, int64_t n_nodes, const gm_feature_desc* desc,
                     float* out , void* stream);

int gm_integrate(const float* pred_acc , const float* obs, int64_t n_nodes,
                 const gm_feature_desc* desc, float* next_pos , void* stream);
int gm_rigid_rank(const float* obs, int64_t n_nodes, const gm_feature_desc* desc, int32_t* rigid_rank,
                  int32_t* n_rigid_dev, void* stream);
int gm_state_pre(float* obs, int64_t n_nodes, const gm_feature_desc* desc, const int32_t* rigid_rank,
                 const float* rigid_target ,
                 void* stream);
int gm_state_post(float* obs, int64_t n_nodes, const gm_feature_desc* desc, const float* next_pos,
                  const int32_t* rigid_rank, const float* rigid_target , void* stream);
int gm_rigid_transform(const float* rigid_init , int64_t n_rigid, const float* rot_cs_ty
                       ,
                       int64_t n_steps, const float ty_init[3], float* out , void* stream);

int gm_rigid_transform_backward(const float* rigid_init , int64_t n_rigid, const float* rot_cs_ty ,
                                int64_t n_steps, const float ty_init[3], const float* d_out ,
                                float* d_rot_cs_ty , void* stream);

size_t gm_edge_features_backward_workspace_bytes(int64_t n_nodes, int64_t n_edges);
int gm_edge_features_backward(const float* pos, int64_t pos_stride, const int64_t* senders, const int64_t* receivers,
                              int64_t n_nodes, int64_t n_edges, float conn_r, const float* d_out ,
                              float* d_pos , void* ws, size_t ws_bytes, void* stream);
int gm_node_features_backward(const float* obs, int64_t n_nodes, const gm_feature_desc* desc,
                              const float* d_out , float* d_obs , void* stream);
int gm_integrate_backward(const float* d_next_pos , int64_t n_nodes, const gm_feature_desc* desc,
                          float* d_pred , float* d_obs , void* stream);

int gm_state_pre_backward(const float* d_obs_after, int64_t n_nodes, const gm_feature_desc* desc, const int32_t* rigid_rank,
                          int has_target, float* d_obs_before, float* d_rigid_target , void* stream);
int gm_state_post_backward(const float* d_obs_after, int64_t n_nodes, const gm_feature_desc* desc,
                           const int32_t* rigid_rank , int has_target, float* d_obs_before, float* d_next_pos ,
                           float* d_rigid_target , void* stream);

typedef struct gm_model_desc {
    int32_t node_dim, edge_dim, out_dim;
    int32_t hidden_size;
    int32_t num_layers;
    int32_t m_steps;
    float ln_eps;
    int32_t flow;
    int32_t col_i, col_j, col_e;
    int32_t node_agg_first;
} gm_model_desc;

int gm_padded_hidden_size(int hidden_size);

int gm_model_num_tensors(const gm_model_desc* desc);
int gm_model_create(const gm_model_desc* desc, const float* const* tensors, int n_tensors,
                    int tensors_on_device, void* stream, gm_model** out);
int gm_model_update(gm_model* m, const float* const* tensors, int n_tensors, int tensors_on_device,
                    void* stream);
void gm_model_destroy(gm_model* m);

int gm_model_set_edge_kernel(gm_model* m, int choice);
int gm_model_set_node_fusion(gm_model* m, int on);
enum { GM_PRECISION_F32 = 0, GM_PRECISION_F16 = 1 };
int gm_model_set_precision(gm_model* m, int precision);

size_t gm_forward_workspace_bytes(const gm_model_desc* desc, int64_t n_nodes, int64_t edge_capacity);
size_t gm_block_workspace_bytes(const gm_model_desc* desc, int64_t n_nodes, int64_t edge_capacity);

int gm_epd_forward(const gm_model* m, const float* nodes , int64_t n_nodes,
                   const float* edge_attr , int edge_attr_is_csr_order,
                   const void* csr_ws, int64_t edge_capacity, float* out ,
                   void* fwd_ws, size_t fwd_ws_bytes, void* stream);

int gm_graph_independent_forward(const gm_model* m, const float* x, int64_t n_nodes, const float* edge_attr,
                                 int64_t n_edges, float* h_out, float* e_out, void* stream);
int gm_interaction_network_forward(const gm_model* m, int block, const float* h, int64_t n_nodes,
                                   const float* e, const void* csr_ws, int64_t edge_capacity,
                                   float* h_out, float* e_out, void* fwd_ws, size_t fwd_ws_bytes,
                                   void* stream);

size_t gm_train_tape_bytes(const gm_model_desc* desc, int64_t n_nodes, int64_t n_edges);
size_t gm_train_backward_workspace_bytes(const gm_model_desc* desc, int64_t n_nodes, int64_t n_edges);
int gm_epd_forward_train(const gm_model* m, const float* nodes, int64_t n_nodes, const float* edge_attr,
                         const int64_t* edge_index, int64_t n_edges, float* out, void* tape,
                         size_t tape_bytes, void* stream);
int gm_epd_backward(const gm_model* m, const float* const* tensors, int n_tensors, const float* nodes,
                    const float* edge_attr, int64_t n_nodes, int64_t n_edges, const float* grad_out,
                    float* const* grads, void* tape, size_t tape_bytes, void* ws, size_t ws_bytes,
                    void* stream);

size_t gm_train_backward_inputs_workspace_bytes(const gm_model_desc* desc, int64_t n_nodes, int64_t n_edges);
int gm_epd_backward_inputs(const gm_model* m, const float* const* tensors, int n_tensors, const float* nodes,
                           const float* edge_attr, int64_t n_nodes, int64_t n_edges, const float* grad_out,
                           float* const* grads, float* d_nodes ,
                           float* d_edge_attr , void* tape,
                           size_t tape_bytes, void* ws, size_t ws_bytes, void* stream);

int gm_epd_backward_inputs_only(const gm_model* m, const float* const* tensors, int n_tensors, const float* nodes,
                                const float* edge_attr, int64_t n_nodes, int64_t n_edges, const float* grad_out,
                                float* d_nodes ,
                                float* d_edge_attr , void* tape,
                                size_t tape_bytes, void* ws, size_t ws_bytes, void* stream);

size_t gm_block_tape_bytes(const gm_model_desc* desc, int interaction_network, int64_t n_nodes, int64_t n_edges);
size_t gm_block_backward_workspace_bytes(const gm_model_desc* desc, int64_t n_nodes, int64_t n_edges);
int gm_graph_independent_forward_train(const gm_model* m, const float* x, int64_t n_nodes, const float* edge_attr,
                                       int64_t n_edges, float* h_out, float* e_out, void* tape, size_t tape_bytes,
                                       void* stream);
int gm_graph_independent_backward(const gm_model* m, const float* const* tensors, int n_tensors, const float* x,
                                  const float* edge_attr, int64_t n_nodes, int64_t n_edges, const float* dh,
                                  const float* de, float* dx ,
                                  float* dedge_attr , float* const* grads, void* tape,
                                  size_t tape_bytes, void* ws, size_t ws_bytes, void* stream);
int gm_interaction_network_forward_train(const gm_model* m, int block, const float* h, int64_t n_nodes,
                                         const float* e, const int64_t* edge_index, int64_t n_edges, float* h_out,
                                         float* e_out, void* tape, size_t tape_bytes, void* stream);
int gm_interaction_network_backward(const gm_model* m, int block, const float* const* tensors, int n_tensors,
                                    const float* h, const float* e, int64_t n_nodes, int64_t n_edges,
                                    const float* dh_out, const float* de_out, float* dh_in, float* de_in,
                                    float* const* grads, void* tape, size_t tape_bytes, void* ws, size_t ws_bytes,
                                    void* stream);

size_t gm_sinkhorn_workspace_bytes(int64_t n, int64_t m);
int gm_sinkhorn_divergence(const float* x, int64_t n, const float* y, int64_t m, float blur, float scaling,
                           float* loss_device, void* ws, size_t ws_bytes, void* stream);
size_t gm_sinkhorn_batched_workspace_bytes(int64_t batch, int64_t n, int64_t m);
int gm_sinkhorn_divergence_batched(const float* x, int64_t batch, int64_t n, const float* y, int64_t m, int y_shared,
                                   float blur, float scaling, float diameter, float* loss_device , void* ws,
                                   size_t ws_bytes, void* stream);
size_t gm_sinkhorn_batched_backward_workspace_bytes(int64_t batch, int64_t n, int64_t m, int y_shared);
int gm_sinkhorn_divergence_batched_backward(const float* x, int64_t batch, int64_t n, const float* y, int64_t m, int y_shared,
                                            float blur, float scaling, const float* grad_loss ,
                                            float* dx ,
                                            float* dy , const void* fwd_ws,
                                            size_t fwd_ws_bytes, void* bwd_ws, size_t bwd_ws_bytes, void* stream);

size_t gm_rollout_workspace_bytes(const gm_model_desc* desc, int64_t n_nodes, int max_neighbours);
int gm_rollout_step(const gm_model* m, float* obs , int64_t n_nodes,
                    const gm_feature_desc* fdesc, int max_neighbours, const int32_t* rigid_rank,
                    const float* rigid_target , float* pred_acc_out ,
                    void* rollout_ws, size_t rollout_ws_bytes, void* stream);
size_t gm_rollout_renumber_workspace_bytes(const gm_feature_desc* fdesc, int64_t n_nodes);
int gm_rollout(const gm_model* m, float* obs , int64_t n_nodes, const gm_feature_desc* fdesc,
               int max_neighbours, const int32_t* rigid_rank, const float* rigid_targets, int64_t n_targets,
               int64_t n_rigid, int64_t steps, float* record_last, int64_t renumber_every, void* renumber_ws,
// ... 128 lines not shown
```

Measured before the change: 131.9 rollout steps/s.

## Skip last message-passing step and decoder work for scripted rigid particles

Result: no change. 132.3 rollout steps/s, median of 6 (+0.3%).

```diff
diff --git a/gnn_manip_amd/_lib.py b/gnn_manip_amd/_lib.py
--- a/gnn_manip_amd/_lib.py
+++ b/gnn_manip_amd/_lib.py
@@ -146,6 +146,7 @@
     "gm_model_profile": (_i32, [_vp, _i32]),
     "gm_model_set_edge_kernel": (_i32, [_vp, _i32]),
     "gm_model_set_node_fusion": (_i32, [_vp, _i32]),
+    "gm_model_set_prune_rigid": (_i32, [_vp, _i32]),
     "gm_model_set_precision": (_i32, [_vp, _i32]),
     "gm_model_profile_query": (_i32, [_vp, _i32, C.POINTER(_i64), C.POINTER(_f64)]),
 }
diff --git a/gnn_manip_amd/csrc/blocks_dev.h b/gnn_manip_amd/csrc/blocks_dev.h
--- a/gnn_manip_amd/csrc/blocks_dev.h
+++ b/gnn_manip_amd/csrc/blocks_dev.h
@@ -9,7 +9,7 @@
 
 #if defined(__HIPCC__)
 __device__ inline void edge_blocks_plan(const int* __restrict__ in_ptr, int n_nodes, const int* n_per_dev, int n_per_host,
-                                        EdgeBlockHeader* tab, int* gblk, int max_graphs) {
+                                        EdgeBlockHeader* tab, int* gblk, int max_graphs, int n_live) {
     int n_per = n_per_dev ? *n_per_dev : n_per_host;
     if (n_per <= 0) n_per = n_nodes > 0 ? n_nodes : 1;
     int G = (n_nodes + n_per - 1) / n_per;
@@ -26,6 +26,8 @@
     tab->n_graphs = G;
     tab->n_per_graph = n_per;
     tab->n_stitch = 0;
+    const int live = (G == 1 && n_live >= 0 && n_live < n_nodes) ? (in_ptr[n_live] + 4 * kBlockEdges - 1) / (4 * kBlockEdges) : pb / 4;
+    tab->n_groups_live = live < pb / 4 ? live : pb / 4;
 }
 
 __device__ inline void edge_blocks_fill(const int* __restrict__ in_ptr, const int* __restrict__ dst, int n_nodes, EdgeBlockHeader* tab,
diff --git a/gnn_manip_amd/csrc/common.h b/gnn_manip_amd/csrc/common.h
--- a/gnn_manip_amd/csrc/common.h
+++ b/gnn_manip_amd/csrc/common.h
@@ -178,7 +178,7 @@
 int csr_from_edge_index(const int64_t* ei, int64_t n, int64_t e, int flow, void* csr_ws, size_t csr_ws_bytes, bool with_blocks, hipStream_t stream);
 
 int cell_order(const float* pos, int64_t pos_stride, int64_t n, int64_t n_per, double conn_r, int K, void* graph_ws, size_t graph_ws_bytes,
-               int* perm, hipStream_t s);
+               int* perm, const int* rank, hipStream_t s);
 
 size_t scan_state_ints(int64_t n_max);
 struct ScanJob {
@@ -260,6 +260,6 @@
 int radius_graph_build_fused(const float* pos, int64_t pos_stride, int64_t n, int64_t n_per, double conn_r, int K, void* graph_ws,
                              size_t graph_ws_bytes, void* csr_ws, size_t csr_ws_bytes, int flow, hipStream_t s);
 int csr_from_graph_fused(const void* graph_ws, int64_t n, int K, void* csr_ws, size_t csr_ws_bytes, const float* pos, int64_t pos_stride,
-                         float conn_r, float* edge_attr, int flow, hipStream_t s);
+                         float conn_r, float* edge_attr, int flow, int64_t n_live, hipStream_t s);
 
 }
diff --git a/gnn_manip_amd/csrc/features.hip b/gnn_manip_amd/csrc/features.hip
--- a/gnn_manip_amd/csrc/features.hip
+++ b/gnn_manip_amd/csrc/features.hip
@@ -277,7 +277,7 @@
     const int64_t id = (int64_t)blockIdx.x * blockDim.x + threadIdx.x;
     if (id >= (int64_t)k * n) return;
     const int64_t t = id / n, j = id - t * n;
-    const int64_t src = ghdr->order_skip ? j : (int64_t)perm[j];
+    const int64_t src = ghdr && ghdr->order_skip ? j : (int64_t)perm[j];
     const float* a = in + (t * n + src) * D;
     float* b = out + (t * n + j) * D;
     for (int d = 0; d < D; ++d) b[d] = a[d];
diff --git a/gnn_manip_amd/csrc/graph.hip b/gnn_manip_amd/csrc/graph.hip
--- a/gnn_manip_amd/csrc/graph.hip
+++ b/gnn_manip_amd/csrc/graph.hip
@@ -405,6 +405,23 @@
     int before = 0;
     for (int q = lo; q < hi; ++q) before += __float_as_int(sorted[q].w) < i ? 1 : 0;
     perm[lo + before] = i;
+}
+
+__global__ void __launch_bounds__(256) class_flag_kernel(const int* __restrict__ order, const GraphHeader* __restrict__ hdr,
+                                                          const int* __restrict__ rank, int64_t n, int* __restrict__ live) {
+    const int64_t p = (int64_t)blockIdx.x * blockDim.x + threadIdx.x;
+    if (p > n) return;
+    live[p] = p < n && rank[hdr->order_skip ? (int)p : order[p]] < 0 ? 1 : 0;
+}
+__global__ void __launch_bounds__(256) class_place_kernel(const int* __restrict__ order, const GraphHeader* __restrict__ hdr,
+                                                           const int* __restrict__ live, const int* __restrict__ before, int64_t n,
+                                                           int64_t n_per, int* __restrict__ perm) {
+    const int64_t p = (int64_t)blockIdx.x * blockDim.x + threadIdx.x;
+    if (p >= n) return;
+    const int i = hdr->order_skip ? (int)p : order[p];
+    const int64_t g0 = p - p % n_per, g1 = g0 + n_per < n ? g0 + n_per : n;
+    const int n_live = before[g1] - before[g0], b = before[p] - before[g0];
+    perm[g0 + (live[p] ? b : n_live + ((int)(p - g0) - b))] = i;
 }
 
 constexpr int NB_LPQ = 16;
@@ -621,10 +638,10 @@
                                                           const int* __restrict__ in_ptr, const int* __restrict__ slot,
                                                           int64_t cap, int flow, int* __restrict__ dst, int* __restrict__ src,
                                                           int* __restrict__ eid, CsrHeader* hdr, const int* n_per_dev,
-                                                          EdgeBlockHeader* tab, int* gblk) {
+                                                          EdgeBlockHeader* tab, int* gblk, int n_live) {
     int64_t id = (int64_t)blockIdx.x * blockDim.x + threadIdx.x, i;
     int s;
-    if (id == 0 && tab) edge_blocks_plan(in_ptr, (int)n, n_per_dev, 0, tab, gblk, (int)n + 1);
+    if (id == 0 && tab) edge_blocks_plan(in_ptr, (int)n, n_per_dev, 0, tab, gblk, (int)n + 1, n_live);
     if (!decode_slot(id, n, K, cnt, i, s)) return;
     const int d = flow ? (int)i : nbr[id];
     int p = in_ptr[d] + slot[id];
@@ -766,7 +783,7 @@
 }
 
 int cell_order(const float* pos, int64_t pos_stride, int64_t n, int64_t n_per, double conn_r, int K, void* graph_ws, size_t graph_ws_bytes,
-               int* perm, hipStream_t s) {
+               int* perm, const int* rank, hipStream_t s) {
     GM_REQUIRE(pos && graph_ws && perm && n > 0 && pos_stride >= 3 && conn_r > 0.0, GM_ERR_INVALID_ARGUMENT, "cell_order: bad argument");
     GraphWs g = carve_graph(graph_ws, n, K);
     GM_REQUIRE(graph_ws_bytes >= g.bytes, GM_ERR_WORKSPACE, "cell_order: workspace %zu < %zu", graph_ws_bytes, g.bytes);
@@ -775,7 +792,16 @@
     if (rc == GM_OK) rc = launch_step_clear(clr, s);
     if (rc == GM_OK) rc = grid_phase(pos, pos_stride, n, n_per, conn_r, g, s);
     if (rc != GM_OK) return rc;
-    hipLaunchKernelGGL(cell_order_kernel, dim3((unsigned)cdiv(n, 256)), dim3(256), 0, s, g.sorted, g.cell_of, g.cell_start, g.hdr, n, perm);
+    int* order = rank ? g.nbr : perm;
+    hipLaunchKernelGGL(cell_order_kernel, dim3((unsigned)cdiv(n, 256)), dim3(256), 0, s, g.sorted, g.cell_of, g.cell_start, g.hdr, n, order);
+    GM_LAUNCH_CHECK();
+    if (!rank) return GM_OK;
+    hipLaunchKernelGGL(class_flag_kernel, dim3((unsigned)cdiv(n + 1, 256)), dim3(256), 0, s, order, g.hdr, rank, n, g.cnt);
+    const ScanJob sj{g.cnt, g.out_ptr, (long long)n + 1, nullptr, g.scan_cnt};
+    rc = scan_lookback(&sj, 1, s);
+    if (rc != GM_OK) return rc;
+    hipLaunchKernelGGL(class_place_kernel, dim3((unsigned)cdiv(n, 256)), dim3(256), 0, s, order, g.hdr, g.cnt, g.out_ptr, n,
+                       n_per > 0 && n_per < n ? n_per : n, perm);
     GM_LAUNCH_CHECK();
     return GM_OK;
 }
@@ -971,7 +997,7 @@
 namespace gm {
 namespace {
 int csr_tail(const GraphWs& g, int64_t n, int K, const CsrWs& c, const float* pos, int64_t pos_stride, float conn_r, float* edge_attr,
-             int flow, bool with_cnt_scan, hipStream_t s) {
+             int flow, bool with_cnt_scan, int64_t n_live, hipStream_t s) {
     const int64_t cap = n * K;
     const unsigned nb = (unsigned)cdiv(cap, 256);
     int* slot = c.sort_tmp;
@@ -981,7 +1007,7 @@
     if (rc != GM_OK) return rc;
     const EdgeBlocks t = carve_edge_blocks(c.blocks, n, cap);
     hipLaunchKernelGGL(fill_graph_kernel, dim3(nb), dim3(256), 0, s, g.cnt, g.out_ptr, g.nbr, n, K, c.in_ptr,
-                       slot, cap, flow, c.dst, c.src, c.eid, c.hdr, &g.hdr->n_per_graph, t.hdr, t.gblk);
+                       slot, cap, flow, c.dst, c.src, c.eid, c.hdr, &g.hdr->n_per_graph, t.hdr, t.gblk, (int)n_live);
     int gb = (int)cdiv(cdiv(cap, kBlockEdges) + 8, 256);
     gb = gb < 1 ? 1 : (gb > 512 ? 512 : gb);
     const BlockTabArgs bt{c.dst, t.hdr, t.gblk, t.blk, t.seg, t.head, t.stitch, t.stitch_list, gb};
@@ -1006,7 +1032,7 @@
     if (rc == GM_OK) rc = launch_step_clear(clr, s);
     if (rc != GM_OK || n <= 0) return rc;
     hipLaunchKernelGGL(indeg_graph_kernel, dim3((unsigned)cdiv(cap, 256)), dim3(256), 0, s, g.cnt, g.nbr, n, K, flow, c.in_ptr, c.sort_tmp);
-    return csr_tail(g, n, K, c, pos, pos_stride, conn_r, edge_attr, flow, false, s);
+    return csr_tail(g, n, K, c, pos, pos_stride, conn_r, edge_attr, flow, false, n, s);
 }
 
 int radius_graph_build_fused(const float* pos, int64_t pos_stride, int64_t n, int64_t n_per, double conn_r, int K, void* graph_ws,
@@ -1020,12 +1046,12 @@
     return radius_graph_build_core(pos, pos_stride, n, n_per, conn_r, K, g, c.in_ptr, c.sort_tmp, flow, s);
 }
 int csr_from_graph_fused(const void* graph_ws, int64_t n, int K, void* csr_ws, size_t csr_ws_bytes, const float* pos, int64_t pos_stride,
-                         float conn_r, float* edge_attr, int flow, hipStream_t s) {
+                         float conn_r, float* edge_attr, int flow, int64_t n_live, hipStream_t s) {
     if (n <= 0) return GM_OK;
     GraphWs g = carve_graph(const_cast<void*>(graph_ws), n, K);
     CsrWs c = carve_csr(csr_ws, n, n * K);
     GM_REQUIRE(csr_ws_bytes >= c.bytes, GM_ERR_WORKSPACE, "csr_from_graph_fused: workspace %zu < %zu", csr_ws_bytes, c.bytes);
-    return csr_tail(g, n, K, c, pos, pos_stride, conn_r, edge_attr, flow, true, s);
+    return csr_tail(g, n, K, c, pos, pos_stride, conn_r, edge_attr, flow, true, n_live, s);
 }
 }
 
diff --git a/gnn_manip_amd/csrc/hedge.h b/gnn_manip_amd/csrc/hedge.h
--- a/gnn_manip_amd/csrc/hedge.h
+++ b/gnn_manip_amd/csrc/hedge.h
@@ -10,7 +10,8 @@
     int n_graphs;
     int n_per_graph;
     int n_stitch;
-    int pad[3];
+    int n_groups_live;
+    int pad[2];
 };
 struct EdgeBlocks {
     EdgeBlockHeader* hdr;
diff --git a/gnn_manip_amd/csrc/hedge.hip b/gnn_manip_amd/csrc/hedge.hip
--- a/gnn_manip_amd/csrc/hedge.hip
+++ b/gnn_manip_amd/csrc/hedge.hip
@@ -293,7 +293,7 @@
 __global__ void __launch_bounds__(SYS_THREADS, 1) sys_edge_kernel(const CsrHeader* a_hdr, const int* __restrict__ a_dst, const int* __restrict__ a_src, const float* __restrict__ a_P,
                                                                        const float* a_e_in, float* a_e_out, float* __restrict__ a_agg, const float* __restrict__ a_hw,
                                                                        const int2* __restrict__ a_blk, const int2* __restrict__ a_seg, const int* __restrict__ a_head,
-                                                                       const EdgeBlockHeader* __restrict__ a_tab, unsigned a_side_off, unsigned a_agg_bytes, unsigned a_P_bytes,
+                                                                       const int* __restrict__ a_n_groups, unsigned a_side_off, unsigned a_agg_bytes, unsigned a_P_bytes,
                                                                        int* a_flags, float a_eps, int a_residual) {
     const int tid = threadIdx.x, lane0 = tid & 63;
     const int wave = __builtin_amdgcn_readfirstlane(tid >> 6);
@@ -303,7 +303,7 @@
     const int role = wave >> 2, jb = wave & 3;
 #endif
     const int E = a_hdr->n_edges;
-    const int2 cr = wg_range(a_tab->n_groups, true);
+    const int2 cr = wg_range(*a_n_groups, true);
     if (cr.y <= cr.x) return;
     const int b0 = 4 * cr.x, b1 = 4 * cr.y;
     const int nb = b1 - b0;
@@ -1255,7 +1255,7 @@
 
 __global__ void __launch_bounds__(256) edge_blocks_plan_kernel(const int* __restrict__ in_ptr, int n_nodes, const int* n_per_dev, int n_per_host,
                                                                EdgeBlockHeader* tab, int* gblk, int max_graphs) {
-    if (threadIdx.x == 0) edge_blocks_plan(in_ptr, n_nodes, n_per_dev, n_per_host, tab, gblk, max_graphs);
+    if (threadIdx.x == 0) edge_blocks_plan(in_ptr, n_nodes, n_per_dev, n_per_host, tab, gblk, max_graphs, n_nodes);
 }
 
 __global__ void __launch_bounds__(256) edge_blocks_fill_kernel(const int* __restrict__ in_ptr, const int* __restrict__ dst, int n_nodes,
@@ -1356,7 +1356,8 @@
     const bool stream = (uint64_t)edge_capacity * H * 4 > kStreamStoreBytes;
     auto go = [&](auto kern) {
         return launch_sys<decltype(kern)::value>(SYS_LDS_BYTES, a.prof, PROF_EDGE, s, a.hdr, a.dst, a.src, a.P, a.e_in, a.e_out, a.agg, a.wstream_h3,
-                                                 t.blk, t.seg, t.head, t.hdr, (unsigned)(a.side - a.agg), (unsigned)agg_bytes,
+                                                 t.blk, t.seg, t.head, a.live_only ? &t.hdr->n_groups_live : &t.hdr->n_groups,
+                                                 (unsigned)(a.side - a.agg), (unsigned)agg_bytes,
                                                  (unsigned)((uint64_t)a.n_nodes_tab * 2 * H * 4), const_cast<int*>(&a.hdr->error_flags), a.eps, a.residual);
     };
     auto pick = [&](auto np_c) {
diff --git a/gnn_manip_amd/csrc/mlp.h b/gnn_manip_amd/csrc/mlp.h
--- a/gnn_manip_amd/csrc/mlp.h
+++ b/gnn_manip_amd/csrc/mlp.h
@@ -28,6 +28,7 @@
     float eps;
     int residual;
     int discard_e_out;
+    int live_only;
     int P_prescaled;
     int k1;
     int h_valid;
diff --git a/gnn_manip_amd/csrc/model.h b/gnn_manip_amd/csrc/model.h
--- a/gnn_manip_amd/csrc/model.h
+++ b/gnn_manip_amd/csrc/model.h
@@ -60,6 +60,7 @@
     std::mutex lazy_mu;
     gm::ProfState* prof = nullptr;
     int edge_kernel = gm::EK_AUTO;
+    bool prune_rigid = true;
     bool node_fusion = true;
     int precision = gm::kPrecisionF32;
     hipEvent_t ready = nullptr;
diff --git a/gnn_manip_amd/csrc/model.hip b/gnn_manip_amd/csrc/model.hip
--- a/gnn_manip_amd/csrc/model.hip
+++ b/gnn_manip_amd/csrc/model.hip
@@ -475,11 +475,12 @@
 
 int epd_forward_impl(const gm_model* m, const float* nodes, int64_t n, const float* edge_attr, int attr_is_csr_order,
                      const void* csr_ws, int64_t cap, float* out, void* fwd_ws, size_t fwd_ws_bytes, void* stream, bool agg_cleared,
-                     int64_t n_per_graph) {
+                     int64_t n_per_graph, int64_t n_live) {
     gm::DevGuard dev_guard(out);
     GM_REQUIRE(m && csr_ws && fwd_ws, GM_ERR_INVALID_ARGUMENT, "gm_epd_forward: null pointer");
     GM_REQUIRE(n >= 0 && cap >= 0 && n < ((int64_t)1 << 31) && cap < ((int64_t)1 << 31), GM_ERR_INVALID_ARGUMENT, "gm_epd_forward: sizes out of range");
     if (n == 0) return GM_OK;
+    GM_REQUIRE(n_live >= 0 && n_live <= n, GM_ERR_INVALID_ARGUMENT, "gm_epd_forward: live rows out of range");
     GM_REQUIRE(nodes && out && (edge_attr || cap == 0), GM_ERR_INVALID_ARGUMENT, "gm_epd_forward: null tensor");
     const int H = m->Hp, NL = m->NL, M = m->M;
     FwdWs f = carve_fwd(fwd_ws, H, n, cap, cap);
@@ -526,20 +527,24 @@
         EdgeArgs ea = proc_edge_args(m, k, c, n, nullptr, f.P, f.e, f.e, f.agg, f.side, 1);
         ea.discard_e_out = k + 1 == M;
         ea.P_prescaled = route.sys_edge;
+        const int64_t rows = k + 1 == M ? n_live : n;
+        ea.live_only = rows < n;
         rc = launch_edge(H, NL, false, route.sys_edge, ea, cap, s);
         if (rc != GM_OK) return rc;
+        if (rows == 0) return GM_OK;
         if (route.sys_node) {
-            rc = launch_agg_stitch(f.agg, f.side, carve_edge_blocks(c.blocks, n, cap), n, m->prof, s);
+            rc = launch_agg_stitch(f.agg, f.side, carve_edge_blocks(c.blocks, n, cap), rows, m->prof, s);
             NodeSysArgs ns{};
             ns.h = f.h; ns.agg = f.agg; ns.Q = f.Q; ns.h_out = f.h; ns.image = m->packed_h3 + m->h3_node[k];
-            ns.n = (int)n; ns.flags = flags; ns.eps = m->d.ln_eps; ns.prof = m->prof;
+            ns.n = (int)rows; ns.flags = flags; ns.eps = m->d.ln_eps; ns.prof = m->prof;
             ns.precision = m->precision;
             const bool fused = k + 1 < M && m->node_fusion;
             if (rc == GM_OK) rc = fused ? launch_node_proj_sys(ns, proj_args(k + 1), s) : launch_node_sys(ns, s);
             if (rc == GM_OK && k + 1 < M && !fused) rc = launch_proj_sys(proj_args(k + 1), s);
-            if (rc == GM_OK && k + 1 == M) rc = launch_node_hm(H, 2, tail_args(m, M, n, f.h, f.P, out, flags), s);
+            if (rc == GM_OK && k + 1 == M) rc = launch_node_hm(H, 2, tail_args(m, M, rows, f.h, f.P, out, flags), s);
         } else {
             HmNodeArgs a = proc_node_args(m, k, c, n, cap, f.h, f.agg, f.side, f.h, 1);
+            a.n_nodes = (int)rows;
             set_tail(m, a, k + 1, f.P, out, route.sys_edge);
             rc = launch_node_hm(H, 1, a, s);
         }
@@ -553,7 +558,7 @@
 
 int gm_epd_forward(const gm_model* m, const float* nodes, int64_t n, const float* edge_attr, int attr_is_csr_order,
                    const void* csr_ws, int64_t cap, float* out, void* fwd_ws, size_t fwd_ws_bytes, void* stream) {
-    return epd_forward_impl(m, nodes, n, edge_attr, attr_is_csr_order, csr_ws, cap, out, fwd_ws, fwd_ws_bytes, stream, false, n);
+    return epd_forward_impl(m, nodes, n, edge_attr, attr_is_csr_order, csr_ws, cap, out, fwd_ws, fwd_ws_bytes, stream, false, n, n);
 }
 
 int gm_graph_independent_forward(const gm_model* m, const float* x, int64_t n, const float* edge_attr, int64_t e,
@@ -659,6 +664,12 @@
     return GM_OK;
 }
 
+int gm_model_set_prune_rigid(gm_model* m, int on) {
+    GM_REQUIRE(m, GM_ERR_INVALID_ARGUMENT, "gm_model_set_prune_rigid: null model");
+    m->prune_rigid = on != 0;
+    return GM_OK;
+}
+
 int gm_model_set_precision(gm_model* m, int precision) {
     GM_REQUIRE(m, GM_ERR_INVALID_ARGUMENT, "gm_model_set_precision: null model");
     GM_REQUIRE(precision == GM_PRECISION_F32 || precision == GM_PRECISION_F16, GM_ERR_INVALID_ARGUMENT,
@@ -705,7 +716,7 @@
 namespace {
 int rollout_step_impl(const gm_model* m, float* obs, int64_t n, const gm_feature_desc* fd, int K, const int32_t* rigid_rank,
                       const float* rigid_target, float* pred_acc_out, const gm::RecordedDrive* rec, void* ws, size_t ws_bytes,
-                      void* stream) {
+                      void* stream, int64_t n_live) {
     gm::DevGuard dev_guard(obs);
     GM_REQUIRE(m && obs && fd && ws, GM_ERR_INVALID_ARGUMENT, "gm_rollout_step: null pointer");
     int rc = gm::check_model_for_scene(m->d, fd, "gm_rollout_step");
@@ -714,6 +725,8 @@
     RolloutWs r = carve_rollout(ws, &m->d, n, K);
     GM_REQUIRE(ws_bytes >= r.bytes, GM_ERR_WORKSPACE, "gm_rollout_step: workspace %zu < %zu", ws_bytes, r.bytes);
     if (n == 0) return GM_OK;
+    GM_REQUIRE(n_live == n || (n_live >= 0 && n_live < n && rigid_rank && !rec && !pred_acc_out && gm::graph_nodes(fd, n) == n),
+               GM_ERR_INVALID_ARGUMENT, "gm_rollout_step: live rows need the scripted drive of one graph without a prediction record");
     const int64_t cap = n * K;
     hipStream_t hs = (hipStream_t)stream;
     {
@@ -737,10 +750,10 @@
     {
         ProfScope prof(m->prof, PROF_REST, hs);
         rc = gm::csr_from_graph_fused(r.graph, n, K, r.csr, r.csr_bytes, last_pos, fd->data_dim, (float)fd->conn_r, r.edge_attr,
-                                      m->d.flow, hs);
-    }
-    if (rc != GM_OK) return rc;
-    rc = epd_forward_impl(m, r.x, n, r.edge_attr, 1, r.csr, cap, r.pred, r.fwd, r.fwd_bytes, stream, true, gm::graph_nodes(fd, n));
+                                      m->d.flow, n_live, hs);
+    }
+    if (rc != GM_OK) return rc;
+    rc = epd_forward_impl(m, r.x, n, r.edge_attr, 1, r.csr, cap, r.pred, r.fwd, r.fwd_bytes, stream, true, gm::graph_nodes(fd, n), n_live);
     if (rc != GM_OK) return rc;
     ProfScope prof(m->prof, PROF_REST, hs);
     return gm::rollout_integrate_post(obs, n, fd, r.pred, rigid_rank, rigid_target, pred_acc_out, hs, rec);
@@ -751,7 +764,7 @@
 
 int gm_rollout_step(const gm_model* m, float* obs, int64_t n, const gm_feature_desc* fd, int K, const int32_t* rigid_rank,
                     const float* rigid_target, float* pred_acc_out, void* ws, size_t ws_bytes, void* stream) {
-    return rollout_step_impl(m, obs, n, fd, K, rigid_rank, rigid_target, pred_acc_out, nullptr, ws, ws_bytes, stream);
+    return rollout_step_impl(m, obs, n, fd, K, rigid_rank, rigid_target, pred_acc_out, nullptr, ws, ws_bytes, stream, n);
 }
 
 size_t gm_rollout_renumber_workspace_bytes(const gm_feature_desc* fd, int64_t n) {
@@ -786,6 +799,8 @@
         r = carve_rollout(ws, &m->d, n, K);
         GM_REQUIRE(ws_bytes >= r.bytes, GM_ERR_WORKSPACE, "%s: workspace %zu < %zu", who, ws_bytes, r.bytes);
     }
+    const bool by_class = renum && !drive.frames && rigid_rank && n_rigid > 0 && n_rigid <= n;
+    const int64_t n_live = by_class && m->prune_rigid && gm::graph_nodes(fd, n) == n ? n - n_rigid : n;
     float* state = obs;
     const int* rank = rigid_rank;
     const int* total = nullptr;
@@ -794,10 +809,10 @@
         if (renum && i % renumber_every == 0) {
             const float* last_pos = state + (size_t)(fd->k_steps - 1) * frame + fd->cart_col;
             int rc = gm::cell_order(last_pos, fd->data_dim, n, gm::graph_nodes(fd, n), fd->conn_r, K, r.graph,
-                                    r.graph_bytes, rw.perm, hs);
+                                    r.graph_bytes, rw.perm, by_class ? rank : nullptr, hs);
             if (rc != GM_OK) return rc;
-            rc = gm::renumber_gather(state, rw.state[flip], fd->k_steps, n, fd->data_dim, rw.perm, r.graph, total, rw.total[flip],
-                                     rigid_rank, rigid_rank ? rw.rank : nullptr, hs);
+            rc = gm::renumber_gather(state, rw.state[flip], fd->k_steps, n, fd->data_dim, rw.perm, by_class ? nullptr : r.graph, total,
+                                     rw.total[flip], rigid_rank, rigid_rank ? rw.rank : nullptr, hs);
             if (rc != GM_OK) return rc;
             state = rw.state[flip];
             total = rw.total[flip];
@@ -807,7 +822,7 @@
         if (drive.frames) {
             const gm::RecordedDrive rec{drive.frames + (size_t)i * frame, total, record_last ? record_last + (size_t)i * frame : nullptr,
                                         drive.record_pred ? drive.record_pred + (size_t)i * n * 3 : nullptr};
-            int rc = rollout_step_impl(m, state, n, fd, K, rank, nullptr, nullptr, &rec, ws, ws_bytes, stream);
+            int rc = rollout_step_impl(m, state, n, fd, K, rank, nullptr, nullptr, &rec, ws, ws_bytes, stream, n);
             if (rc != GM_OK) return rc;
             continue;
         }
@@ -820,7 +835,7 @@
             else GM_HIP_CHECK(hipMemcpyAsync(record_last + (size_t)i * frame, last, frame * sizeof(float), hipMemcpyDeviceToDevice, hs));
             if (rc != GM_OK) return rc;
         }
-        int rc = gm_rollout_step(m, state, n, fd, K, rank, target, nullptr, ws, ws_bytes, stream);
+        int rc = rollout_step_impl(m, state, n, fd, K, rank, target, nullptr, nullptr, ws, ws_bytes, stream, n_live);
         if (rc != GM_OK) return rc;
     }
     if (total) return gm::renumber_scatter(state, obs, fd->k_steps, n, fd->data_dim, total, hs);
diff --git a/gnn_manip_amd/rollout.py b/gnn_manip_amd/rollout.py
--- a/gnn_manip_amd/rollout.py
+++ b/gnn_manip_amd/rollout.py
@@ -139,7 +139,7 @@
     RENUMBER_EVERY = 64
 
     def __init__(self, model, graph_attr, n_nodes, k_steps=6, data_dim=None, max_neighbours=20, device="cuda:0",
-                 candidates=1, renumber="auto"):
+                 candidates=1, renumber="auto", prune_rigid=True):
         self.model = model
         self.graph_attr = graph_attr
         self.candidates = int(candidates)
@@ -164,6 +164,7 @@
             renumber = os.environ["GM_RENUMBER"] == "1"
         self.renumber = (self.n_per >= self.RENUMBER_MIN_NODES) if renumber == "auto" else bool(renumber)
         self._renumber_ws = None
+        self.prune_rigid = bool(prune_rigid)
 
     def _rank_rigid(self, obs):
         rank = torch.empty(self.n, dtype=torch.int32, device=self.device)
@@ -334,6 +335,8 @@
         recs = torch.empty((steps, self.n, self.data_dim), dtype=torch.float32, device=self.device) if record else None
         handle = self.model.device_handle(self.device)
         every, rws = self._renumbering(steps)
+        if every:
+            check(lib().gm_model_set_prune_rigid(handle, int(self.prune_rigid)))
         check(lib().gm_rollout(handle, ptr(obs), self.n, C.byref(self.fdesc), self.max_neighbours, ptr(self.rigid_rank),
                            ptr(trajectory), T, self.n_rigid, steps, ptr(recs), every, ptr(rws), 0 if rws is None else rws.numel(),
                            ptr(self.ws), self.ws.numel(), current_stream()))
diff --git a/include/gnn_manip_hip.h b/include/gnn_manip_hip.h
--- a/include/gnn_manip_hip.h
+++ b/include/gnn_manip_hip.h
@@ -129,6 +129,7 @@
 
 int gm_model_set_edge_kernel(gm_model* m, int choice);
 int gm_model_set_node_fusion(gm_model* m, int on);
+int gm_model_set_prune_rigid(gm_model* m, int on);
 enum { GM_PRECISION_F32 = 0, GM_PRECISION_F16 = 1 };
 int gm_model_set_precision(gm_model* m, int precision);
 
```
